# utiasASRL/dICP

Hardware: AMD Instinct MI355X
Metric: ICP cloud-iterations/sec (fwd+bwd), B=256x16384-pt clouds per GPU (higher is better)
Workload: dtype f32

## Files before the change

### dicp_amd/ICP.py

```python
import os.path as osp

import torch
import yaml

from . import _call, _lib
from ._ops import F16_SWEEP_MIN_TARGETS, F16_SWEEP_STATIC_TARGETS, KabschLoop, compute_device, pack_list, packable, prebuild_search, transform_points
from ._loop import CallHints, ICPLoop, LoopConfig, form_tally_wanted, resort_schedule
from .nn import nn


class ICP:
    def __init__(self, config_path=None, icp_type='pt2pl', max_iterations=100, tolerance=1e-12, differentiable=True):
        if config_path is None:
            config_path = osp.join(osp.dirname(osp.abspath(__file__)), 'config', 'dICP_config.yaml')
        with open(config_path, 'r') as f:
            self.config = yaml.safe_load(f)

        prm, log, fun = (self.config['dICP'][k] for k in ('parameters', 'logging', 'functionality'))
        self.icp_type = icp_type
        self.max_iterations = max_iterations
        self.tolerance = tolerance
        self.const_iter = prm['const_iter']
        self.verbose = log['verbose']
        self.target_pad_val = prm['target_pad_val']
        self.source_zeroes_are_pad = prm['source_zeroes_are_pad']
        self.match_ratio_thresh = log['matched_ratio_thresh']
        self.diff = differentiable
        self.nn = nn(self.diff, use_gumbel=fun['gumbel'], eps=fun['gumbel_eps'], tau=fun['gumbel_tau'])
        self.knn_variant = _lib.KNN_AUTO
        self.knn_stats = {}
        self.reuse_matches = True
        self.bwd_window = True
        self.bwd_skip_eps = None
        self.sync_every = None
        self.strict_errors = False
        self.deterministic = False
        self._tuning = dict(
            small_loop=True,
            sweep_resort=None,
            cert_from=None,
            cert_sets=True,
            cert_hint=True,
            cert_backoff=True,
            first_search=True,
            plan_call=True,
            bwd_tail=True,
            one_call=True,
            timing_events=None)
        self._hints = CallHints()
        self._eye = {}

    def icp(self, source, target, T_init, weight=None, trim_dist=None, loss_fn=None, dim=3, source_rows=None, target_rows=None):
        return self.dICP(source, target, T_init, weight, trim_dist, loss_fn, dim, source_rows, target_rows)

    def dICP(self, source, target, T_init, weight=None, trim_dist=None, loss_fn=None, dim=3, source_rows=None, target_rows=None):
        assert dim == 2 or dim == 3, "dim must be 2 or 3"
        unit_w = (weight is None and isinstance(source, torch.Tensor) and isinstance(target, torch.Tensor) and len(source) > 0 and len(target) > 0
                  and not self.source_zeroes_are_pad and not (self.nn.differentiable and self.nn.use_gumbel))
        source, target, T_init, w_pts, rows, per_cloud_w = self._batch(source, target, T_init, weight, unit_weights=unit_w)
        per_cloud_w = per_cloud_w and source.shape[1] > 1 and not self.source_zeroes_are_pad
        assert source.dtype == target.dtype == T_init.dtype
        if self.icp_type == 'pt2pl':
            assert target.shape[2] == 6
        else:
            target = target[:, :, :3]
        if loss_fn is not None and loss_fn['name'] not in ('huber', 'cauchy', 'trim'):
            raise ValueError("Invalid loss name: {}".format(loss_fn['name']))
        home = source.device
        dev = home if source.is_cuda else compute_device()
        source, target, T_init = (t.to(dev) for t in (source, target, T_init))
        w_pts = w_pts.to(dev) if w_pts is not None else None
        src_rows, tgt_rows = self._device_rows(rows, dev)
        if source_rows is not None or target_rows is not None:
            if rows is not None:
                raise ValueError("source_rows / target_rows describe a padded batch: not together with lists of clouds")
            src_rows, tgt_rows = self._given_rows(source_rows, source, "source_rows"), self._given_rows(target_rows, target, "target_rows")
            if src_rows is not None:
                live = (torch.arange(source.shape[1], device=dev)[None, :] < src_rows[:, None]).to(source.dtype)
                w_pts = live if w_pts is None else w_pts * live

        if dim == 2:
            key = ("dim2", source.dtype, dev)
            if key not in self._eye:
                self._eye[key] = torch.tensor([1.0, 1.0, 0.0, 1.0, 1.0, 0.0], dtype=source.dtype, device=dev)
            keep_t = self._eye[key][:target.shape[2]]
            source = source * self._eye[key][:3]
            target = target * keep_t

        loss_name = loss_fn['name'] if loss_fn is not None else None
        soft = bool(self.nn.differentiable and self.nn.use_gumbel)
        if not soft:
            target = target.contiguous()
            source = source.contiguous()
        wants_grad = torch.is_grad_enabled() and any(t.requires_grad for t in (source, target, T_init, w_pts) if t is not None)
        first_search = bool(self._tuning["first_search"]) and self._tuning["timing_events"] is None and not (wants_grad and not self.bwd_window)
        deterministic = bool(self.deterministic) and wants_grad
        if deterministic and soft:
            raise NotImplementedError("ICP.deterministic: not with Gumbel-softmax correspondences (their adjoint adds to the target with float atomics)")
        cfg = LoopConfig(
            icp_type=self.icp_type, differentiable=bool(self.diff), max_iterations=int(self.max_iterations),
            tolerance=float(self.tolerance), trim_dist=trim_dist, loss_name=loss_name,
            loss_metric=float(loss_fn['metric']) if loss_fn is not None else 1.0, dim=dim,
            const_iter=bool(self.const_iter),
            tanh_steepness=float(self.config['dICP']['parameters']['tanh_steepness']),
            match_ratio_thresh=float(self.match_ratio_thresh),
            knn_variant=(_lib.KNN_SWEEP | (self.knn_variant & 0xff00)) if deterministic else self.knn_variant, bwd_window=True if deterministic else bool(self.bwd_window),
            deterministic=deterministic, stats_out=self.knn_stats, hints=self._hints,
            sync_every=self.sync_every, timing_events=self._tuning["timing_events"], small_loop=False if deterministic else bool(self._tuning["small_loop"]),
            src_rows=src_rows, tgt_rows=tgt_rows, sweep_resort=resort_schedule(self._tuning["sweep_resort"], source.shape[0], source.shape[1], int(self.max_iterations), bool(self.reuse_matches), self._tuning["cert_from"]), reuse_matches=bool(self.reuse_matches), cert_from=self._tuning["cert_from"],
            bwd_skip_eps=self.bwd_skip_eps, cert_backoff=bool(self._tuning["cert_backoff"]), cert_sets=bool(self._tuning["cert_sets"]), cert_hint=bool(self._tuning["cert_hint"]),
            plan_call=bool(self._tuning["plan_call"]), bwd_tail=bool(self._tuning["bwd_tail"]), first_search=first_search, strict_errors=bool(self.strict_errors),
            gumbel=(self.nn.eps, self.nn.tau, getattr(self.nn, "_inject_U", None)) if soft else None)
        T_c = T_init.contiguous()
        if self._tuning["one_call"] and not deterministic and _call.eligible(cfg, source, target, T_c, w_pts, wants_grad):
            T, pc, deltas, weights, costs, converged, iterations, matched = _call.CallLoop.apply(source, target, T_c, w_pts, cfg)
        else:
            if not soft:
                rec = self._hints.form_record(dev, (source.shape[0], source.shape[1], target.shape[1], source.dtype)) if source.is_cuda else None
                cfg.prebuilt = prebuild_search(source, target, cfg.knn_variant, wants_grad and bool(cfg.bwd_window), T_init, src_rows, tgt_rows, first_search=first_search,
                                               tally=target.shape[1] < F16_SWEEP_STATIC_TARGETS and form_tally_wanted(rec, target.shape[1] >= F16_SWEEP_MIN_TARGETS))
            T, pc, deltas, weights, costs, converged, iterations, matched = ICPLoop.apply(source.contiguous(), target.contiguous(), T_init, w_pts, cfg)

        if per_cloud_w:
            n_pts = float(source.shape[1])
            on = (w_pts[:, 0] > self.match_ratio_thresh) & (matched > 0)
            matched = torch.where(on, torch.round(matched * n_pts), matched)
        if self.verbose:
            print("ICP converged in {} iterations".format(deltas.shape[1]))
            print("Final del_T_ts: {}".format(torch.linalg.norm(deltas[:, -1])))

        if self.icp_type == 'pt2pt':
            weights = weights.repeat_interleave(3, dim=2)
        results = {
            "pc": pc,
            "T": T,
            "costs": costs.unsqueeze(-1),
            "deltas": deltas.unsqueeze(-1),
            "weights": weights.unsqueeze(-1),
            "stats": {"converged": converged, "iterations": iterations, "matched_ratio": matched},
        }
        if home != dev:
            results = {k: (v.to(home) if k != "stats" else {s: x.to(home) for s, x in v.items()})
                       for k, v in results.items()}
        return results

    def check_errors(self):
        self._hints.check(wait=True)

    def pt2pt_dICP_SVD(self, source, target, T_init, trim_dist=None, huber_delta=None, dim=3, weight=None):
        single = not isinstance(source, list) and source is not None and source.dim() == 2
        s_b, t_b, T_b, w_pts, rows, _ = self._batch(source, target, T_init, weight)
        t_b = t_b[:, :, :3]
        assert s_b.dtype == t_b.dtype == T_b.dtype
        home = s_b.device
        dev = home if s_b.is_cuda else compute_device()
        s_b, t_b, T_b, w_pts = (t.to(dev) for t in (s_b, t_b, T_b, w_pts))
        src_rows, tgt_rows = self._device_rows(rows, dev)
        seed = bool(getattr(self, "svd_seed_T_init", False))
        if seed:
            T_start = T_b
        else:
            key = (int(T_b.shape[0]), T_b.dtype, dev)
            T_start = self._eye.get(key)
            if T_start is None:
                if len(self._eye) > 16:
                    self._eye.clear()
                T_start = self._eye[key] = torch.eye(4, dtype=T_b.dtype, device=dev).expand(T_b.shape[0], 4, 4).contiguous()
        if self._tuning["one_call"] and _call.kabsch_eligible(s_b, t_b, T_start, w_pts, bool(self.const_iter), self.knn_variant, src_rows, tgt_rows):
            T_found, pc, costs, iterations = _call.KabschCall.apply(s_b, t_b, T_start, w_pts, int(self.max_iterations), trim_dist)
        else:
            T_found, costs, iterations = KabschLoop.apply(s_b, t_b, T_start, w_pts, int(self.max_iterations), float(self.tolerance),
                                                          trim_dist, bool(self.const_iter), self.knn_variant, src_rows, tgt_rows, self.sync_every)
            pc = transform_points(s_b, T_found)
        if self.verbose:
            print("ICP converged in {} iterations".format(int(iterations.max().item()) - 1))
        T = T_found if seed else torch.matmul(T_found, T_b)
        self.svd_stats = {"costs": costs, "iterations": iterations}
        if home != dev:
            pc, T = pc.to(home), T.to(home)
        return (pc[0], T[0]) if single else (pc, T)

    def batch_size_handling(self, source, target, T_init=None, weight=None):
        s, t, T, w, _, _ = self._batch(source, target, T_init, weight)
        if self.icp_type == 'pt2pt':
            w = w.repeat_interleave(3, dim=1)
        return s, t, T, w

    @staticmethod
    def _device_rows(rows, dev):
        if rows is None:
            return None, None
        src_len, tgt_len, n_max, m_max = rows
        out = []
        for lens, full, extra in ((src_len, n_max, 0), (tgt_len, m_max, 1)):
# ... 137 lines not shown
```

### dicp_amd/_call.py

```python
import ctypes

import torch

from . import _lib
from . import _loop
from . import _ops
from ._ops import _DT, _on, _p, _stream

MAX_POINTS = 1 << 20
_PLANS = {}


def eligible(cfg, source, target, T_init, w0, need_grad):
    if cfg.gumbel is not None or not cfg.const_iter or cfg.timing_events is not None or cfg.src_rows is not None or cfg.tgt_rows is not None:
        return False
    if not cfg.plan_call or (cfg.knn_variant & 0xff00) or (need_grad and not cfg.bwd_window):
        return False
    dt = source.dtype
    if dt not in _DT or not (source.is_cuda and target.is_cuda and T_init.is_cuda) or target.dtype != dt or T_init.dtype != dt:
        return False
    if not (source.is_contiguous() and target.is_contiguous() and T_init.is_contiguous()) or (w0 is not None and not (w0.is_cuda and w0.is_contiguous() and w0.dtype == dt)):
        return False
    N, n, _ = source.shape
    m, c = target.shape[1], target.shape[2]
    if N * n > MAX_POINTS or N * m > 4 * MAX_POINTS:
        return False
    if tuple(T_init.shape) != (N, 4, 4) or c != (6 if cfg.icp_type == "pt2pl" else 3):
        return False
    kind = cfg.knn_variant & 0xff
    if kind == _lib.KNN_AUTO:
        kind = _ops.auto_knn_kind(N, n, m)
    if kind != _lib.KNN_SWEEP:
        return False
    Kmax = int(cfg.max_iterations)
    resorts = [k for k in cfg.sweep_resort if 0 <= k < Kmax]
    if len([k for k in resorts if k > 0]) >= _lib.MAX_SEGMENTS:
        return False
    cert_from = (max(resorts) if resorts else 0) if cfg.cert_from is None else max(0, int(cfg.cert_from))
    if _loop.certificates_pay(cfg.reuse_matches, Kmax, cert_from, N, n):
        return False
    if _ops.F16_SWEEP and dt == torch.float32 and float(N) * n >= _ops.F16_SWEEP_MIN_QUERIES and m >= _ops.F16_SWEEP_MIN_TARGETS:
        return False
    if _ops.HIST_CHUNK_BYTES // max(1, N * n * max(source.element_size(), 4)) < Kmax:
        return False
    return not torch.cuda.is_current_stream_capturing()


def _plan(code, N, n, m, c, K, dim, need_grad, resort, flags):
    key = (code, N, n, m, c, K, dim, need_grad, resort, flags)
    got = _PLANS.get(key)
    if got is None:
        call = _lib.Call(N=N, n=n, m=m, c=c, K=K, dim=dim, need_grad=need_grad, n_resort=len(resort), flags=flags)
        for i, k in enumerate(resort):
            call.resort[i] = k
        lay = _lib.CallLayout()
        _lib.check(_lib.load().dicp_call_plan(code, ctypes.byref(call), ctypes.byref(lay)), "dicp_call_plan")
        if len(_PLANS) > 256:
            _PLANS.clear()
        got = _PLANS[key] = lay
    return got


class CallLoop(torch.autograd.Function):

    @staticmethod
    def forward(ctx, source, target, T_init, w0, cfg):
        lib = _lib.load()
        dev, dt = source.device, source.dtype
        code, es = _DT[dt], source.element_size()
        N, n, _ = source.shape
        m, c = target.shape[1], target.shape[2]
        K = int(cfg.max_iterations)
        need_grad = int(any(ctx.needs_input_grad[:4]))
        stats = cfg.stats_out
        if stats is not None:
            for key in ("knn_pairs", "searched_again", "budgets", "bwd_live", "certs_off"):
                stats.pop(key, None)
        ctx.set_materialize_grads(False)
        resort = tuple(sorted(set(k for k in cfg.sweep_resort if 0 < k < K)))
        flags = (_lib.CALL_FIRST_SEARCH if cfg.first_search else 0) | (0 if cfg.small_loop else _lib.CALL_NO_SMALL_LOOP)
        L = _plan(code, N, n, m, c, K, int(cfg.dim), need_grad, resort, flags)
        P = cfg.params()
        with _on(dev):
            ws = torch.empty((L.total // es,), dtype=dt, device=dev)
            rs = torch.empty((L.results_total // es,), dtype=dt, device=dev)
            T = torch.empty((N, 4, 4), dtype=dt, device=dev)
            pc = torch.empty((N, n, 3), dtype=dt, device=dev)
            call = _lib.Call(T_out=T.data_ptr(), pc_out=pc.data_ptr(), results=rs.data_ptr(), src=source.data_ptr(), tgt=target.data_ptr(), T_init=T_init.data_ptr(), w0=w0.data_ptr() if w0 is not None else None,
                             N=N, n=n, m=m, c=c, K=K, dim=int(cfg.dim), need_grad=need_grad, n_resort=len(resort), flags=flags,
                             directions=int(_ops.FRAME_DIRECTIONS), quantum=_ops.CENTER_QUANTUM, tolerance=float(cfg.tolerance), workspace=ws.data_ptr())
            for i, k in enumerate(resort):
                call.resort[i] = k
            _lib.check(lib.dicp_call_forward(code, ctypes.byref(P), ctypes.byref(call), _stream()), "dicp_call_forward")
        def piece(off, count, shape):
            return rs.narrow(0, off // es, count).view(shape).data
        deltas = piece(L.deltas, N * K * 6, (N, K, 6))
        weights = piece(L.weights, N * K * n, (N, K, n))
        costs = piece(L.costs, N * K, (N, K))
        iterations = piece(L.iterations, N, (N,))
        matched = piece(L.matched_ratio, N, (N,))
        conv = rs[L.converged // es:L.converged // es + (N + es - 1) // es].view(torch.uint8)[:N].bool()
        if stats is not None:
            stats["knn_pairs"] = ws[L.pairs // es:L.pairs // es + _lib.PAIR_SHARDS * 8 // es].view(torch.int64).clone()
        if need_grad:
            ctx.save_for_backward(source, target, w0, deltas)
            ctx.ws, ctx.call, ctx.cfg, ctx.P, ctx.L = ws, call, cfg, P, L
        ctx.mark_non_differentiable(deltas, weights, costs, conv, iterations, matched)
        return T, pc, deltas, weights, costs, conv, iterations, matched

    @staticmethod
    def backward(ctx, gT, gpc, *_unused):
        src, tgt, w0, deltas = ctx.saved_tensors
        cfg, P, call, FL = ctx.cfg, ctx.P, ctx.call, ctx.L
        lib = _lib.load()
        dev, dt = src.device, src.dtype
        code, es = _DT[dt], src.element_size()
        N, n, _ = src.shape
        m = tgt.shape[1]
        K = call.K
        stats = cfg.stats_out
        want_tgt, want_w = bool(ctx.needs_input_grad[1]), bool(ctx.needs_input_grad[3] and w0 is not None)
        with _on(dev):
            st = _stream()
            gsrc_pc = None
            if gpc is not None:
                gsrc_pc = torch.empty_like(src)
                pcp = torch.empty((N, FL.nblk, _lib.NBWD_PAD), dtype=dt, device=dev)
                pose_K = ctx.ws.as_strided((N, 12), (12, 1), FL.poses // es + K * N * 12)
                _lib.check(lib.dicp_transform_points_bwd(code, _p(src), _p(pose_K), _p(gpc.contiguous()), _p(gsrc_pc), _p(pcp), N, n, st), "dicp_transform_points_bwd")
                gT_pc = _ops._pose_sums_to_gT(pcp, N, dt, dev, st)
                gT = gT_pc if gT is None else gT + gT_pc
            base = ctx.ws.data_ptr()
            F = _lib.LoopBackwardIn(src=src.data_ptr(), tgt_sorted=base + FL.tgt_sorted, w0=w0.data_ptr() if w0 is not None else None, tperm=base + FL.tperm,
                                    qorder=base + FL.orders + (FL.n_orders - 1) * N * n * 4, spos=base + FL.spos, poses=base + FL.poses, deltas=deltas.data_ptr(),
                                    areg=base + FL.areg, alive=base + FL.alive, N=N, n=n, m=m, c=call.c, K=K, K_cap=K, m_pad=FL.m_pad, dim=call.dim,
                                    knn_variant=_lib.KNN_SWEEP | ((1 << 25) if (call.flags & _lib.CALL_NO_SMALL_LOOP) else 0))
            gsrc, gtgt, gT0, gw = _loop.backward_once(lib, code, P, F, cfg, src, tgt, w0, gT, want_tgt, want_w)
            if gsrc_pc is not None:
                gsrc += gsrc_pc
        return gsrc, gtgt, gT0, gw, None


def kabsch_eligible(source, target, T_start, w0, const_iter, knn_variant, src_rows, tgt_rows):
    if not const_iter or src_rows is not None or tgt_rows is not None or (knn_variant & 0xff00):
        return False
    dt = source.dtype
    if dt not in _DT or not (source.is_cuda and target.is_cuda and T_start.is_cuda and w0.is_cuda) or target.dtype != dt or T_start.dtype != dt or w0.dtype != dt:
        return False
    N, n, _ = source.shape
    m = target.shape[1]
    if N * n > MAX_POINTS or N * m > 4 * MAX_POINTS or tuple(T_start.shape) != (N, 4, 4) or tuple(w0.shape) != (N, n):
        return False
    kind = knn_variant & 0xff
    if kind == _lib.KNN_AUTO:
        kind = _ops.auto_knn_kind(N, n, m)
    return kind == _lib.KNN_SWEEP and not torch.cuda.is_current_stream_capturing()


_KPLANS = {}


class KabschCall(torch.autograd.Function):

# ... 63 lines not shown
```

### dicp_amd/_lib.py

```python
import ctypes
import os
import subprocess
import threading

_HERE = os.path.dirname(os.path.abspath(__file__))
_ROOT = os.path.dirname(_HERE)
LIB_PATH = os.environ.get("DICP_HIP_LIB") or os.path.join(_HERE, "libdicp_hip.so")
SOURCES = [os.path.join(_HERE, "csrc", f) for f in ("dicp_kernels.hip", "knn_f16.hip", "dicp_call.hip", "normals.hip", "voxel.hip", "knn_points.hip")]
HEADERS = ([os.path.join(_HERE, "csrc", f) for f in ("dicp_math.h", "dicp_common.h", "dicp_internal.h", "dicp_fill.h", "dicp_normals.h", "dicp_voxel.h", "dicp_topk.h")]
           + [os.path.join(_HERE, "csrc", "kernels_%s.h" % f) for f in ("setup", "search", "setup_sort", "rows", "accumulate", "backward", "soft_svd", "host")]
           + [os.path.join(_ROOT, "include", "dicp_hip.h")])

F32, F64 = 0, 1
PT2PT, PT2PL = 0, 1
LOSS_NONE, LOSS_HUBER, LOSS_CAUCHY, LOSS_TRIM = 0, 1, 2, 3
KNN_AUTO, KNN_VALU, KNN_MFMA, KNN_SWEEP, KNN_GUMBEL = 0, 1, 2, 3, 4
NACC_PAD, NBWD_PAD, KAB_SAVE = 32, 16, 40
PAIR_SHARDS = 64
ABI_VERSION = 11
_ERRORS = {1: "null pointer", 2: "bad shape/stride", 3: "unsupported dtype", 4: "bad enum value", 5: "misaligned buffer"}

vp, i32, i64, f64 = ctypes.c_void_p, ctypes.c_int32, ctypes.c_int64, ctypes.c_double


# ... 32 lines not shown
    _fields_ = [("spos_ref", vp), ("gts_far", vp), ("overwrite", i32), ("skip", vp), ("mref", vp), ("live", vp), ("skip_eps", f64), ("tail_from", i32), ("tail_partials", vp),
                ("tail_arrive", vp), ("det_far_row", vp), ("det_far_val", vp)]


class LoopBuffers(ctypes.Structure):
    _fields_ = [("abi", i32), ("src", vp), ("tgt", vp), ("w_init", vp), ("c", i32), ("K", i32), ("converged", vp), ("iterations", vp), ("matched_ratio", vp), ("n_start", vp), ("n_matched", vp),
                ("partials", vp), ("counters", vp), ("counters_host", vp), ("counters_tag", i32), ("events", vp), ("src_rows", vp), ("tgt_rows", vp),
                ("search", SearchBuffers), ("cert", CertBuffers), ("hist", HistoryBuffers), ("bwd", BwdBuffers)]

    def __init__(self, **kw):
        super().__init__(abi=ABI_VERSION)
        subs = (self, self.search, self.cert, self.hist, self.bwd)
        where = LoopBuffers._KW
        for k, v in kw.items():
            if v is not None:
                i, f = where[k]
                setattr(subs[i], f, v)


LoopBuffers._KW = dict([(f[0], (0, f[0])) for f in LoopBuffers._fields_[:-4]] +
                       [(g + "_" + f[0], (i + 1, f[0])) for i, (g, cls) in enumerate((("search", SearchBuffers), ("cert", CertBuffers), ("hist", HistoryBuffers), ("bwd", BwdBuffers)))
                        for f in cls._fields_])


class GumbelLoop(ctypes.Structure):
    _fields_ = [("U", vp), ("seeds", vp), ("eps", f64), ("tau", f64), ("ps_t", vp), ("nbr", vp), ("lse", vp), ("g_nbr", vp), ("g_ps", vp)]


MAX_SEGMENTS = 16
CERT_OFF_FOR_GOOD = 1 << 20


class SegmentPlan(ctypes.Structure):
    _fields_ = [("nseg", i32), ("k0", i32 * MAX_SEGMENTS), ("k1", i32 * MAX_SEGMENTS), ("new_order", i32 * MAX_SEGMENTS),
                ("cert_from", i32), ("pad0", i32), ("order", vp * MAX_SEGMENTS), ("keys", vp), ("cert_q", vp), ("cert_qu", vp), ("cert_count", vp), ("cert_cloud", vp), ("cert_set", vp),
                ("cert_nbr", vp), ("cert_gdirty", vp), ("cert_pend", vp), ("cert_cm", vp), ("cert_glist", vp), ("cert_gcount", vp), ("cert_slist", vp), ("cert_scount", vp)]


class Call(ctypes.Structure):
    _fields_ = [("src", vp), ("tgt", vp), ("T_init", vp), ("w0", vp), ("N", i32), ("n", i32), ("m", i32), ("c", i32), ("K", i32), ("dim", i32), ("need_grad", i32),
                ("n_resort", i32), ("resort", i32 * MAX_SEGMENTS), ("flags", i32), ("directions", i32), ("quantum", f64), ("tolerance", f64), ("workspace", vp), ("results", vp), ("T_out", vp), ("pc_out", vp)]


_sz = ctypes.c_size_t


class CallLayout(ctypes.Structure):
    _fields_ = ([(k, _sz) for k in ("total", "zeroed", "results_total", "results_zeroed", "T", "pc", "deltas", "weights", "costs", "converged", "iterations", "matched_ratio", "pairs", "n_matched", "counters",
                                    "poses", "poses_search", "alive", "areg", "n_start", "partials", "tgs4", "tperm", "bucket", "brange", "keys", "tgt_sorted", "scratch",
                                    "scratch_bytes", "frame", "pose_s", "orders", "spos")]
                + [("n_orders", i32), ("m_pad", i32), ("nblk", i32), ("pad0", i32)])


class CallGrads(ctypes.Structure):
    _fields_ = [("gT", vp), ("gsrc", vp), ("gtgt", vp), ("gT0", vp), ("gw", vp), ("workspace", vp), ("skip_eps", f64), ("tail_from", i32), ("pad0", i32), ("live_host", vp)]


class CallBackwardLayout(ctypes.Structure):
    _fields_ = ([(k, _sz) for k in ("total", "zeroed", "live", "arrive", "mref", "decisions", "far", "gpose", "gtmp", "src_s", "w_s", "gsrc_s", "gw_s", "slab", "gs", "gb",
                                    "partials", "tail_partials", "spos_ref")] + [("nblk_w", i32), ("pad0", i32)])


class LoopBackwardIn(ctypes.Structure):
    _fields_ = ([(k, vp) for k in ("src", "tgt_sorted", "w0", "tperm", "qorder", "spos", "poses", "deltas", "areg", "alive", "src_rows", "tgt_rows", "spos_of")]
                + [(k, i32) for k in ("N", "n", "m", "c", "K", "K_cap", "m_pad", "dim", "knn_variant", "spos_of_from")]
                + [(k, vp) for k in ("src_s", "w_s", "spos_ref")])


class KabschCall(ctypes.Structure):
    _fields_ = [("src", vp), ("tgt", vp), ("T_start", vp), ("w0", vp), ("N", i32), ("n", i32), ("m", i32), ("c", i32), ("K", i32), ("trim_on", i32), ("directions", i32), ("pad0", i32),
                ("trim_dist", f64), ("quantum", f64), ("tolerance", f64), ("workspace", vp), ("T_out", vp), ("pc_out", vp)]


class KabschCallLayout(ctypes.Structure):
    _fields_ = ([(k, _sz) for k in ("total", "zeroed", "costs", "iterations", "pairs", "counters", "frame", "keys", "tperm", "bucket", "brange", "tgs4", "scratch", "scratch_bytes",
                                    "pose", "pose_search", "pose_used", "partials", "save", "idx", "rows_live", "orders", "gpose", "gacc")] + [("m_pad", i32), ("nblk", i32)])


class KabschCallGrads(ctypes.Structure):
    _fields_ = [("gT", vp), ("gsrc", vp), ("gtgt", vp), ("gw", vp)]


CALL_FIRST_SEARCH, CALL_NO_SMALL_LOOP, CALL_NBKT = 1, 2, 1024


class KabschBuffers(ctypes.Structure):
    _fields_ = [("src", vp), ("tgt", vp), ("w_init", vp), ("c", i32), ("K", i32), ("knn_variant", i32), ("m_pad", i32), ("tgt4", vp), ("tperm", vp),
                ("qorder", vp), ("bucket", vp), ("brange", vp), ("nbkt", i32), ("pad0", i32), ("pairs", vp), ("frame", vp), ("pose", vp),
                ("pose_search", vp), ("pose_used", vp), ("idx", vp), ("partials", vp), ("save", vp), ("costs", vp), ("iterations", vp),
                ("rows_live", vp), ("tgt_rows", vp), ("counters", vp), ("tgt_f16", vp)]


_SIGNATURES = {
    "dicp_abi_version": ([], ctypes.c_int),
    "dicp_copy": ([vp, vp, ctypes.c_size_t, vp], ctypes.c_int),
    "dicp_zero": ([vp, ctypes.c_size_t, vp], ctypes.c_int),
    "dicp_padded_targets": ([i32], ctypes.c_int),
    "dicp_accumulate_blocks": ([i32], ctypes.c_int),
    "dicp_pack_target": ([i32, vp, i32, vp, vp, i32, i32, vp, i32, vp], ctypes.c_int),
    "dicp_search_frame": ([i32, vp, i32, vp, i32, i32, f64, i32, vp, vp, i32, vp, vp, vp], ctypes.c_int),
    "dicp_knn_f16_bytes": ([i32, i32], ctypes.c_size_t),
    "dicp_knn_f16_pack": ([vp, vp, i32, i32, i32, vp, vp], ctypes.c_int),
    "dicp_knn_f16_probe": ([vp, vp, vp, vp, vp, vp, i32, i32, i32, i32, vp, vp], ctypes.c_int),
    "dicp_knn": ([i32, vp, vp, vp, vp, vp, i32, i32, i32, i32, vp, i32, vp, vp], ctypes.c_int),
    "dicp_knn_sweep": ([i32, vp, vp, vp, vp, vp, vp, vp, i32, vp, vp, i32, i32, i32, i32, vp, vp, vp, i32, vp, vp, vp, i32, vp], ctypes.c_int),
    "dicp_window_blocks": ([i32, i32, i32], ctypes.c_int),
    "dicp_window_rows": ([i32], ctypes.c_int),
    "dicp_bwd_tail_max_blocks": ([i32], ctypes.c_int),
    "dicp_sweep_sort_scratch_bytes": ([i32, i32, i32], ctypes.c_size_t),
    "dicp_sweep_sort": ([i32, vp, i32, vp, vp, i32, i32, i32, vp, vp, i32, vp, vp, vp, ctypes.c_size_t, vp], ctypes.c_int),
    "dicp_sweep_build": ([i32, vp, i32, vp, vp, vp, i32, i32, i32, vp, vp, i32, vp], ctypes.c_int),
    "dicp_sweep_setup": ([i32, vp, i32, vp, i32, i32, i32, f64, i32, vp, vp, vp, i32, vp, vp, vp, ctypes.c_size_t, vp, vp, i32, vp, vp, i32, vp, vp, vp, vp], ctypes.c_int),
    "dicp_query_order": ([i32, vp, vp, vp, i32, i32, i32, vp, vp, vp, vp, i32, vp, i32, vp, vp, i32, vp, vp, vp], ctypes.c_int),
    "dicp_query_reorder": ([i32, vp, vp, vp, vp, vp, i32, i32, i32, vp, i32, vp, vp, i32, vp, vp, vp], ctypes.c_int),
    "dicp_query_keys": ([i32, vp, vp, i32, i32, vp, vp], ctypes.c_int),
    "dicp_loop_init": ([i32, vp, vp, ctypes.c_double, i32, i32, i32, vp, vp, vp, vp, vp, vp, vp, vp, i32, vp], ctypes.c_int),
    "dicp_search_pose": ([i32, vp, vp, i32, vp, vp], ctypes.c_int),
    "dicp_loop_finish": ([i32, vp, vp, vp, vp, i32, i32, vp, vp, vp, vp], ctypes.c_int),
    "dicp_accumulate_bwd_window": ([i32, ctypes.POINTER(WeightParams), vp, vp, i32, vp, vp, vp, vp, vp, vp, vp, vp, vp, i32, i32, i32, vp, vp, vp, vp, vp, i32, vp], ctypes.c_int),
    "dicp_resolve_matches": ([vp, vp, i32, vp, i32, i32, vp, vp], ctypes.c_int),
    "dicp_match_order_scratch_bytes": ([i32, i32, i32], ctypes.c_size_t),
    "dicp_match_order": ([i32, vp, vp, i32, i32, vp, ctypes.c_size_t, vp, vp], ctypes.c_int),
    "dicp_window_reduce": ([i32, vp, vp, vp, vp, vp, vp, i32, i32, i32, i32, i32, vp, i32, i32, vp], ctypes.c_int),
    "dicp_permute_add_rows": ([i32, vp, vp, i32, i32, i32, i32, i32, i32, vp, i32, i32, vp], ctypes.c_int),
    "dicp_pose_grad_in": ([i32, vp, vp, i32, vp], ctypes.c_int),
    "dicp_pose_grad_out": ([i32, vp, vp, i32, vp, i32, vp], ctypes.c_int),
    "dicp_permute_rows": ([i32, vp, vp, i32, i32, i32, i32, i32, i32, vp, i32, i32, vp], ctypes.c_int),
    "dicp_gather_rows": ([i32, vp, vp, i32, i32, i32, i32, vp, vp], ctypes.c_int),
    "dicp_scatter_add_rows": ([i32, vp, vp, i32, i32, i32, i32, vp, vp], ctypes.c_int),
    "dicp_pack_list": ([i32, vp, vp, vp, i32, i32, i32, vp, vp, vp], ctypes.c_int),
    "dicp_unpack_list": ([i32, vp, vp, vp, vp, i32, i32, i32, i32, vp], ctypes.c_int),
    "dicp_accumulate": ([i32, ctypes.POINTER(WeightParams), vp, vp, i32, vp, vp, vp, vp, vp, i32, i32, i32, vp, vp, i64, vp], ctypes.c_int),
    "dicp_step": ([i32, ctypes.POINTER(StepIO), i32, vp], ctypes.c_int),
    "dicp_icp_forward": ([i32, ctypes.POINTER(WeightParams), ctypes.POINTER(LoopBuffers), i32, i32, i32, i32, i32, f64, i32, i32, vp], ctypes.c_int),
    "dicp_icp_forward_plan": ([i32, ctypes.POINTER(WeightParams), ctypes.POINTER(LoopBuffers), ctypes.POINTER(SegmentPlan), i32, i32, i32, i32, i32, f64, vp], ctypes.c_int),
    "dicp_icp_backward": ([i32, ctypes.POINTER(WeightParams), ctypes.POINTER(LoopBuffers), i32, i32, i32, i32, vp, vp, i32, vp, vp, vp, vp, vp, vp, i32, i32, vp], ctypes.c_int),
    "dicp_step_bwd": ([i32, vp, vp, i32, i32, vp, vp, i64, vp, vp, vp, vp, i32, vp], ctypes.c_int),
    "dicp_accumulate_bwd": ([i32, ctypes.POINTER(WeightParams), vp, vp, i32, vp, vp, vp, vp, vp, vp, vp, i32, i32, i32, vp, vp, vp, vp, vp], ctypes.c_int),
    "dicp_gumbel_nn": ([i32, vp, vp, i32, vp, ctypes.c_uint32, f64, f64, i32, i32, i32, vp, vp, vp], ctypes.c_int),
    "dicp_gumbel_nn_bwd": ([i32, vp, vp, i32, vp, ctypes.c_uint32, f64, f64, vp, vp, vp, i32, i32, i32, vp, vp, vp], ctypes.c_int),
    "dicp_kabsch_accumulate": ([i32, vp, vp, i32, vp, vp, vp, i32, f64, vp, i32, i32, i32, vp, vp], ctypes.c_int),
    "dicp_kabsch_step": ([i32, vp, i32, vp, vp, vp, i32, vp], ctypes.c_int),
    "dicp_kabsch_step_bwd": ([i32, vp, vp, vp, i32, vp], ctypes.c_int),
    "dicp_kabsch_forward": ([i32, ctypes.POINTER(KabschBuffers), i32, i32, i32, i32, f64, i32, f64, i32, i32, vp], ctypes.c_int),
    "dicp_kabsch_bwd": ([i32, vp, vp, i32, vp, vp, vp, i32, f64, vp, vp, i32, i32, i32, vp, vp, vp, vp], ctypes.c_int),
    "dicp_transform_points": ([i32, vp, vp, vp, i32, i32, vp], ctypes.c_int),
    "dicp_transform_points_bwd": ([i32, vp, vp, vp, vp, vp, i32, i32, vp], ctypes.c_int),
    "dicp_loss_weight": ([i32, i32, i32, f64, f64, vp, i64, i32, vp, vp], ctypes.c_int),
    "dicp_loss_weight_bwd": ([i32, i32, i32, f64, f64, vp, vp, i64, i32, vp, vp], ctypes.c_int),
    "dicp_call_plan": ([i32, ctypes.POINTER(Call), ctypes.POINTER(CallLayout)], ctypes.c_int),
    "dicp_call_forward": ([i32, ctypes.POINTER(WeightParams), ctypes.POINTER(Call), vp], ctypes.c_int),
    "dicp_call_backward_plan": ([i32, ctypes.POINTER(WeightParams), ctypes.POINTER(Call), i32, i32, ctypes.POINTER(CallBackwardLayout)], ctypes.c_int),
    "dicp_call_backward": ([i32, ctypes.POINTER(WeightParams), ctypes.POINTER(Call), ctypes.POINTER(CallGrads), vp], ctypes.c_int),
    "dicp_loop_backward_plan": ([i32, ctypes.POINTER(WeightParams), ctypes.POINTER(LoopBackwardIn), i32, i32, ctypes.POINTER(CallBackwardLayout)], ctypes.c_int),
    "dicp_loop_backward": ([i32, ctypes.POINTER(WeightParams), ctypes.POINTER(LoopBackwardIn), ctypes.POINTER(CallGrads), vp], ctypes.c_int),
    "dicp_loop_backward_prepare": ([i32, ctypes.POINTER(LoopBackwardIn), vp, vp, vp, vp], ctypes.c_int),
    "dicp_kabsch_call_plan": ([i32, ctypes.POINTER(KabschCall), ctypes.POINTER(KabschCallLayout)], ctypes.c_int),
    "dicp_kabsch_call_forward": ([i32, ctypes.POINTER(KabschCall), vp], ctypes.c_int),
    "dicp_kabsch_call_backward": ([i32, ctypes.POINTER(KabschCall), ctypes.POINTER(KabschCallGrads), vp], ctypes.c_int),
    "dicp_normals_workspace_bytes": ([i32, i32, i32, i32, i32, i32], ctypes.c_size_t),
    "dicp_normals_forward": ([i32, vp, i32, vp, i32, i32, i32, vp, i32, vp, vp, vp, vp, ctypes.c_size_t, vp, vp], ctypes.c_int),
    "dicp_normals_backward": ([i32, vp, vp, vp, i32, vp, i32, i32, i32, i32, vp, vp, vp, ctypes.c_size_t, vp], ctypes.c_int),
    "dicp_voxel_workspace_bytes": ([i32, i32, i32, i32], ctypes.c_size_t),
    "dicp_voxel_count": ([i32, vp, i32, vp, i32, i32, f64, f64, f64, vp, i32, i32, vp, vp, ctypes.c_size_t, vp], ctypes.c_int),
    "dicp_voxel_reduce": ([i32, vp, i32, i32, i32, i32, vp, ctypes.c_size_t, vp, vp, vp, vp], ctypes.c_int),
    "dicp_voxel_backward": ([i32, vp, vp, vp, i32, i32, i32, i32, vp, vp], ctypes.c_int),
# ... 74 lines not shown
```

### dicp_amd/_loop.py

```python
import ctypes
import time
from dataclasses import dataclass
from types import SimpleNamespace

import torch

from . import _lib
from . import _ops
from ._ops import (_DT, _LOSS, SweepIndex, _Arena, _gather_rows_raw, _on, _p, _pose_sums_to_gT, _segments, _stream, auto_knn_kind, f16_image,
                   pack_target, require_device, search_frame)


def form_tally_wanted(rec, have_image):
    if rec is None:
        return bool(have_image)
    reporting = rec["event"] is None and (rec["calls"] < 2 or rec["calls"] % 16 == 0)
    return bool(reporting or ((have_image or rec["long"]) and not rec.get("plan")))



class TailTimeout(RuntimeError):
    """A wait inside the one-launch tail of a backward pass ran out (dicp_hip.h, bwd_tail_arrive): that pass poisoned the gradients of the clouds
    concerned with NaN.  Raised by the pass itself when ICP.strict_errors is set (it then waits for its own kernels), else at the next backward pass of the
    same ICP object, or by ICP.check_errors()."""
# ... 26 lines not shown

    def tail_records(self, dev, shape, any_stream=False):
        key = self._where(dev) + tuple(shape)
        if any_stream and not self.tail.get(key):
            same = [recs for k, recs in self.tail.items() if k[0] == key[0] and k[2:] == key[2:] and recs]
            if same:
                return max(same, key=lambda recs: recs[-1][5])
        return self._slot(self.tail, key, list)

    def form_record(self, dev, shape):
        return self._slot(self.form, self._where(dev) + tuple(shape), lambda: {"long": False, "host": None, "event": None, "calls": 0})

    def cert_record(self, dev, shape):
        return self._slot(self.cert, self._where(dev) + tuple(shape), lambda: {"skip": 0, "host": None, "event": None, "calls": 0})

    def check(self, wait=False):
        for recs in self.tail.values():
            for rec in recs:
                if rec[1] is None or rec[4]:
                    continue
                if wait:
                    rec[1].synchronize()
                if rec[1].query():
                    rec[4] = True
                    if int(rec[0][rec[3]]) != 0:
                        raise TailTimeout("dicp_amd: a wait of an earlier backward pass's one-launch tail ran out (the GPU was kept full by other work for "
                                          "~0.5 s); the gradients of that pass were poisoned with NaN.  Re-run it, or set ICP._tuning['bwd_tail'] = False"
                                          "  [report word 0x%08x: arrivals seen %d, block %d, generation %d; live clouds by iteration %s]"
                                          % (int(rec[0][rec[3]]) & 0xffffffff, (int(rec[0][rec[3]]) >> 16) & 0xfff, (int(rec[0][rec[3]]) >> 8) & 0xff,
                                             int(rec[0][rec[3]]) & 0xff, rec[0][:rec[3]].tolist()))


CERT_MIN_WORK = 2.0e6
RESORT_SMALL_POINTS = 262144


def certificates_pay(reuse_matches, Kmax, cert_from, N, n):
    left = Kmax - 1 - cert_from
    return bool(reuse_matches) and left >= 3 and float(left) * N * n >= CERT_MIN_WORK


def resort_schedule(resort, N, n, Kmax, reuse_matches, cert_from):
    if resort is not None:
        return tuple(int(v) for v in resort)
    full, small = (0, 1, 2, 3), (0, 1)
    cf = max([k for k in full if k < Kmax] or [0]) if cert_from is None else max(0, int(cert_from))
    if certificates_pay(reuse_matches, Kmax, cf, N, n) or N * n >= RESORT_SMALL_POINTS:
        return full
    cf_small = max([k for k in small if k < Kmax] or [0]) if cert_from is None else cf
    return full if certificates_pay(reuse_matches, Kmax, cf_small, N, n) else small




@dataclass
class LoopConfig:
    icp_type: str
    differentiable: bool
    max_iterations: int
    tolerance: float
    trim_dist: object
    loss_name: object
    loss_metric: float
    dim: int
    const_iter: bool
    tanh_steepness: float
    match_ratio_thresh: float
    knn_variant: int = _lib.KNN_AUTO
    sweep_resort: tuple = (0, 1, 2, 3)
    bwd_window: bool = True
    stats_out: object = None
    hints: object = None
    sync_every: object = None
    timing_events: object = None
    prebuilt: object = None
    small_loop: bool = True
    cert_from: object = None
    gumbel: object = None
    deterministic: bool = False
    bwd_tail: bool = True
    strict_errors: bool = False
    plan_call: bool = True
    first_search: bool = True
    cert_hint: bool = True
    cert_sets: bool = True
    cert_backoff: bool = True
    reuse_matches: bool = True
    bwd_skip_eps: object = None
    src_rows: object = None
    tgt_rows: object = None

    def params(self):
        return _lib.WeightParams(
            mode=_lib.PT2PL if self.icp_type == "pt2pl" else _lib.PT2PT,
            trim_on=int(self.trim_dist is not None and self.trim_dist >= 0.0),
            differentiable=int(self.differentiable),
            loss=_LOSS[self.loss_name],
            trim_dist=float(self.trim_dist if self.trim_dist is not None else 0.0),
            tanh_k=float(self.tanh_steepness),
            loss_delta=float(self.loss_metric),
            match_thresh=float(self.match_ratio_thresh))



def order_by_matches(src, spos_ref, m, m_pad, src_rows, tgt_rows):
    N, n, _ = src.shape
    qo = torch.empty((N, n), dtype=torch.int32, device=src.device)
    unused = torch.ones((N, 2), dtype=src.dtype, device=src.device)
    with _on(src.device):
        _lib.check(_lib.load().dicp_query_order(_DT[src.dtype], _p(src), None, _p(unused), SweepIndex.NBKT, N, n, _p(qo), None, None, None, 0, _p(spos_ref), int(m_pad),
                                                None, None, int(m), _p(src_rows), _p(tgt_rows), _stream()), "dicp_query_order")
    return qo


def backward_once(lib, code, P, F, cfg, src, tgt, w0c, gT, want_tgt, want_w):
    dev, dt = src.device, src.dtype
    es = src.element_size()
    N, n, m, K, Kcap = F.N, F.n, F.m, F.K, F.K_cap
    stats = cfg.stats_out
    st = _stream()
    L = _lib.CallBackwardLayout()
    _lib.check(lib.dicp_loop_backward_plan(code, ctypes.byref(P), ctypes.byref(F), int(want_tgt), int(want_w), ctypes.byref(L)), "dicp_loop_backward_plan")
    eps = cfg.bwd_skip_eps
    if eps is None:
        eps = 2.0 ** -22 if dt == torch.float32 else 2.0 ** -40
    if cfg.loss_name == "huber" and not cfg.differentiable:
        eps = 0.0
    ws = torch.empty((L.total // es,), dtype=dt, device=dev)
    if stats is not None and eps > 0.0:
        stats["bwd_live"] = ws[L.live // es:L.live // es + (Kcap + 1 + (es // 4) - 1) * 4 // es].view(torch.int32)[:Kcap + 1]
    tail_from, hints, entry = 0, None, None
    capturing = torch.cuda.is_current_stream_capturing()
    use_tail = eps > 0.0 and cfg.bwd_tail and cfg.hints is not None
    if use_tail:
        if not capturing:
            cfg.hints.check()
        hints = cfg.hints.tail_records(dev, (N, n, m, Kcap, dt), any_stream=capturing)
        hint = next((h for h in reversed(hints) if h[2] == (N, n, K) and (capturing or h[1].query())), None)
        if hint is not None and L.nblk_w <= lib.dicp_bwd_tail_max_blocks(code):
            counts = hint[0][:K].tolist()
            tail_from = min(K, max(0, next((k for k in range(K) if counts[k] * 8 >= N), K) - 1))
        if not capturing:
            if len(hints) >= 4:
                if hints[0][1].query() and hints[0][0].numel() >= Kcap + 1:
                    cfg.hints.check()
                    entry = hints.pop(0)
            else:
                entry = [torch.empty((max(Kcap + 1, 64),), dtype=torch.int32).pin_memory(), None, None, Kcap, False, 0]
    tail_word = None
    if tail_from > 0:
        a0 = L.arrive // es
        tail_word = ws[a0:a0 + (N + 1 + (es // 4) - 1) * 4 // es].view(torch.int32)[N:N + 1]
    if stats is not None:
        stats["bwd_tail_from"] = int(tail_from)
        stats["bwd_tail_error"] = tail_word
    gsrc = torch.empty_like(src)
    gtgt = torch.empty_like(tgt) if want_tgt else None
    gw = torch.empty_like(w0c) if want_w else None
    gT0 = torch.empty((N, 4, 4), dtype=dt, device=dev)
    gTc = gT.contiguous() if gT is not None else None
    G = _lib.CallGrads(gT=gTc.data_ptr() if gTc is not None else None, gsrc=gsrc.data_ptr(), gtgt=gtgt.data_ptr() if want_tgt else None,
                       gT0=gT0.data_ptr(), gw=gw.data_ptr() if want_w else None, workspace=ws.data_ptr(), skip_eps=float(eps), tail_from=int(tail_from),
                       live_host=entry[0].data_ptr() if entry is not None else None)
    _lib.check(lib.dicp_loop_backward(code, ctypes.byref(P), ctypes.byref(F), ctypes.byref(G), st), "dicp_loop_backward")
    if entry is not None:
        entry[1] = torch.cuda.Event()
# ... 34 lines not shown
    S.kind = kind
    S.owned = kind == _lib.KNN_SWEEP and S.need_grad and cfg.bwd_window
    if cfg.deterministic and S.need_grad and not S.owned:
        raise NotImplementedError("ICP.deterministic covers the sweep search with the windowed backward (knn_variant KNN_SWEEP, bwd_window): this call "
                                  "would take another form")
    sweep = None
    with_q = S.T_init.dtype == dt and tuple(S.T_init.shape) == (N, 4, 4)
    if kind == _lib.KNN_SWEEP:
        pre = cfg.prebuilt
        if (pre is not None and pre[0].data_ptr() == S.tgt.data_ptr() and pre[0].shape == S.tgt.shape and pre[0].dtype == S.tgt.dtype
                and pre[1].tgt_s is not None and pre[1].tgt_rows is cfg.tgt_rows):
            sweep = pre[1]
        else:
            sweep = SweepIndex(S.tgt, sorted_rows=True, tgt_rows=cfg.tgt_rows,
                               frame=search_frame(S.tgt, tgt_rows=cfg.tgt_rows, src=S.src if with_q else None, T_init=S.T_init if with_q else None, src_rows=cfg.src_rows))
    S.sweep = sweep
    S.soft = kind == _lib.KNN_GUMBEL
    S.center = sweep.frame if sweep is not None else (None if S.soft else search_frame(S.tgt, tgt_rows=cfg.tgt_rows, src=S.src if with_q else None,
                                                                                   T_init=S.T_init if with_q else None, src_rows=cfg.src_rows))
    S.tgt4 = sweep.tgs4 if sweep is not None else (None if S.soft else pack_target(S.tgt, S.center, cfg.tgt_rows))
    S.m_pad = S.tgt4.shape[1] if S.tgt4 is not None else 0
    img16 = f16_image(S.tgt4, m, cfg.tgt_rows) if kind == _lib.KNN_MFMA else (sweep.img16 if sweep is not None else None)
    tally = (sweep is not None and _ops.F16_SWEEP and _ops.F16_SWEEP_ADAPTIVE and dt == torch.float32 and float(N) * n >= _ops.F16_SWEEP_MIN_QUERIES
             and not (cfg.knn_variant & 0xff00) and m < _ops.F16_SWEEP_STATIC_TARGETS)
    form_hint = None
    if tally and cfg.hints is not None and not torch.cuda.is_current_stream_capturing():
        form_hint = cfg.hints.form_record(dev, (N, n, m, dt))
        if form_hint["event"] is not None and form_hint["event"].query():
            rep = form_hint["host"].tolist()
            form_hint["long"] = bool(4 * rep[0] >= N)
            form_hint["moving"] = bool(4 * rep[1] >= N)
            form_hint["plan"] = [0] + [0 if c < 0 else (2 if 2 * c >= N else 1) for c in rep[2:2 + _ops.FORM_PLAN_ITERS]]
            form_hint["event"] = None
        if img16 is None and form_hint["long"]:
            img16 = sweep.make_image()
    S.form_plan = None
    if tally and img16 is not None and form_hint is not None and form_hint.get("plan"):
        pl = form_hint["plan"]
        S.form_plan = (ctypes.c_int32 * S.Kmax)(*[(pl[k] if k < len(pl) else pl[-1]) for k in range(S.Kmax)])
    if tally and not form_tally_wanted(form_hint, img16 is not None):
        tally = False
    S.img16, S.tally, S.form_hint = img16, tally, form_hint
    S.adaptive = bool(tally) and kind == _lib.KNN_SWEEP


def _fwd_certificate_policy(S):
    cfg, N, n, m, dt, dev, Kmax, sweep = S.cfg, S.N, S.n, S.m, S.dt, S.dev, S.Kmax, S.sweep
    S.keep_idx = (sweep is None or (S.need_grad and not S.owned)) and not S.soft
    resorts = [k for k in cfg.sweep_resort if 0 <= k < Kmax]
    S.cert_from = (max(resorts) if resorts else 0) if cfg.cert_from is None else max(0, int(cfg.cert_from))
    want_certs = sweep is not None and not (cfg.knn_variant & 0xff00) and not S.keep_idx and certificates_pay(cfg.reuse_matches, Kmax, S.cert_from, N, n)
    cert_hint = None
    clouds_moving = False
    if want_certs and cfg.cert_hint and cfg.cert_backoff and cfg.hints is not None and not torch.cuda.is_current_stream_capturing():
        cert_hint = cfg.hints.cert_record(dev, (N, n, m, Kmax, dt))
        if cert_hint["host"] is None or cert_hint["host"].shape[0] < N:
            cert_hint["host"] = torch.empty((N, 8), dtype=torch.int32).pin_memory()
        if cert_hint["skip"] > 0:
            cert_hint["skip"] -= 1
            want_certs = False
            clouds_moving = bool(cert_hint.get("moving", False))
        elif cert_hint["event"] is not None and cert_hint["event"].query():
            hc = cert_hint["host"][:N]
            most_off = float((hc[:, 2] > 0).float().mean()) >= 0.5
            if most_off or (N * ((n + 127) // 128) <= 8192 and bool((hc[:, 7] >= 2).any())):
                cert_hint.update(skip=31, calls=0, moving=most_off)
                want_certs = False
                clouds_moving = most_off
            cert_hint["event"] = None
        if want_certs:
            cert_hint["calls"] += 1
    S.clouds_moving = bool(clouds_moving or (not want_certs and S.form_hint is not None and S.form_hint.get("moving", False)))
    S.want_certs, S.cert_hint = want_certs, cert_hint


def _fwd_loop_state(S):
    cfg, lib, N, n, m, c, dt, dev, es, Kmax, sweep = S.cfg, S.lib, S.N, S.n, S.m, S.c, S.dt, S.dev, S.es, S.Kmax, S.sweep
    S.nblk = lib.dicp_accumulate_blocks(n)
    S.poses = torch.empty((Kmax + 1, N, 12), dtype=dt, device=dev)
    S.poses_c = torch.empty((Kmax + 1, N, 12), dtype=dt, device=dev) if S.center is not None else None
    S.alive = torch.empty((Kmax + 1, N), dtype=dt, device=dev)
    S.areg = torch.empty((Kmax, N, 36), dtype=torch.float64, device=dev) if S.need_grad else None
    S.n_start = torch.empty((N,), dtype=dt, device=dev)
    S.partials = torch.empty((N, S.nblk, _lib.NACC_PAD), dtype=dt, device=dev)
    want_certs = S.want_certs
    arena = _Arena(dev)
    arena.take((N, Kmax, 6), dt)
    arena.take((N, Kmax), dt)
    arena.take((N,), torch.uint8)
    arena.take((N,), dt)
    arena.take((N,), dt)
    arena.take((N,), dt)
    arena.take((Kmax,), torch.int32)
    arena.take((Kmax, 128) if want_certs else (0,), torch.int32)
    arena.take((N, 8) if want_certs else (0,), torch.int32)
    arena.take((N, n) if want_certs else (0,), torch.int32)
    arena.take((Kmax + 1, 8) if want_certs else (0,), torch.int32)
    arena.take((Kmax, N) if S.adaptive else (0,), torch.int32)
    arena.take((N,) if (want_certs and cfg.cert_sets) else (0,), torch.int32)
    (S.deltas, S.costs, S.converged, S.iterations, S.matched, S.n_matched, S.counters, cert_count, S.cert_cloud, cert_pend, cert_gcount, S.sweep_form,
     cert_scount) = arena.finish()
    S.certs = None
    if want_certs:
        units = (n + 63) // 64
        S.certs = dict(q=torch.empty((N, n), dtype=dt, device=dev), qu=torch.empty((N, units), dtype=dt, device=dev), count=cert_count,
                       nbr=torch.empty((N, n, 6 if cfg.icp_type == "pt2pl" else 3), dtype=dt, device=dev), gdirty=torch.empty((N, units), dtype=torch.int32, device=dev),
                       cm=torch.empty((N, n), dtype=torch.int32, device=dev), glist=torch.empty((8, max(N, 2) * units), dtype=torch.int32, device=dev), gcount=cert_gcount,
                       slist=torch.empty((N, n), dtype=torch.int32, device=dev) if cfg.cert_sets else None, scount=cert_scount if cfg.cert_sets else None,
                       pend=cert_pend, of=torch.empty((Kmax + 1, N, units), dtype=torch.int32, device=dev) if S.need_grad else None,
                       set=torch.empty((N * n * (es + 16),), dtype=torch.uint8, device=dev) if cfg.cert_sets else None,
                       rmax=torch.empty((N, 4), dtype=dt, device=dev), dcum=torch.empty((N, 2 * (Kmax + 1)), dtype=dt, device=dev))
    certs = S.certs
    _lib.check(lib.dicp_loop_init(S.code, _p(S.T_init.contiguous()), _p(S.w0c), float(cfg.match_ratio_thresh), S.rows, N, n,
                                  _p(S.poses), _p(S.alive), _p(S.n_start), _p(S.center), _p(S.poses_c),
                                  _p(S.src) if certs else None, _p(certs["rmax"]) if certs else None, _p(certs["dcum"]) if certs else None, 2 * (Kmax + 1), S.st),
               "dicp_loop_init")
    S.idx_once = torch.empty((N, n), dtype=torch.int32, device=dev) if (S.keep_idx and not S.need_grad) else None
    S.keep_spos = sweep is not None and S.need_grad
    S.spos_once = torch.empty((N, n), dtype=torch.int32, device=dev) if (sweep is not None and not S.need_grad) else None
    per_iter = N * n * max(es, 4)
    S.kc = max(1, min(Kmax, _ops.HIST_CHUNK_BYTES // max(1, per_iter)))
    S.w_slabs, S.idx_slabs, S.spos_slabs = [], [], []
    cuts = list(range(0, Kmax, S.kc))
    if sweep is not None:
        cuts += list(cfg.sweep_resort) + ([S.cert_from] if certs is not None else [])
    if not cfg.const_iter:
        every = cfg.sync_every
        if every is None:
            every = 1 if float(N) * n * m >= _ops.SWEEP_MIN_PAIRS else 4
        cuts += list(range(0, Kmax, max(1, int(every))))
    S.segs = _segments(Kmax, cuts)
    ev = cfg.timing_events
    S.events = ev.handles(Kmax) if ev is not None else None
    S.gum = None
    if S.soft:
        g_eps, g_tau, inject_U = cfg.gumbel
        S.nbr_hist = torch.empty((Kmax, N, n, c), dtype=dt, device=dev)
        S.lse_hist = torch.empty((Kmax, N, n), dtype=dt, device=dev)
        S.ps_t = torch.empty((N, n, 3), dtype=dt, device=dev)
        S.U_list = [u.to(device=dev, dtype=dt).contiguous() for u in inject_U[:Kmax]] if inject_U is not None else None
        assert S.U_list is None or len(S.U_list) >= Kmax, "one injected noise tensor per iteration"
        S.U_arr = (ctypes.c_void_p * Kmax)(*[u.data_ptr() for u in S.U_list]) if S.U_list is not None else None
        S.seed_list = [int(v) & 0xFFFFFFFF for v in torch.randint(0, 2 ** 31 - 1, (Kmax,)).tolist()] if S.U_list is None else [0] * Kmax
        S.seeds = (ctypes.c_uint32 * Kmax)(*S.seed_list)
        S.gum = _lib.GumbelLoop(U=ctypes.cast(S.U_arr, ctypes.c_void_p) if S.U_arr is not None else None, seeds=ctypes.cast(S.seeds, ctypes.c_void_p),
                                eps=float(g_eps), tau=float(g_tau), ps_t=_p(S.ps_t), nbr=_p(S.nbr_hist), lse=_p(S.lse_hist))
        S.g_eps, S.g_tau = float(g_eps), float(g_tau)
    S.first = cfg.prebuilt[2] if (sweep is not None and cfg.prebuilt is not None and cfg.prebuilt[1] is sweep) else None
    S.have_first = (S.first is not None and S.first[0].data_ptr() == S.src.data_ptr() and S.first[0].shape == S.src.shape
                    and S.first[1].data_ptr() == S.T_init.data_ptr() and S.T_init.is_contiguous())
    S.first_spos = None
    if (S.have_first and len(S.first) > 3 and S.first[3] is not None and not S.keep_idx and S.events is None and not (certs is not None and S.cert_from <= 0)):
        S.first_spos = S.first[3]
        if S.adaptive and sweep.form0 is not None:
            _lib.check(S.lib.dicp_copy(_p(S.sweep_form[0]), _p(sweep.form0), N * 4, S.st), "dicp_copy")
        if not S.keep_spos:
            S.spos_once = S.first_spos
    S.qorders, S.seg_q, S.done_segs = [], [], []
    S.K = Kmax


def _fwd_loop_buffers(S, plan_call):
    cfg, sweep, certs = S.cfg, S.sweep, S.certs
    LB = _lib.LoopBuffers(
        src=_p(S.src), tgt=_p(S.tgt), w_init=_p(S.w0c), c=S.c, K=S.Kmax, search_knn_variant=S.kind | (cfg.knn_variant & 0xff00) | ((0 if cfg.small_loop else 1) << 25), search_m_pad=S.m_pad,
        search_tgt4=_p(S.tgt4), search_tperm=_p(sweep.tperm) if sweep else None,
        search_bucket=_p(sweep.bucket) if sweep else None, search_brange=_p(sweep.brange) if sweep else None,
        search_nbkt=SweepIndex.NBKT, hist_per_iter=int(S.need_grad), search_pairs=_p(sweep.pair_shards) if sweep else None,
        hist_poses=_p(S.poses), hist_deltas=_p(S.deltas), hist_costs=_p(S.costs), hist_areg=_p(S.areg), hist_alive=_p(S.alive), converged=_p(S.converged),
        iterations=_p(S.iterations), matched_ratio=_p(S.matched), n_start=_p(S.n_start), n_matched=_p(S.n_matched),
        search_tgt_sorted=_p(sweep.tgt_s) if sweep is not None else None, search_tgt_sorted_stride=sweep.row_stride if sweep is not None else 0,
        cert_rmax=_p(certs["rmax"]) if certs else None, cert_dcum=_p(certs["dcum"]) if certs else None,
        hist_w_iter=S.n, hist_w_stride=S.kc * S.n,
        partials=_p(S.partials), counters=_p(S.counters), events=S.events, search_frame=_p(S.center), search_poses=_p(S.poses_c),
        src_rows=_p(cfg.src_rows), tgt_rows=_p(cfg.tgt_rows), search_tgt_f16=_p(S.img16),
        search_form=_p(S.sweep_form) if S.adaptive else None, search_form_default=sweep.form_default if sweep is not None else 0,
        search_form_plan=ctypes.cast(S.form_plan, ctypes.c_void_p) if S.form_plan is not None else None)
    if plan_call:
        LB.hist.w = _p(S.w_slabs[0])
        LB.hist.spos = _p(S.spos_slabs[0]) if S.keep_spos else _p(S.spos_once)
        LB.hist.idx = (_p(S.idx_slabs[0]) if S.need_grad else _p(S.idx_once)) if S.keep_idx else None
        LB.search.first_done = int(S.first_spos is not None)
        LB.hist.spos_of = _p(certs["of"]) if certs else None
    if S.gum is not None:
        LB.search.gumbel = ctypes.cast(ctypes.pointer(S.gum), ctypes.c_void_p)
    return LB


def _fwd_new_slab(S, j):
    kk = min(S.kc, S.Kmax - j * S.kc)
    S.w_slabs.append(torch.empty((S.N, S.kc, S.n), dtype=S.dt, device=S.dev))
    if S.need_grad and S.keep_idx:
        S.idx_slabs.append(torch.empty((kk, S.N, S.n), dtype=torch.int32, device=S.dev))
    if S.keep_spos:
        S.spos_slabs.append(torch.empty((kk, S.N, S.n), dtype=torch.int32, device=S.dev))
        if j == 0 and S.first_spos is not None:
            _lib.check(S.lib.dicp_copy(_p(S.spos_slabs[0][0]), _p(S.first_spos), S.first_spos.numel() * 4, S.st), "dicp_copy")


def _fwd_enqueue_plan(S):
    cfg, certs, N, n = S.cfg, S.certs, S.N, S.n
    _fwd_new_slab(S, 0)
    SP = _lib.SegmentPlan(nseg=len(S.segs), cert_from=S.cert_from if certs is not None else -1, keys=_p(S.sweep.keys),
                          cert_q=_p(certs["q"]) if certs else None, cert_qu=_p(certs["qu"]) if certs else None,
                          cert_count=_p(certs["count"]) if certs else None, cert_cloud=_p(S.cert_cloud) if (certs and cfg.cert_backoff) else None,
                          cert_set=_p(certs["set"]) if certs else None, cert_nbr=_p(certs["nbr"]) if certs else None,
                          cert_gdirty=_p(certs["gdirty"]) if certs else None, cert_pend=_p(certs["pend"]) if certs else None,
                          cert_cm=_p(certs["cm"]) if certs else None, cert_glist=_p(certs["glist"]) if certs else None,
                          cert_gcount=_p(certs["gcount"]) if certs else None, cert_slist=_p(certs["slist"]) if certs else None,
                          cert_scount=_p(certs["scount"]) if certs else None)
    n_new = sum(1 for (k0, _) in S.segs if (k0 == 0 or k0 in cfg.sweep_resort)) - (1 if S.have_first else 0)
    fresh_orders = torch.empty((max(n_new, 1), N, n), dtype=torch.int32, device=S.dev)
    used, qorder = 0, None
    for si, (k0, k1) in enumerate(S.segs):
        SP.k0[si], SP.k1[si] = k0, k1
        if k0 == 0 or k0 in cfg.sweep_resort:
            if k0 == 0 and S.have_first:
                qorder, SP.new_order[si] = S.first[2], 0
            else:
                qorder, SP.new_order[si] = fresh_orders[used], 1
                used += 1
            S.qorders.append(qorder)
        else:
            SP.new_order[si] = 0
        SP.order[si] = qorder.data_ptr()
        S.seg_q.append(len(S.qorders) - 1)
        S.done_segs.append((k0, k1))
    LB = _fwd_loop_buffers(S, True)
    _lib.check(S.lib.dicp_icp_forward_plan(S.code, ctypes.byref(S.P), ctypes.byref(LB), ctypes.byref(SP), N, n, S.m, int(cfg.dim), 1, float(cfg.tolerance), S.st),
               "dicp_icp_forward_plan")


_TOL_WORDS = {}


def _tolerance_words(dev, Kmax):
    key = CallHints._where(dev)
    rec = _TOL_WORDS.get(key)
    if rec is None or rec[0].numel() < Kmax:
        t = torch.empty((max(64, Kmax),), dtype=torch.int32).pin_memory()
        rec = _TOL_WORDS[key] = [t, t.numpy(), rec[2] if rec else 0, (rec[3] + [rec[0]]) if rec else []]
    rec[2] = (rec[2] + 1) % 0x7ff
    rec[1][:Kmax] = -1
    return rec, rec[2] << 20


def _words_converged_at(pending, view, tag):
    k0, k1 = pending
# ... 444 lines not shown
```

### dicp_amd/csrc/dicp_call.hip

```cpp
#include <hip/hip_runtime.h>
#include <string.h>
#include "dicp_hip.h"
#include "dicp_fill.h"

namespace {

struct Carver {
    size_t off = 0;
    size_t take(size_t bytes) {
        size_t o = off;
        off += (bytes + 255) / 256 * 256;
        return o;
    }
};

inline size_t esize(int dtype) { return dtype == DICP_F64 ? 8 : 4; }

inline bool call_ok(int dtype, const dicp_call* c) {
    if (dtype != DICP_F32 && dtype != DICP_F64) return false;
    if (c->N < 1 || c->n < 1 || c->m < 1 || c->K < 1 || (c->c != 3 && c->c != 6) || (c->dim != 2 && c->dim != 3)) return false;
    if (c->n_resort < 0 || c->n_resort >= DICP_MAX_SEGMENTS) return false;
    int prev = 0;
    for (int i = 0; i < c->n_resort; ++i) {
        if (c->resort[i] <= prev || c->resort[i] >= c->K) return false;
        prev = c->resort[i];
    }
    return true;
}

inline int zero_fill(void* p, size_t bytes, hipStream_t st) { return dicp_fill::zero(p, bytes, st); }

inline char* at(const dicp_call* c, size_t off) { return (char*)c->workspace + off; }
inline char* res(const dicp_call* c, size_t off) { return (char*)c->results + off; }

template <typename T>
__global__ void kabsch_prep_kernel(int32_t* __restrict__ rows_live, int N, int n) {
    const int b = blockIdx.x * blockDim.x + threadIdx.x;
    if (b < N) rows_live[b] = n;
}
template <typename T>
__global__ void kabsch_finish_kernel(const T* __restrict__ pose, T* __restrict__ iterations, T* __restrict__ T_out, int N, int K) {
    const int i = blockIdx.x * blockDim.x + threadIdx.x;
    if (i >= N * 16) return;
    const int b = i >> 4, e = i & 15, row = e >> 2, col = e & 3;
    T v = row == 3 ? (col == 3 ? T(1) : T(0)) : (col == 3 ? pose[b * 12 + 9 + row] : pose[b * 12 + row * 3 + col]);
    T_out[i] = v;
    if (e == 0 && iterations[b] == T(0)) iterations[b] = T(K);
}
template <typename T>
__global__ void kabsch_gpose_kernel(const T* __restrict__ gT, T* __restrict__ gpose, int N) {
    const int i = blockIdx.x * blockDim.x + threadIdx.x;
    if (i >= N * 12) return;
    const int b = i / 12, e = i % 12;
    gpose[i] = gT ? (e < 9 ? gT[b * 16 + (e / 3) * 4 + e % 3] : gT[b * 16 + (e - 9) * 4 + 3]) : T(0);
}

inline bool kabsch_call_ok(int dtype, const dicp_kabsch_call* c) {
    return (dtype == DICP_F32 || dtype == DICP_F64) && c->N >= 1 && c->n >= 1 && c->m >= 1 && c->K >= 1 && (c->c == 3 || c->c == 6);
}
inline char* kat(const dicp_kabsch_call* c, size_t off) { return (char*)c->workspace + off; }
inline int last_launch() { const hipError_t e = hipGetLastError(); return e == hipSuccess ? 0 : -(int)e; }

}

extern "C" {

int dicp_call_plan(int dtype, const dicp_call* c, dicp_call_layout* L) {
    if (!c || !L) return DICP_ERR_NULL;
    if (!call_ok(dtype, c)) return dtype != DICP_F32 && dtype != DICP_F64 ? DICP_ERR_DTYPE : DICP_ERR_SHAPE;
    const size_t es = esize(dtype), N = c->N, n = c->n, K = c->K;
    memset(L, 0, sizeof(*L));
    L->m_pad = dicp_padded_targets(c->m);
    L->nblk = dicp_accumulate_blocks(c->n);
    L->n_orders = 1 + c->n_resort;
    const size_t m_pad = L->m_pad;
    Carver rs;
    L->deltas = rs.take(N * K * 6 * es);
    L->costs = rs.take(N * K * es);
    L->converged = rs.take(N);
    L->iterations = rs.take(N * es);
    L->matched_ratio = rs.take(N * es);
    L->results_zeroed = rs.off;
    L->weights = rs.take(N * K * n * es);
    L->results_total = rs.off;
    Carver w;
    L->n_matched = w.take(N * es);
    L->counters = w.take(K * 4);
    L->pairs = w.take(DICP_PAIR_SHARDS * 8);
    L->zeroed = w.off;
    L->T = w.take(N * 16 * es);
    L->pc = w.take(N * n * 3 * es);
    L->poses = w.take((K + 1) * N * 12 * es);
    L->poses_search = w.take((K + 1) * N * 12 * es);
    L->alive = w.take((K + 1) * N * es);
    L->areg = c->need_grad ? w.take(K * N * 36 * 8) : 0;
    L->n_start = w.take(N * es);
    L->partials = w.take(N * L->nblk * DICP_NACC_PAD * es);
    L->tgs4 = w.take(N * m_pad * 4 * es);
    L->tperm = w.take(N * m_pad * 4);
    L->bucket = w.take(N * (DICP_CALL_NBKT + 1) * 4);
    L->brange = w.take(N * 2 * es);
    L->keys = w.take(N * m_pad * es);
    L->tgt_sorted = w.take(N * m_pad * c->c * es);
    L->scratch_bytes = dicp_sweep_sort_scratch_bytes(dtype, c->N, L->m_pad);
    L->scratch = L->scratch_bytes ? w.take(L->scratch_bytes) : 0;
    L->frame = w.take(N * 12 * es);
    L->pose_s = w.take(N * 12 * es);
    L->orders = w.take((size_t)L->n_orders * N * n * 4);
    L->spos = w.take((c->need_grad ? K : 1) * N * n * 4);
    L->total = w.off;
    return 0;
}

int dicp_call_forward(int dtype, const dicp_weight_params* prm, const dicp_call* c, void* stream) {
    if (!prm || !c || !c->src || !c->tgt || !c->T_init || !c->workspace || !c->results) return DICP_ERR_NULL;
    dicp_call_layout L;
    if (int rc = dicp_call_plan(dtype, c, &L)) return rc;
    if (((uintptr_t)c->workspace & 255) != 0 || ((uintptr_t)c->results & 255) != 0) return DICP_ERR_ALIGN;
    const size_t es = esize(dtype), N = c->N, n = c->n;
    const int K = c->K;
    hipStream_t st = (hipStream_t)stream;
    if (int rc = zero_fill(c->workspace, L.zeroed, st)) return rc;
    if (int rc = zero_fill(c->results, L.results_zeroed, st)) return rc;
    int32_t* order0 = (int32_t*)at(c, L.orders);
    int32_t* spos = (int32_t*)at(c, L.spos);
    if (int rc = dicp_sweep_setup(dtype, c->tgt, c->c, nullptr, c->N, c->m, L.m_pad, c->quantum, c->directions, at(c, L.frame), at(c, L.keys),
                                  (int32_t*)at(c, L.tperm), DICP_CALL_NBKT, (int32_t*)at(c, L.bucket), at(c, L.brange), L.scratch_bytes ? at(c, L.scratch) : nullptr,
                                  L.scratch_bytes, at(c, L.tgs4), at(c, L.tgt_sorted), c->c, c->src, nullptr, c->n, c->T_init, at(c, L.pose_s), order0, stream))
        return rc;
    const bool first_search = (c->flags & DICP_CALL_FIRST_SEARCH) != 0;
    if (first_search)
        if (int rc = dicp_knn_sweep(dtype, c->src, at(c, L.pose_s), at(c, L.tgs4), (int32_t*)at(c, L.tperm), order0, (int32_t*)at(c, L.bucket), at(c, L.brange),
                                    DICP_CALL_NBKT, nullptr, nullptr, c->N, c->n, c->m, L.m_pad, nullptr, spos, (unsigned long long*)at(c, L.pairs), 0, nullptr, nullptr, nullptr, 0, stream))
            return rc;
    if (int rc = dicp_loop_init(dtype, c->T_init, c->w0, prm->match_thresh, prm->mode == DICP_PT2PT ? 3 : 1, c->N, c->n, at(c, L.poses), at(c, L.alive),
                                at(c, L.n_start), at(c, L.frame), at(c, L.poses_search), nullptr, nullptr, nullptr, 2 * (K + 1), stream))
        return rc;
    dicp_segment_plan SP;
    memset(&SP, 0, sizeof(SP));
    SP.cert_from = -1;
    SP.keys = at(c, L.keys);
    int cuts[DICP_MAX_SEGMENTS + 1], nc = 0;
    cuts[nc++] = 0;
    for (int i = 0; i < c->n_resort; ++i) cuts[nc++] = c->resort[i];
    cuts[nc] = K;
    SP.nseg = nc;
    for (int s = 0; s < nc; ++s) {
        SP.k0[s] = cuts[s];
        SP.k1[s] = cuts[s + 1];
        SP.new_order[s] = s > 0;
        SP.order[s] = order0 + (size_t)s * N * n;
    }
    dicp_loop_buffers B;
    memset(&B, 0, sizeof(B));
    B.abi = DICP_ABI_VERSION;
    B.src = c->src; B.tgt = c->tgt; B.w_init = c->w0; B.c = c->c; B.K = K;
    B.search.knn_variant = DICP_KNN_SWEEP | ((c->flags & DICP_CALL_NO_SMALL_LOOP) ? (1 << 25) : 0);
    B.search.m_pad = L.m_pad;
    B.search.tgt4 = at(c, L.tgs4); B.search.tperm = (int32_t*)at(c, L.tperm); B.search.bucket = (int32_t*)at(c, L.bucket); B.search.brange = at(c, L.brange);
    B.search.nbkt = DICP_CALL_NBKT; B.hist.per_iter = c->need_grad ? 1 : 0; B.search.pairs = (unsigned long long*)at(c, L.pairs);
    B.hist.poses = at(c, L.poses); B.hist.deltas = res(c, L.deltas); B.hist.costs = res(c, L.costs); B.hist.areg = c->need_grad ? (double*)at(c, L.areg) : nullptr;
    B.hist.alive = at(c, L.alive); B.converged = (uint8_t*)res(c, L.converged); B.iterations = res(c, L.iterations); B.matched_ratio = res(c, L.matched_ratio);
    B.n_start = at(c, L.n_start); B.n_matched = at(c, L.n_matched);
    B.search.tgt_sorted = at(c, L.tgt_sorted); B.search.tgt_sorted_stride = c->c;
    B.hist.w_iter = c->n; B.hist.w_stride = (int64_t)K * c->n; B.hist.w = res(c, L.weights);
    B.hist.spos = spos;
    B.partials = at(c, L.partials); B.counters = (int32_t*)at(c, L.counters);
    B.search.frame = at(c, L.frame); B.search.poses = at(c, L.poses_search);
    B.search.first_done = first_search ? 1 : 0;
    if (int rc = dicp_icp_forward_plan(dtype, prm, &B, &SP, c->N, c->n, c->m, c->dim, 1, c->tolerance, stream)) return rc;
    char* pose_K = at(c, L.poses) + (size_t)K * N * 12 * es;
    if (int rc = dicp_loop_finish(dtype, pose_K, at(c, L.alive) + (size_t)K * N * es, at(c, L.n_start), at(c, L.n_matched), K, c->N, res(c, L.iterations),
                                  res(c, L.matched_ratio), c->T_out ? c->T_out : at(c, L.T), stream))
        return rc;
    return dicp_transform_points(dtype, c->src, pose_K, c->pc_out ? c->pc_out : at(c, L.pc), c->N, c->n, stream);
}

static int backward_layout(int dtype, const dicp_weight_params* prm, int N_, int n_, int m_, int Kcap_, bool has_w0, int want_tgt, int want_w, dicp_call_backward_layout* L) {
    const size_t es = esize(dtype), N = N_, n = n_, K = Kcap_;
    const int m_pad = dicp_padded_targets(m_), cv = prm->mode == DICP_PT2PL ? 6 : 3;
    memset(L, 0, sizeof(*L));
    L->nblk_w = dicp_window_blocks(dtype, n_, m_pad);
    const size_t nblk = (size_t)(L->nblk_w > dicp_accumulate_blocks(n_) ? L->nblk_w : dicp_accumulate_blocks(n_));
    Carver w;
    L->mref = w.take(N * 8);
    L->decisions = w.take(N * 4);
    L->live = w.take((K + 1) * 4);
    L->arrive = w.take((N + 1) * 4);
    L->far = want_tgt ? w.take(N * (size_t)m_pad * cv * es) : 0;
    L->zeroed = w.off;
    L->gpose = w.take(N * 12 * 8);
    L->gtmp = w.take(N * 12 * 8);
    L->src_s = w.take(N * n * 3 * es);
    L->w_s = has_w0 ? w.take(N * n * es) : 0;
    L->gsrc_s = w.take(N * n * 3 * es);
    L->gw_s = want_w ? w.take(N * n * es) : 0;
    L->slab = want_tgt ? w.take(N * (size_t)L->nblk_w * dicp_window_rows(dtype) * cv * es) : 0;
    L->gs = w.take(N * 36 * es);
    L->gb = w.take(N * 6 * es);
    L->partials = w.take(N * nblk * DICP_NBWD_PAD * es);
    L->tail_partials = w.take(N * (size_t)L->nblk_w * DICP_NBWD_PAD * es);
    L->spos_ref = w.take(N * n * 4);
    L->total = w.off;
    return 0;
}

static int prepare_pass(int dtype, const dicp_loop_backward_in* f, void* src_s, void* w_s, int32_t* spos_ref, void* stream) {
    if (int rc = dicp_gather_rows(dtype, f->src, f->qorder, f->N, f->n, f->n, 3, src_s, stream)) return rc;
    if (f->w0)
        if (int rc = dicp_gather_rows(dtype, f->w0, f->qorder, f->N, f->n, f->n, 1, w_s, stream)) return rc;
    if (spos_ref)
        if (int rc = dicp_resolve_matches(f->spos, f->spos_of, f->K - 1, f->src_rows, f->N, f->n, spos_ref, stream)) return rc;
    return 0;
}

static int backward_once(int dtype, const dicp_weight_params* prm, const dicp_loop_backward_in* f, const dicp_call_grads* g, void* stream) {
    const int want_tgt = g->gtgt != nullptr, want_w = g->gw != nullptr;
    if (want_w && !f->w0) return DICP_ERR_NULL;
    const int cv = prm->mode == DICP_PT2PL ? 6 : 3;
    if (f->c != cv) return DICP_ERR_SHAPE;
    if (((uintptr_t)g->workspace & 255) != 0) return DICP_ERR_ALIGN;
    dicp_call_backward_layout L;
    backward_layout(dtype, prm, f->N, f->n, f->m, f->K_cap, f->w0 != nullptr, want_tgt, want_w, &L);
    const size_t N = f->N, n = f->n;
    const int K = f->K;
    const bool skip = g->skip_eps > 0.0;
    int tail_from = skip ? g->tail_from : 0;
    if (tail_from < 0) return DICP_ERR_SHAPE;
    if (tail_from > K) tail_from = K;
    hipStream_t st = (hipStream_t)stream;
    char* W = (char*)g->workspace;
    if (int rc = zero_fill(W, L.zeroed, st)) return rc;
    double* gpose = (double*)(W + L.gpose);
    double* gtmp = (double*)(W + L.gtmp);
    if (int rc = dicp_pose_grad_in(dtype, g->gT, gpose, f->N, stream)) return rc;
    const int32_t* qo = f->qorder;
    const bool prepared = f->src_s != nullptr;
    if (prepared && f->w0 && !f->w_s) return DICP_ERR_NULL;
    const char* src_s = prepared ? (const char*)f->src_s : W + L.src_s;
    const char* w_s = f->w0 ? (prepared ? (const char*)f->w_s : W + L.w_s) : nullptr;
// ... 190 lines not shown
```

### dicp_amd/csrc/dicp_kernels.hip

```cpp
#include <hip/hip_runtime.h>
#include <hip/hip_ext.h>
#include <stdint.h>

#include "dicp_common.h"
#include "dicp_internal.h"
#include "dicp_fill.h"

namespace {

#include "kernels_setup.h"
#include "kernels_search.h"
#include "kernels_setup_sort.h"
#include "kernels_rows.h"
#include "kernels_accumulate.h"
#include "kernels_backward.h"
#include "kernels_soft_svd.h"
#include "kernels_host.h"

}

extern "C" {

int dicp_abi_version(void) { return DICP_ABI_VERSION; }
int dicp_copy(void* dst, const void* src, size_t bytes, void* stream) {
// ... 302 lines not shown
#undef DICP_SWEEP_CG
#undef DICP_SWEEP_ARGS
    return launch_status();
}

int dicp_knn_sweep(int dtype, const void* src, const void* pose, const void* tgs4, const int32_t* tperm,
                   const int32_t* qorder, const int32_t* bucket, const void* brange, int nbkt, const int32_t* src_rows, const int32_t* tgt_rows,
                   int N, int n, int m, int m_pad, int32_t* idx, int32_t* spos, unsigned long long* pairs, int cfg, const void* f16_image,
                   const int32_t* form_in, int32_t* form_out, int form_default, void* stream) {
    if (!src || !tgs4 || !tperm || !bucket || !brange || (!idx && !spos)) return DICP_ERR_NULL;
    if (bad_dtype(dtype)) return DICP_ERR_DTYPE;
    if (N <= 0 || n <= 0 || m <= 0 || nbkt <= 0 || m_pad != dicp_padded_targets(m)) return DICP_ERR_SHAPE;
    if ((uintptr_t)tgs4 % (dtype == DICP_F32 ? 16 : 32)) return DICP_ERR_ALIGN;
    begin_launch();
    return sweep_launch(dtype, src, pose, tgs4, tperm, qorder, bucket, brange, nbkt, N, n, m, m_pad, idx, spos, pairs, cfg, Rows{src_rows, tgt_rows}, (hipStream_t)stream,
                        CertArgs{}, f16_image, FormArgs{form_in, form_out, form_default});
}

int dicp_gather_rows(int dtype, const void* tgt, const int32_t* idx, int N, int n, int m, int c, void* out, void* stream) {
    if (!tgt || !idx || !out) return DICP_ERR_NULL;
    if (bad_dtype(dtype)) return DICP_ERR_DTYPE;
    if (N <= 0 || n <= 0 || m <= 0 || c <= 0) return DICP_ERR_SHAPE;
    hipStream_t st = (hipStream_t)stream;
    begin_launch();
    if ((size_t)n * c > 0x7fffffffu) return DICP_ERR_SHAPE;
    const int bpc = (int)(((size_t)n * c + BLOCK * ROWS_U - 1) / (BLOCK * ROWS_U));
    const unsigned g = grid_for(N, bpc);
#define DICP_ROWS(K, T, C) K<T, C><<<g, BLOCK, 0, st>>>((const T*)tgt, idx, N, n, m, c, bpc, (T*)out)
#define DICP_ROWS_C(K, T) do { if (c == 1) DICP_ROWS(K, T, 1); else if (c == 3) DICP_ROWS(K, T, 3); else if (c == 6) DICP_ROWS(K, T, 6); \
        else DICP_ROWS(K, T, 0); } while (0)
    if (dtype == DICP_F32) DICP_ROWS_C(gather_kernel, float); else DICP_ROWS_C(gather_kernel, double);
#undef DICP_ROWS
    return launch_status();
}

int dicp_pack_list(int dtype, const void* const* ptrs, const int32_t* lens, const int32_t* strides, int N, int n_max, int cols, void* out, const void* pad, void* stream) {
    if (!ptrs || !lens || !strides || !out) return DICP_ERR_NULL;
    if (bad_dtype(dtype)) return DICP_ERR_DTYPE;
    if (N <= 0 || n_max <= 0 || cols <= 0) return DICP_ERR_SHAPE;
    hipStream_t st = (hipStream_t)stream;
    begin_launch();
    const int bpc = (int)blocks_for((size_t)n_max * cols);
    if (dtype == DICP_F32) pack_list_kernel<float><<<grid_for(N, bpc), BLOCK, 0, st>>>((const float* const*)ptrs, lens, strides, N, n_max, cols, bpc, (float*)out, (const float*)pad);
    else                   pack_list_kernel<double><<<grid_for(N, bpc), BLOCK, 0, st>>>((const double* const*)ptrs, lens, strides, N, n_max, cols, bpc, (double*)out, (const double*)pad);
    return launch_status();
}
int dicp_unpack_list(int dtype, const void* gout, void* const* ptrs, const int32_t* lens, const int32_t* strides, int N, int n_max, int cols, int stride_max, void* stream) {
    if (!gout || !ptrs || !lens || !strides) return DICP_ERR_NULL;
    if (bad_dtype(dtype)) return DICP_ERR_DTYPE;
    if (N <= 0 || n_max <= 0 || cols <= 0 || stride_max < cols) return DICP_ERR_SHAPE;
    hipStream_t st = (hipStream_t)stream;
    begin_launch();
    const int bpc = (int)blocks_for((size_t)n_max * stride_max);
    if (dtype == DICP_F32) unpack_list_kernel<float><<<grid_for(N, bpc), BLOCK, 0, st>>>((const float*)gout, (float* const*)ptrs, lens, strides, N, n_max, cols, bpc);
    else                   unpack_list_kernel<double><<<grid_for(N, bpc), BLOCK, 0, st>>>((const double*)gout, (double* const*)ptrs, lens, strides, N, n_max, cols, bpc);
    return launch_status();
}
int dicp_scatter_add_rows(int dtype, const void* gout, const int32_t* idx, int N, int n, int m, int c, void* gtgt, void* stream) {
    if (!gout || !idx || !gtgt) return DICP_ERR_NULL;
    if (bad_dtype(dtype)) return DICP_ERR_DTYPE;
    if (N <= 0 || n <= 0 || m <= 0 || c <= 0) return DICP_ERR_SHAPE;
    hipStream_t st = (hipStream_t)stream;
    begin_launch();
    if ((size_t)n * c > 0x7fffffffu) return DICP_ERR_SHAPE;
    const int bpc = (int)blocks_for((size_t)n * c);
    const unsigned g = grid_for(N, bpc);
#define DICP_ROWS(K, T, C) K<T, C><<<g, BLOCK, 0, st>>>((const T*)gout, idx, N, n, m, c, bpc, (T*)gtgt)
    if (dtype == DICP_F32) DICP_ROWS_C(scatter_add_kernel, float); else DICP_ROWS_C(scatter_add_kernel, double);
#undef DICP_ROWS
#undef DICP_ROWS_C
    return launch_status();
}

static int check_params(const dicp_weight_params* p, int c) {
    if (!p) return DICP_ERR_NULL;
    if (p->mode != DICP_PT2PT && p->mode != DICP_PT2PL) return DICP_ERR_ENUM;
    if (p->loss < DICP_LOSS_NONE || p->loss > DICP_LOSS_TRIM) return DICP_ERR_ENUM;
    if (p->mode == DICP_PT2PL ? (c != 6 && c != 8) : (c != 3 && c != 4 && c != 6 && c != 8)) return DICP_ERR_SHAPE;
    return 0;
}

static int accumulate_go(int dtype, const dicp_weight_params* prm, const void* src, const void* tgt, int c,
                         const int32_t* idx, const void* pose, const void* w_init, const void* alive, const int32_t* src_rows,
                         int N, int n, int m, void* partials, void* w_out, int64_t w_stride, void* stream, const CertAcc* ca, const void* w_prev = nullptr) {
    if (const int e = check_params(prm, c)) return e;
    if (!src || !tgt || !partials) return DICP_ERR_NULL;
    if (bad_dtype(dtype)) return DICP_ERR_DTYPE;
    if (N <= 0 || n <= 0 || m <= 0 || (w_out && w_stride < n) || (!idx && !ca && m != n)) return DICP_ERR_SHAPE;
    hipStream_t st = (hipStream_t)stream;
    begin_launch();
    const WeightParams P = to_params(prm);
    const int bpc = dicp_accumulate_blocks(n);
    const unsigned g = grid_for(N, bpc);
    hipEvent_t ev0, ev1;
    take_launch_events(ev0, ev1);
#define DICP_ACC(T, M, CERT, PS) hipExtLaunchKernelGGL((accumulate_kernel<T, M, CERT>), dim3(g), dim3(BLOCK), 0, st, ev0, ev1, 0, P, (const T*)src, (const T*)tgt, c, idx, (const T*)pose, \
        (const T*)w_init, (const T*)alive, N, n, m, bpc, (T*)partials, (T*)w_out, (long)w_stride, src_rows, PS, (const T*)w_prev)
#define DICP_ACC_T(T) do { \
        AccCert<T> ps{}; \
        if (ca) { \
            ps.spos = ca->spos; ps.hist = ca->hist; ps.hist_prev = ca->hist_prev; ps.of = ca->of; ps.k_floor = ca->k_floor; ps.N = N; ps.nwr = (n + WAVE - 1) / WAVE; ps.k = ca->k; \
            ps.nbr = (T*)ca->nbr; ps.gdirty = ca->gdirty; ps.pend = ca->pend; ps.cloud = ca->cloud; ps.fresh = ca->fresh; ps.units = ca->units; ps.sets = ca->sets; ps.scount = ca->scount; \
            if (P.mode == MODE_PT2PL) DICP_ACC(T, MODE_PT2PL, true, ps); else DICP_ACC(T, MODE_PT2PT, true, ps); \
        } else { if (P.mode == MODE_PT2PL) DICP_ACC(T, MODE_PT2PL, false, ps); else DICP_ACC(T, MODE_PT2PT, false, ps); } } while (0)
    if (dtype == DICP_F32) DICP_ACC_T(float); else DICP_ACC_T(double);
#undef DICP_ACC_T
#undef DICP_ACC
    return launch_status();
}

int dicp_accumulate(int dtype, const dicp_weight_params* prm, const void* src, const void* tgt, int c,
                    const int32_t* idx, const void* pose, const void* w_init, const void* alive, const int32_t* src_rows,
                    int N, int n, int m, void* partials, void* w_out, int64_t w_stride, void* stream) {
    return accumulate_go(dtype, prm, src, tgt, c, idx, pose, w_init, alive, src_rows, N, n, m, partials, w_out, w_stride, stream, nullptr);
}

int dicp_step(int dtype, const dicp_step_io* io, int N, void* stream) {
    if (!io || !io->partials || !io->pose_in || !io->pose_out || !io->delta || !io->cost || !io->alive || !io->alive_out ||
        !io->converged || !io->iterations || !io->matched_ratio || !io->n_start) return DICP_ERR_NULL;
    if (bad_dtype(dtype)) return DICP_ERR_DTYPE;
    if (N <= 0 || io->nblk <= 0 || (io->dim != 2 && io->dim != 3) || io->delta_stride < 6 || io->cost_stride < 1 ||
        (io->w_cur && io->w_stride < io->n)) return DICP_ERR_SHAPE;
    hipStream_t st = (hipStream_t)stream;
    begin_launch();
    if (dtype == DICP_F32) step_kernel<float><<<N, WAVE, 0, st>>>(*io, N);
    else                   step_kernel<double><<<N, WAVE, 0, st>>>(*io, N);
    return launch_status();
}

struct SkipHost { int32_t* skip; double* mref; const void* alive_k; int32_t* live_k; double eps; int k; };
static int step_bwd_go(int dtype, const double* gpose_in, const void* bwd_partials, int nblk, int dim,
                       const void* pose_k, const void* delta_k, int64_t delta_stride, const double* areg_k,
                       void* gs, void* gb, double* gpose_out, int N, void* stream, const SkipHost& sh) {
    if (!gpose_in || !pose_k || !delta_k || !areg_k || !gs || !gb || !gpose_out || (sh.skip && !sh.mref)) return DICP_ERR_NULL;
    if (bad_dtype(dtype)) return DICP_ERR_DTYPE;
    if (N <= 0 || (dim != 2 && dim != 3) || delta_stride < 6 || (bwd_partials && nblk <= 0)) return DICP_ERR_SHAPE;
    hipStream_t st = (hipStream_t)stream;
    begin_launch();
    if (dtype == DICP_F32)
        step_bwd_kernel<float><<<N, WAVE, 0, st>>>(gpose_in, (const float*)bwd_partials, nblk, dim, (const float*)pose_k,
                                                  (const float*)delta_k, (long)delta_stride, areg_k, (float*)gs, (float*)gb, gpose_out, N,
                                                  SkipArgs<float>{sh.skip, sh.mref, (const float*)sh.alive_k, sh.live_k, sh.eps, sh.k});
    else
        step_bwd_kernel<double><<<N, WAVE, 0, st>>>(gpose_in, (const double*)bwd_partials, nblk, dim, (const double*)pose_k,
                                                   (const double*)delta_k, (long)delta_stride, areg_k, (double*)gs, (double*)gb, gpose_out, N,
                                                   SkipArgs<double>{sh.skip, sh.mref, (const double*)sh.alive_k, sh.live_k, sh.eps, sh.k});
    return launch_status();
}
int dicp_step_bwd(int dtype, const double* gpose_in, const void* bwd_partials, int nblk, int dim,
                  const void* pose_k, const void* delta_k, int64_t delta_stride, const double* areg_k,
                  void* gs, void* gb, double* gpose_out, int N, void* stream) {
    return step_bwd_go(dtype, gpose_in, bwd_partials, nblk, dim, pose_k, delta_k, delta_stride, areg_k, gs, gb, gpose_out, N, stream, SkipHost{});
}

static int accumulate_bwd_go(int dtype, const dicp_weight_params* prm, const void* src, const void* tgt, int c,
                             const int32_t* idx, const void* pose, const void* w_init, const void* alive,
                             const void* gs, const void* gb, const int32_t* src_rows, int N, int n, int m,
                             void* gsrc, void* gtgt, void* gw, void* bwd_partials, void* stream, const int32_t* skip);
int dicp_accumulate_bwd(int dtype, const dicp_weight_params* prm, const void* src, const void* tgt, int c,
                        const int32_t* idx, const void* pose, const void* w_init, const void* alive,
                        const void* gs, const void* gb, const int32_t* src_rows, int N, int n, int m,
                        void* gsrc, void* gtgt, void* gw, void* bwd_partials, void* stream) {
    return accumulate_bwd_go(dtype, prm, src, tgt, c, idx, pose, w_init, alive, gs, gb, src_rows, N, n, m, gsrc, gtgt, gw, bwd_partials, stream, nullptr);
}
static int accumulate_bwd_go(int dtype, const dicp_weight_params* prm, const void* src, const void* tgt, int c,
                             const int32_t* idx, const void* pose, const void* w_init, const void* alive,
                             const void* gs, const void* gb, const int32_t* src_rows, int N, int n, int m,
                             void* gsrc, void* gtgt, void* gw, void* bwd_partials, void* stream, const int32_t* skip) {
    if (const int e = check_params(prm, c)) return e;
    if (!src || !tgt || !gs || !gb || !gsrc || !bwd_partials || (gw && !w_init)) return DICP_ERR_NULL;
    if (bad_dtype(dtype)) return DICP_ERR_DTYPE;
    if (N <= 0 || n <= 0 || m <= 0 || (!idx && m != n)) return DICP_ERR_SHAPE;
    hipStream_t st = (hipStream_t)stream;
    begin_launch();
    const WeightParams P = to_params(prm);
    const int bpc = dicp_accumulate_blocks(n);
    const unsigned g = grid_for(N, bpc);
#define DICP_BWD(T, M) accumulate_bwd_kernel<T, M><<<g, BLOCK, 0, st>>>(P, (const T*)src, (const T*)tgt, c, idx, (const T*)pose, \
        (const T*)w_init, (const T*)alive, (const T*)gs, (const T*)gb, N, n, m, bpc, (T*)gsrc, (T*)gtgt, (T*)gw, (T*)bwd_partials, src_rows, skip)
    if (dtype == DICP_F32) { if (P.mode == MODE_PT2PL) DICP_BWD(float, MODE_PT2PL); else DICP_BWD(float, MODE_PT2PT); }
    else                   { if (P.mode == MODE_PT2PL) DICP_BWD(double, MODE_PT2PL); else DICP_BWD(double, MODE_PT2PT); }
#undef DICP_BWD
    return launch_status();
}

int dicp_gumbel_nn(int dtype, const void* x, const void* y, int c, const void* U, uint32_t seed, double eps, double tau,
                   int N, int n, int m, void* out, void* lse, void* stream) {
    if (!x || !y || !out || !lse) return DICP_ERR_NULL;
    if (bad_dtype(dtype)) return DICP_ERR_DTYPE;
    if (N <= 0 || n <= 0 || m <= 0 || (c != 3 && c != 6) || !(tau > 0.0)) return DICP_ERR_SHAPE;
    hipStream_t st = (hipStream_t)stream;
    begin_launch();
    const int bpc = (n + BLOCK - 1) / BLOCK;
    const unsigned g = grid_for(N, bpc);
#define DICP_GF(T, C) gumbel_fwd_kernel<T, C><<<g, BLOCK, 0, st>>>((const T*)x, (const T*)y, (const T*)U, seed, (T)eps, (T)(1.0 / tau), (T*)out, (T*)lse, N, n, m, bpc)
    if (dtype == DICP_F32) { if (c == 6) DICP_GF(float, 6); else DICP_GF(float, 3); }
    else                   { if (c == 6) DICP_GF(double, 6); else DICP_GF(double, 3); }
#undef DICP_GF
    return launch_status();
}

static int gumbel_nn_bwd_go(int dtype, const void* x, const void* y, int c, const void* U, uint32_t seed, double eps, double tau,
                            const void* out, const void* lse, const void* gout, int N, int n, int m, void* gx, void* gy, int add_gy, void* stream);
int dicp_gumbel_nn_bwd(int dtype, const void* x, const void* y, int c, const void* U, uint32_t seed, double eps, double tau,
                       const void* out, const void* lse, const void* gout, int N, int n, int m, void* gx, void* gy, void* stream) {
// ... 230 lines not shown
    hipStream_t st = (hipStream_t)stream;
    begin_launch();
    const int bpc = dicp_window_blocks(dtype, n, m_pad);
    const int rpc = (m * cv + BLOCK * WR_U - 1) / (BLOCK * WR_U);
    const unsigned g = grid_for(N, rpc);
#define DICP_RED(T, CVV) window_reduce_kernel<T, WindowRows<T>::v, CVV><<<g, BLOCK, 0, st>>>((const T*)slab, spos_ref, qorder, tperm, (const T*)gts_far, N, n, m, m_pad, cv, \
        window_slots(WindowRows<T>::v, n, m_pad), bpc, rpc, (T*)gtgt, c, overwrite, src_rows)
    if (dtype == DICP_F32) { if (cv == 6) DICP_RED(float, 6); else DICP_RED(float, 3); }
    else                   { if (cv == 6) DICP_RED(double, 6); else DICP_RED(double, 3); }
#undef DICP_RED
    return launch_status();
}

static int permute_rows(int dtype, const void* in, const int32_t* perm, int N, int cnt, int in_rows, int perm_rows, int c_in, int cols,
                        void* out, int out_rows, int c_out, int overwrite, void* stream);
int dicp_permute_add_rows(int dtype, const void* in, const int32_t* perm, int N, int cnt, int in_rows, int perm_rows, int c_in, int cols,
                          void* out, int out_rows, int c_out, void* stream) {
    return permute_rows(dtype, in, perm, N, cnt, in_rows, perm_rows, c_in, cols, out, out_rows, c_out, 0, stream);
}
int dicp_permute_rows(int dtype, const void* in, const int32_t* perm, int N, int cnt, int in_rows, int perm_rows, int c_in, int cols,
                      void* out, int out_rows, int c_out, void* stream) {
    return permute_rows(dtype, in, perm, N, cnt, in_rows, perm_rows, c_in, cols, out, out_rows, c_out, 1, stream);
}
static int permute_rows(int dtype, const void* in, const int32_t* perm, int N, int cnt, int in_rows, int perm_rows, int c_in, int cols,
                        void* out, int out_rows, int c_out, int overwrite, void* stream) {
    if (!in || !perm || !out) return DICP_ERR_NULL;
    if (bad_dtype(dtype)) return DICP_ERR_DTYPE;
    if (N <= 0 || cnt <= 0 || cnt > in_rows || cnt > perm_rows || cols <= 0 || cols > c_in || cols > c_out || out_rows <= 0) return DICP_ERR_SHAPE;
    hipStream_t st = (hipStream_t)stream;
    begin_launch();
    if ((size_t)cnt * cols > 0x7fffffffu) return DICP_ERR_SHAPE;
    const int bpc = (int)(((size_t)cnt * cols + BLOCK * ROWS_U - 1) / (BLOCK * ROWS_U));
    const unsigned g = grid_for(N, bpc);
#define DICP_PERM(T, C) permute_add_rows_kernel<T, C><<<g, BLOCK, 0, st>>>((const T*)in, perm, N, cnt, in_rows, perm_rows, c_in, cols, (T*)out, out_rows, c_out, bpc, overwrite)
#define DICP_PERM_C(T) do { if (cols == 1) DICP_PERM(T, 1); else if (cols == 3) DICP_PERM(T, 3); else if (cols == 6) DICP_PERM(T, 6); else DICP_PERM(T, 0); } while (0)
    if (dtype == DICP_F32) DICP_PERM_C(float); else DICP_PERM_C(double);
#undef DICP_PERM
#undef DICP_PERM_C
    return launch_status();
}

constexpr long SMALL_PAIRS = 128L * 1024;
static bool small_loop_eligible(int dtype, int kind, int knn_variant, int n, int m_pad) {
    if (kind == DICP_KNN_SWEEP || kind == DICP_KNN_MFMA || ((knn_variant >> 25) & 1) || ((knn_variant >> 8) & 0xff)) return false;
    const size_t lds = (size_t)m_pad * (dtype == DICP_F32 ? 16 : 32);
    return lds <= 48 * 1024 && (long)n * m_pad <= SMALL_PAIRS;
}

static int transform_points_bwd_go(int dtype, const void* src, const void* pose, const void* gout, void* gsrc, void* partials, int N, int n, int add, void* stream);
static int report_counters(const dicp_loop_buffers* B, int const_iter, int k0, int k1, void* stream) {
    if (const_iter || !B->counters_host || k1 <= k0) return 0;
    begin_launch();
    counters_report_kernel<<<1, WAVE, 0, (hipStream_t)stream>>>(B->counters, B->counters_host, k0, k1 - k0, B->counters_tag);
    return launch_status();
}

int dicp_icp_forward(int dtype, const dicp_weight_params* prm, const dicp_loop_buffers* B, int N, int n, int m,
                     int dim, int const_iter, double tolerance, int k0, int k1, void* stream) {
    if (!prm || !B || !B->src || !B->tgt || !B->hist.poses || !B->hist.deltas || !B->hist.costs || !B->hist.alive ||
        !B->converged || !B->iterations || !B->matched_ratio || !B->n_start || !B->n_matched || !B->hist.w ||
        !B->partials || !B->counters) return DICP_ERR_NULL;
    if (B->abi != DICP_ABI_VERSION) return DICP_ERR_ABI;
    if (bad_dtype(dtype)) return DICP_ERR_DTYPE;
    if (k0 < 0 || k1 > B->K || k0 > k1 || N <= 0 || n <= 0 || m <= 0 || B->hist.w_stride < n || B->hist.w_iter < n) return DICP_ERR_SHAPE;
    const size_t es = dtype == DICP_F32 ? 4 : 8;
    const int kind = B->search.knn_variant & 0xff;
    const dicp_gumbel_loop* G = kind == DICP_KNN_GUMBEL ? B->search.gumbel : nullptr;
    if (kind == DICP_KNN_GUMBEL) { if (!G || !G->ps_t || !G->nbr || !G->lse || (!G->U && !G->seeds)) return DICP_ERR_NULL; }
    else if ((!B->hist.idx && !B->hist.spos) || (kind == DICP_KNN_SWEEP ? (!B->search.tperm || !B->search.bucket || !B->search.brange) : !B->search.tgt4)) return DICP_ERR_NULL;
    hipStream_t st = (hipStream_t)stream;
    const int nblk = dicp_accumulate_blocks(n);
    if (!G && small_loop_eligible(dtype, kind, B->search.knn_variant, n, B->search.m_pad) && k1 > k0) {
        if (const int e = check_params(prm, B->c)) return e;
        begin_launch();
        const WeightParams P = to_params(prm);
        const size_t lds = (size_t)B->search.m_pad * (dtype == DICP_F32 ? sizeof(float4) : sizeof(double4));
#define DICP_SMALL(T, M) icp_small_forward_kernel<T, M><<<N, BLOCK, lds, st>>>(P, *B, N, n, m, dim, const_iter, tolerance, k0, k1)
        if (dtype == DICP_F32) { if (P.mode == MODE_PT2PL) DICP_SMALL(float, MODE_PT2PL); else DICP_SMALL(float, MODE_PT2PT); }
        else                   { if (P.mode == MODE_PT2PL) DICP_SMALL(double, MODE_PT2PL); else DICP_SMALL(double, MODE_PT2PT); }
#undef DICP_SMALL
        if (const int e = launch_status()) return e;
        return report_counters(B, const_iter, k0, k1, stream);
    }
    for (int k = k0; k < k1; ++k) {
        const char* pose_k = (const char*)B->hist.poses + (size_t)k * N * 12 * es;
        const char* pose_s = B->search.poses ? (const char*)B->search.poses + (size_t)k * N * 12 * es : pose_k;
        int32_t* idx_k = B->hist.idx ? B->hist.idx + (B->hist.per_iter ? (size_t)k * N * n : 0) : nullptr;
        char* w_k = (char*)B->hist.w + (size_t)k * B->hist.w_iter * es;
        const char* w_prev_k = k > k0 ? (const char*)B->hist.w + (size_t)(k - 1) * B->hist.w_iter * es : (const char*)B->hist.w_prev0;
        const char* alive_k = (const char*)B->hist.alive + (size_t)k * N * es;
        if (B->events) {
            if (kind == DICP_KNN_SWEEP) set_launch_events((hipEvent_t)B->events[6 * k + 0], (hipEvent_t)B->events[6 * k + 1]);
            else if (hipEventRecord((hipEvent_t)B->events[6 * k + 0], st) != hipSuccess) return -(int)hipGetLastError();
        }
        int rc;
        if (kind == DICP_KNN_SWEEP) {
            int cfg = (B->search.knn_variant >> 8) & 0xff;
            int32_t* spos_k = B->hist.spos ? B->hist.spos + (B->hist.per_iter ? (size_t)k * N * n : 0) : nullptr;
            const bool sorted_rows = B->search.tgt_sorted && spos_k;
            if (!sorted_rows && !B->hist.idx) { set_launch_events(nullptr, nullptr); return DICP_ERR_NULL; }
            const int cfg_plain = cfg ? cfg : sweep_auto_cfg(N, n);
            const bool cert = B->cert.q && B->cert.qu && B->cert.rmax && B->cert.dcum && spos_k && sorted_rows && !B->hist.idx && B->search.qorder && sweep_queries_per_lane(cfg_plain) > 0;
            if (cert && (!B->cert.nbr || !B->cert.gdirty || !B->cert.pend || !B->cert.cm || !B->cert.glist || !B->cert.gcount || (B->cert.set && (!B->cert.slist || !B->cert.scount)) || (B->hist.per_iter && !B->hist.spos_of))) { set_launch_events(nullptr, nullptr); return DICP_ERR_NULL; }
            const int cert_units = cert ? (n + WAVE * sweep_queries_per_lane(cfg_plain) - 1) / (WAVE * sweep_queries_per_lane(cfg_plain)) : 0;
            const int glist_cap = guard_list_cap(N, n);
            const bool fresh = k == 0 || (k == k0 && B->cert.reset);
            int32_t* count_k = B->cert.count ? B->cert.count + (size_t)k * 2 * CERT_SHARDS : nullptr;
            const bool searched = B->search.first_done && k == 0 && !cert && spos_k && !B->hist.idx;
            if (searched) rc = 0;
            else if (cert) {
                begin_launch();
                rc = sweep_launch(dtype, B->src, pose_s, B->search.tgt4, B->search.tperm, B->search.qorder, B->search.bucket, B->search.brange, B->search.nbkt, N, n, m, B->search.m_pad, nullptr, spos_k,
                                  B->search.pairs, cfg, Rows{B->src_rows, B->tgt_rows}, st, CertArgs{B->cert.q, B->cert.qu, B->cert.dcum, 2 * (B->K + 1), k, count_k, !fresh, B->cert.cloud, B->cert.set,
                                                                                              B->cert.cm, B->cert.pend, B->cert.gdirty, B->cert.set ? B->cert.slist : nullptr, B->cert.set ? B->cert.scount : nullptr,
                                                                                              B->cert.glist, B->cert.gcount ? B->cert.gcount + (size_t)k * 8 : nullptr, glist_cap});
            } else
            {
                const int planned = (B->search.form_plan && B->search.tgt_f16) ? B->search.form_plan[k] : 0;
                const int32_t* form_in = (!planned && B->search.form && B->search.tgt_f16 && k > 0) ? B->search.form + (size_t)(k - 1) * N : nullptr;
                int32_t* form_out = B->search.form ? B->search.form + (size_t)k * N : nullptr;
                const void* img = planned ? (planned == 2 ? B->search.tgt_f16 : nullptr) : ((form_in || B->search.form_default || !B->search.form) ? B->search.tgt_f16 : nullptr);
                begin_launch();
                rc = sweep_launch(dtype, B->src, pose_s, B->search.tgt4, B->search.tperm, B->search.qorder, B->search.bucket, B->search.brange, B->search.nbkt, N, n, m, B->search.m_pad, B->hist.idx ? idx_k : nullptr, spos_k, B->search.pairs, cfg,
                                  Rows{B->src_rows, B->tgt_rows}, st, CertArgs{}, img, FormArgs{form_in, form_out, B->search.form_default});
            }
            set_launch_events(nullptr, nullptr);
            if (rc) return rc;
            if (B->events) set_launch_events((hipEvent_t)B->events[6 * k + 2], (hipEvent_t)B->events[6 * k + 3]);
            if (cert) {
                const CertAcc ca{spos_k, B->hist.spos, B->hist.spos_prev_chunk, B->hist.per_iter ? B->hist.spos_of : nullptr, B->hist.spos_floor, k,
                                 B->cert.nbr, B->cert.gdirty, B->cert.pend, B->cert.cloud, fresh ? 1 : 0, cert_units, B->cert.set ? 1 : 0, B->cert.scount};
                rc = accumulate_go(dtype, prm, B->src, B->search.tgt_sorted, B->search.tgt_sorted_stride, spos_k, pose_k, B->w_init, alive_k, B->src_rows, N, n, B->search.m_pad,
                                   B->partials, w_k, B->hist.w_stride, stream, &ca, w_prev_k);
            } else if (sorted_rows)
                rc = accumulate_go(dtype, prm, B->src, B->search.tgt_sorted, B->search.tgt_sorted_stride, spos_k, pose_k, B->w_init, alive_k, B->src_rows, N, n, B->search.m_pad,
                                   B->partials, w_k, B->hist.w_stride, stream, nullptr, w_prev_k);
            else
                rc = accumulate_go(dtype, prm, B->src, B->tgt, B->c, idx_k, pose_k, B->w_init, alive_k, B->src_rows, N, n, m, B->partials, w_k, B->hist.w_stride, stream, nullptr, w_prev_k);
            set_launch_events(nullptr, nullptr);
            if (rc) return rc;
        } else if (G) {
            char* nbr_k = (char*)G->nbr + (size_t)k * N * n * B->c * es;
            char* lse_k = (char*)G->lse + (size_t)k * N * n * es;
            rc = dicp_transform_points(dtype, B->src, pose_k, G->ps_t, N, n, stream);
            if (!rc) rc = dicp_gumbel_nn(dtype, G->ps_t, B->tgt, B->c, G->U ? G->U[k] : nullptr, G->seeds ? G->seeds[k] : 0u, G->eps, G->tau, N, n, m, nbr_k, lse_k, stream);
            if (rc) return rc;
            if (B->events) {
                if (hipEventRecord((hipEvent_t)B->events[6 * k + 1], st) != hipSuccess) return -(int)hipGetLastError();
                set_launch_events((hipEvent_t)B->events[6 * k + 2], (hipEvent_t)B->events[6 * k + 3]);
            }
            rc = accumulate_go(dtype, prm, B->src, nbr_k, B->c, nullptr, pose_k, B->w_init, alive_k, nullptr, N, n, n, B->partials, w_k, B->hist.w_stride, stream, nullptr, w_prev_k);
            set_launch_events(nullptr, nullptr);
            if (rc) return rc;
        } else {
            rc = dicp_knn(dtype, B->src, pose_s, B->search.tgt4, B->src_rows, B->tgt_rows, N, n, m, B->search.m_pad, idx_k, B->search.knn_variant & 0xffff, B->search.tgt_f16, stream);
            if (rc) return rc;
            if (B->events) {
                if (hipEventRecord((hipEvent_t)B->events[6 * k + 1], st) != hipSuccess) return -(int)hipGetLastError();
                set_launch_events((hipEvent_t)B->events[6 * k + 2], (hipEvent_t)B->events[6 * k + 3]);
            }
            rc = accumulate_go(dtype, prm, B->src, B->tgt, B->c, idx_k, pose_k, B->w_init, alive_k, B->src_rows, N, n, m, B->partials, w_k, B->hist.w_stride, stream, nullptr, w_prev_k);
            set_launch_events(nullptr, nullptr);
            if (rc) return rc;
        }
        dicp_step_io io = make_step_io(*B, k, k0, N, n, prm->mode, dim, const_iter, tolerance, es, nblk);
        io.w_copied = w_prev_k ? 1 : 0;
        if (kind == DICP_KNN_SWEEP && B->cert.q && B->cert.qu && B->cert.glist && B->cert.gcount && B->cert.rmax && B->cert.dcum && k + 1 < B->K) {
            const int cfgp = ((B->search.knn_variant >> 8) & 0xff) ? ((B->search.knn_variant >> 8) & 0xff) : sweep_auto_cfg(N, n);
            const int Qp = sweep_queries_per_lane(cfgp);
            if (Qp > 0) {
                io.cert_qu = B->cert.qu; io.cert_units = (n + WAVE * Qp - 1) / (WAVE * Qp); io.glist_cap = guard_list_cap(N, n);
                io.glist = B->cert.glist; io.gcount = B->cert.gcount + (size_t)(k + 1) * 8;
                io.cert_scount = B->cert.set ? B->cert.scount : nullptr; io.cert_slist = B->cert.set ? B->cert.slist : nullptr;
            }
        }
        rc = dicp_step(dtype, &io, N, stream);
        if (rc) return rc;
    }
    return report_counters(B, const_iter, k0, k1, stream);
}

int dicp_icp_forward_plan(int dtype, const dicp_weight_params* prm, const dicp_loop_buffers* buf, const dicp_segment_plan* S, int N, int n, int m,
                          int dim, int const_iter, double tolerance, void* stream) {
    if (!prm || !buf || !S) return DICP_ERR_NULL;
    if (buf->abi != DICP_ABI_VERSION) return DICP_ERR_ABI;
    if (bad_dtype(dtype)) return DICP_ERR_DTYPE;
    if (S->nseg <= 0 || S->nseg > DICP_MAX_SEGMENTS) return DICP_ERR_SHAPE;
    const size_t es = dtype == DICP_F32 ? 4 : 8;
    dicp_loop_buffers B = *buf;
    const int32_t* order_before = nullptr;
    int k_before = 0;
    for (int s = 0; s < S->nseg; ++s) {
        const int k0 = S->k0[s], k1 = S->k1[s];
        if (k0 < 0 || k1 > B.K || k0 >= k1 || (s > 0 && k0 != S->k1[s - 1])) return DICP_ERR_SHAPE;
        int32_t* qo = S->order[s];
        if (qo && S->new_order[s]) {
            if (!S->keys) return DICP_ERR_NULL;
            const char* poses_s = (const char*)(B.search.poses ? B.search.poses : B.hist.poses);
            if (const int rc = query_order_go(dtype, B.src, poses_s + (size_t)k0 * N * 12 * es, B.search.brange, B.search.nbkt, N, n, qo, nullptr, nullptr, nullptr, 0, nullptr, B.search.m_pad,
                                              S->keys, B.search.bucket, m, B.src_rows, B.tgt_rows, (order_before && order_before != qo) ? poses_s + (size_t)k_before * N * 12 * es : nullptr,
                                              order_before != qo ? order_before : nullptr, stream)) return rc;
        }
        if (qo && qo != order_before) { order_before = qo; k_before = k0; }
        B.search.qorder = qo;
        const bool certs = S->cert_from >= 0 && k0 >= S->cert_from;
        B.cert.q = certs ? S->cert_q : nullptr; B.cert.qu = certs ? S->cert_qu : nullptr; B.cert.count = certs ? S->cert_count : nullptr;
        B.cert.cloud = certs ? S->cert_cloud : nullptr;
        B.cert.set = certs ? S->cert_set : nullptr;
        B.cert.nbr = certs ? S->cert_nbr : nullptr; B.cert.gdirty = certs ? S->cert_gdirty : nullptr; B.cert.pend = certs ? S->cert_pend : nullptr; B.cert.cm = certs ? S->cert_cm : nullptr; B.cert.glist = certs ? S->cert_glist : nullptr; B.cert.gcount = certs ? S->cert_gcount : nullptr; B.cert.slist = certs ? S->cert_slist : nullptr; B.cert.scount = certs ? S->cert_scount : nullptr;
        B.cert.reset = (S->cert_from >= 0 && k0 == S->cert_from) ? 1 : 0;
        B.hist.spos_prev_chunk = nullptr; B.hist.spos_floor = 0;
        B.hist.w_prev0 = k0 > 0 ? (const char*)B.hist.w + (size_t)(k0 - 1) * B.hist.w_iter * es : nullptr;
        if (const int rc = dicp_icp_forward(dtype, prm, &B, N, n, m, dim, const_iter, tolerance, k0, k1, stream)) return rc;
    }
    return 0;
}

int dicp_icp_backward(int dtype, const dicp_weight_params* prm, const dicp_loop_buffers* B, int N, int n, int m, int dim,
                      double* gpose, double* gpose_tmp, int have_partials, void* gs, void* gb, void* gsrc, void* gtgt, void* gw,
                      void* bwd_partials, int k0, int k1, void* stream) {
    const dicp_gumbel_loop* G = (B && (B->search.knn_variant & 0xff) == DICP_KNN_GUMBEL) ? B->search.gumbel : nullptr;
    if (!prm || !B || !B->src || !B->tgt || !B->hist.poses || !B->hist.deltas || !B->hist.areg || !B->hist.alive || (!G && !B->hist.idx && !B->hist.spos) || (gw && !B->w_init) ||
        !gpose || !gpose_tmp || !gs || !gb || !gsrc || !bwd_partials) return DICP_ERR_NULL;
    if (B->abi != DICP_ABI_VERSION) return DICP_ERR_ABI;
    if ((B->search.knn_variant & 0xff) == DICP_KNN_GUMBEL && (!G || !G->ps_t || !G->nbr || !G->lse || !G->g_nbr || !G->g_ps || (!G->U && !G->seeds))) return DICP_ERR_NULL;
    if (bad_dtype(dtype)) return DICP_ERR_DTYPE;
    if (k0 < 0 || k1 > B->K || k0 > k1 || !B->hist.per_iter || (B->hist.spos && (B->search.m_pad <= 0 || !B->bwd.spos_ref))) return DICP_ERR_SHAPE;
    if (B->bwd.skip && (!B->bwd.mref || !(B->bwd.skip_eps >= 0.0))) return DICP_ERR_NULL;
    const size_t es = dtype == DICP_F32 ? 4 : 8;
    hipStream_t st = (hipStream_t)stream;
    const int nblk = B->hist.spos ? dicp_window_blocks(dtype, n, B->search.m_pad) : dicp_accumulate_blocks(n);
    {
        const size_t lds = (size_t)m * (prm->mode == DICP_PT2PL ? 6 : 3) * es;
        if (!G && !B->hist.spos && k1 > k0 && B->search.m_pad > 0 && lds <= 40 * 1024 &&
            small_loop_eligible(dtype, B->search.knn_variant & 0xff, B->search.knn_variant, n, B->search.m_pad)) {
            if (const int e = check_params(prm, B->c)) return e;
            begin_launch();
            const WeightParams P = to_params(prm);
            double* dst = ((k1 - k0) & 1) ? gpose_tmp : gpose;
#define DICP_SMALLB(T, M) icp_small_backward_kernel<T, M><<<N, BLOCK, lds, st>>>(P, *B, N, n, m, dim, gpose, dst, have_partials, \
                (T*)gsrc, (T*)gtgt, (T*)gw, (T*)bwd_partials, nblk, k0, k1)
            if (dtype == DICP_F32) { if (P.mode == MODE_PT2PL) DICP_SMALLB(float, MODE_PT2PL); else DICP_SMALLB(float, MODE_PT2PT); }
            else                   { if (P.mode == MODE_PT2PL) DICP_SMALLB(double, MODE_PT2PL); else DICP_SMALLB(double, MODE_PT2PT); }
#undef DICP_SMALLB
            return launch_status();
        }
    }
    double* gin = gpose;
    double* gout = gpose_tmp;
    int kt = k0;
    if (B->hist.spos && B->bwd.skip && B->bwd.tail_from > k0) {
        if (B->bwd.det_far_row) return DICP_ERR_SHAPE;
        if (k0 != 0) return DICP_ERR_SHAPE;
        if (!B->bwd.tail_partials || !B->bwd.tail_arrive) return DICP_ERR_NULL;
        if (nblk > dicp_bwd_tail_max_blocks(dtype)) return DICP_ERR_SHAPE;
        kt = B->bwd.tail_from < k1 ? B->bwd.tail_from : k1;
        if (B->bwd.overwrite && kt >= k1) kt = k1 - 1;
    }
    for (int k = k1 - 1; k >= kt; --k) {
        const char* pose_k = (const char*)B->hist.poses + (size_t)k * N * 12 * es;
// ... 114 lines not shown
```

### dicp_amd/csrc/dicp_math.h

```cpp
#pragma once
#include <math.h>

#if defined(__HIPCC__)
#define DICP_HD __host__ __device__ __forceinline__
#else
#define DICP_HD inline
#endif

namespace dicp {

enum Mode { MODE_PT2PT = 0, MODE_PT2PL = 1 };
enum Loss { LOSS_NONE = 0, LOSS_HUBER = 1, LOSS_CAUCHY = 2, LOSS_TRIM = 3 };

constexpr int ACC_A = 0, ACC_B = 21, ACC_COST = 27, ACC_SUMW = 28, ACC_NMATCH = 29, NACC = 30;
constexpr int NACC_PAD = 32;
constexpr int NBWD = 12, NBWD_PAD = 16;

struct WeightParams {
    int mode;
    int trim_on;
    int differentiable;
    int loss;
    double trim_dist;
    double tanh_k;
// ... 268 lines not shown
    gp[1] = C[1] * qbar[0] + C[4] * qbar[1] + C[7] * qbar[2];
    gp[2] = C[2] * qbar[0] + C[5] * qbar[1] + C[8] * qbar[2];
}


DICP_HD void so3_coeffs(const double* phi, double& a, double& b, double& c) {
    const double t2 = phi[0] * phi[0] + phi[1] * phi[1] + phi[2] * phi[2];
    if (t2 < 1e-8) {
        a = 1.0 - t2 / 6.0 + t2 * t2 / 120.0;
        b = 0.5 - t2 / 24.0 + t2 * t2 / 720.0;
        c = 1.0 / 6.0 - t2 / 120.0 + t2 * t2 / 5040.0;
    } else {
        const double t = sqrt(t2);
        a = sin(t) / t;
        b = (1.0 - cos(t)) / t2;
        c = (1.0 - a) / t2;
    }
}

DICP_HD void so3_exp(const double* phi, double* R) {
    double a, b, c;
    so3_coeffs(phi, a, b, c);
    const double x = phi[0], y = phi[1], z = phi[2];
    const double t2 = x * x + y * y + z * z;
    R[0] = 1.0 + b * (x * x - t2); R[1] = -a * z + b * x * y;     R[2] = a * y + b * x * z;
    R[3] = a * z + b * x * y;      R[4] = 1.0 + b * (y * y - t2); R[5] = -a * x + b * y * z;
    R[6] = -a * y + b * x * z;     R[7] = a * x + b * y * z;      R[8] = 1.0 + b * (z * z - t2);
}

template <typename T> DICP_HD void unpack_sym6(const T* tri21, double* A) {
    int k = 0;
    for (int i = 0; i < 6; ++i)
        for (int j = i; j < 6; ++j) { A[i * 6 + j] = A[j * 6 + i] = (double)tri21[k++]; }
}

DICP_HD int slot(int dim, int i) { return dim == 2 ? i + 2 : i; }
DICP_HD int ndof(int dim) { return dim == 2 ? 3 : 6; }

template <int D>
DICP_HD bool solve_fixed(double (&M)[D * D], double (&rhs)[D], double (&x)[D]) {
#pragma unroll
    for (int k = 0; k < D; ++k) {
        int piv = k;
        double best = fabs(M[k * D + k]);
#pragma unroll
        for (int i = k + 1; i < D; ++i) {
            const double v = fabs(M[i * D + k]);
            if (v > best) { best = v; piv = i; }
        }
        if (best == 0.0) return false;
#pragma unroll
        for (int i = k + 1; i < D; ++i) {
            const bool sw = (piv == i);
#pragma unroll
            for (int c = k; c < D; ++c) {
                const double a = M[k * D + c], b = M[i * D + c];
                M[k * D + c] = sw ? b : a;
                M[i * D + c] = sw ? a : b;
            }
            const double a = rhs[k], b = rhs[i];
            rhs[k] = sw ? b : a;
            rhs[i] = sw ? a : b;
        }
        const double inv = 1.0 / M[k * D + k];
#pragma unroll
        for (int i = k + 1; i < D; ++i) {
            const double f = M[i * D + k] * inv;
#pragma unroll
            for (int c = k + 1; c < D; ++c) M[i * D + c] -= f * M[k * D + c];
            rhs[i] -= f * rhs[k];
        }
    }
#pragma unroll
    for (int i = D - 1; i >= 0; --i) {
        double v = rhs[i];
#pragma unroll
        for (int c = i + 1; c < D; ++c) v -= M[i * D + c] * x[c];
        x[i] = v / M[i * D + i];
    }
    return true;
}

template <int D>
DICP_HD void step_solve_fixed(const double* A6, const double* b6, double* delta6, double* Areg) {
    constexpr int OFF = (D == 3) ? 2 : 0;
    double M[D * D], rhs[D], x[D];
#pragma unroll
    for (int i = 0; i < D; ++i) {
#pragma unroll
        for (int j = 0; j < D; ++j) M[i * D + j] = A6[(i + OFF) * 6 + (j + OFF)];
        M[i * D + i] += 1e-12;
        rhs[i] = b6[i + OFF];
    }
    for (int i = 0; i < 36; ++i) Areg[i] = 0.0;
#pragma unroll
    for (int i = 0; i < D; ++i)
#pragma unroll
        for (int j = 0; j < D; ++j) Areg[i * 6 + j] = M[i * D + j];
    for (int i = 0; i < 6; ++i) delta6[i] = 0.0;
    if (solve_fixed<D>(M, rhs, x)) {
#pragma unroll
        for (int i = 0; i < D; ++i) delta6[i + OFF] = -x[i];
    }
}

DICP_HD void step_solve(const double* A6, const double* b6, int dim, double* delta6, double* Areg) {
    if (dim == 2) step_solve_fixed<3>(A6, b6, delta6, Areg);
    else          step_solve_fixed<6>(A6, b6, delta6, Areg);
}

DICP_HD void step_forward(const double* A6, const double* b6, int dim, const double* C, const double* r,
                          double* delta6, double* Cn, double* rn, double* Areg) {
    step_solve(A6, b6, dim, delta6, Areg);
    double R[9];
    so3_exp(delta6, R);
    for (int i = 0; i < 3; ++i)
        for (int j = 0; j < 3; ++j)
            Cn[i * 3 + j] = R[0 * 3 + i] * C[0 * 3 + j] + R[1 * 3 + i] * C[1 * 3 + j] + R[2 * 3 + i] * C[2 * 3 + j];
    for (int i = 0; i < 3; ++i) rn[i] = r[i] - delta6[3 + i];
}

template <int D>
DICP_HD void step_backward_fixed(const double* gCn, const double* grn, const double* C,
                                 const double* delta6, const double* Areg,
                                 double* Gs, double* gb, double* gC, double* gr) {
    constexpr int OFF = (D == 3) ? 2 : 0;
    double R[9];
    so3_exp(delta6, R);
    double gR[9];
    for (int i = 0; i < 3; ++i)
        for (int j = 0; j < 3; ++j) {
            gC[i * 3 + j] = R[i * 3 + 0] * gCn[0 * 3 + j] + R[i * 3 + 1] * gCn[1 * 3 + j] + R[i * 3 + 2] * gCn[2 * 3 + j];
            gR[i * 3 + j] = C[i * 3 + 0] * gCn[j * 3 + 0] + C[i * 3 + 1] * gCn[j * 3 + 1] + C[i * 3 + 2] * gCn[j * 3 + 2];
        }
    for (int i = 0; i < 3; ++i) gr[i] = grn[i];
    double Mm[9];
    for (int i = 0; i < 3; ++i)
        for (int j = 0; j < 3; ++j)
            Mm[i * 3 + j] = gR[i * 3 + 0] * R[j * 3 + 0] + gR[i * 3 + 1] * R[j * 3 + 1] + gR[i * 3 + 2] * R[j * 3 + 2];
    const double v[3] = {Mm[7] - Mm[5], Mm[2] - Mm[6], Mm[3] - Mm[1]};
    double a, b, c;
    so3_coeffs(delta6, a, b, c);
    const double* phi = delta6;
    const double pv = phi[0] * v[0] + phi[1] * v[1] + phi[2] * v[2];
    double pxv[3];
    cross3(phi, v, pxv);
    double gd[6];
    for (int i = 0; i < 3; ++i) gd[i] = a * v[i] + c * phi[i] * pv - b * pxv[i];
    for (int i = 0; i < 3; ++i) gd[3 + i] = -grn[i];
    double Mx[D * D], rhs[D], g[D];
#pragma unroll
    for (int i = 0; i < D; ++i) {
#pragma unroll
        for (int j = 0; j < D; ++j) Mx[i * D + j] = Areg[i * 6 + j];
        rhs[i] = gd[i + OFF];
    }
    for (int i = 0; i < 36; ++i) Gs[i] = 0.0;
    for (int i = 0; i < 6; ++i) gb[i] = 0.0;
    if (!solve_fixed<D>(Mx, rhs, g)) return;
#pragma unroll
    for (int i = 0; i < D; ++i) {
        gb[i + OFF] = -g[i];
#pragma unroll
        for (int j = 0; j < D; ++j) Gs[(i + OFF) * 6 + (j + OFF)] = -(g[i] * delta6[j + OFF] + delta6[i + OFF] * g[j]);
    }
}
// ... 158 lines not shown
```

### dicp_amd/csrc/kernels_accumulate.h

```cpp
template <typename T, int H>
__device__ __forceinline__ void halve_step(T* v, int lane) {
    const bool up = (lane & (2 * H)) != 0;
#pragma unroll
    for (int k = 0; k < H; ++k) {
        const T keep = up ? v[H + k] : v[k];
        const T give = up ? v[k] : v[H + k];
        v[k] = keep + __shfl_xor(give, 2 * H);
    }
}
template <typename T, int NV, int PAD, int NT>
__device__ __forceinline__ void block_reduce_store(T* v, T* __restrict__ out, T* lds ) {
    static_assert(NV <= 32 && PAD >= NV, "reduce-scatter over 32 slots");
    const int tid = threadIdx.x, lane = tid & (WAVE - 1), wave = tid >> 6;
    if constexpr (NV <= 16) {
        T a[16];
#pragma unroll
        for (int k = 0; k < 16; ++k) a[k] = k < NV ? v[k] : T(0);
        halve_step<T, 8>(a, lane);
        halve_step<T, 4>(a, lane);
        halve_step<T, 2>(a, lane);
        halve_step<T, 1>(a, lane);
        T x = a[0] + __shfl_xor(a[0], 1);
        x += __shfl_xor(x, 32);
        const int slot = ((lane >> 4) & 1) * 8 + ((lane >> 3) & 1) * 4 + ((lane >> 2) & 1) * 2 + ((lane >> 1) & 1);
        if (!(lane & 33) && slot < NV) lds[wave * PAD + slot] = x;
        __syncthreads();
        if (tid < PAD) {
            T s = T(0);
            if (tid < NV) {
#pragma unroll
                for (int w = 0; w < NT / WAVE; ++w) s += lds[w * PAD + tid];
            }
            out[tid] = s;
        }
        return;
    }
    T a[32];
#pragma unroll
    for (int k = 0; k < 32; ++k) a[k] = k < NV ? v[k] : T(0);
    halve_step<T, 16>(a, lane);
    halve_step<T, 8>(a, lane);
    halve_step<T, 4>(a, lane);
    halve_step<T, 2>(a, lane);
    halve_step<T, 1>(a, lane);
    const T x = a[0] + __shfl_xor(a[0], 1);
    const int slot = ((lane >> 5) & 1) * 16 + ((lane >> 4) & 1) * 8 + ((lane >> 3) & 1) * 4 + ((lane >> 2) & 1) * 2 + ((lane >> 1) & 1);
    if (!(lane & 1) && slot < NV) lds[wave * PAD + slot] = x;
    __syncthreads();
    if (tid < PAD) {
        T s = T(0);
        if (tid < NV) {
#pragma unroll
            for (int w = 0; w < NT / WAVE; ++w) s += lds[w * PAD + tid];
        }
        out[tid] = s;
    }
}

constexpr bool PAIR_ROWS = true;
template <typename T, int NB> __device__ __forceinline__ void load_cached_row(const T* __restrict__ p, T* v) {
    if constexpr (NB == 6 && sizeof(T) == 4) {
        const float2* q = reinterpret_cast<const float2*>(p);
        const float2 a = q[0], b = q[1], c = q[2];
        v[0] = a.x; v[1] = a.y; v[2] = b.x; v[3] = b.y; v[4] = c.x; v[5] = c.y;
    } else {
#pragma unroll
        for (int k = 0; k < NB; ++k) v[k] = p[k];
    }
}
template <typename T, int NB> __device__ __forceinline__ void store_cached_row(T* __restrict__ p, const T* v) {
    if constexpr (NB == 6 && sizeof(T) == 4) {
        float2* q = reinterpret_cast<float2*>(p);
        q[0] = make_float2(v[0], v[1]); q[1] = make_float2(v[2], v[3]); q[2] = make_float2(v[4], v[5]);
    } else {
#pragma unroll
        for (int k = 0; k < NB; ++k) p[k] = v[k];
    }
}

#ifndef DICP_ACC_CERT_WAVES
#define DICP_ACC_CERT_WAVES 7
#endif
#ifndef DICP_ACC_PRELOAD
#define DICP_ACC_PRELOAD 2
#endif
template <typename T, int MODE, bool CERT = false>
__global__ __launch_bounds__(BLOCK, (CERT && sizeof(T) == 4) ? DICP_ACC_CERT_WAVES : 1) void accumulate_kernel(WeightParams P, const T* __restrict__ src, const T* __restrict__ tgt, int c ,
                                                           const int32_t* __restrict__ idx, const T* __restrict__ pose,
                                                           const T* __restrict__ w_init, const T* __restrict__ alive,
                                                           int N, int n, int m, int bpc, T* __restrict__ partials,
                                                           T* __restrict__ w_out, long w_stride, const int32_t* __restrict__ src_rows, AccCert<T> ps,
                                                           const T* __restrict__ w_prev ) {
    constexpr int NB = MODE == MODE_PT2PL ? 6 : 3;
    constexpr int ROUNDS = ACC_PTS / BLOCK;
    __shared__ T red[(BLOCK / WAVE) * NACC_PAD];
    int cloud, blk;
    if (!decode_block(bpc, N, cloud, blk)) return;
    const int nc = rows_of(src_rows, cloud, n);
    const int end = min(nc, (blk + 1) * ACC_PTS);
    const int lane = threadIdx.x & (WAVE - 1);
    const int wave = __builtin_amdgcn_readfirstlane((int)(threadIdx.x >> 6));
    bool cached = false;
    size_t of_k = 0;
    unsigned live_mask = 0, todo_mask = 0;
    int gslab[ROUNDS];
#pragma unroll
    for (int t = 0; t < ROUNDS; ++t) gslab[t] = 0;
    if (CERT) {
        of_k = ((size_t)ps.k * ps.N + cloud) * ps.nwr;
        const int cstate = ps.cloud ? ps.cloud[(size_t)cloud * CERT_CLOUD + 2] : 0;
        int dirty[ROUNDS];
#pragma unroll
        for (int t = 0; t < ROUNDS; ++t) {
            const int g0 = blk * ACC_PTS + t * BLOCK + wave * WAVE;
            const bool have = g0 < end;
            dirty[t] = (have && !ps.fresh) ? ps.gdirty[(size_t)cloud * ps.nwr + (g0 >> 6)] : 0;
            gslab[t] = (have && !ps.fresh && ps.of) ? ps.of[of_k + (g0 >> 6)] : ps.k;
            live_mask |= have ? (1u << t) : 0u;
        }
        cached = !ps.fresh && !(cstate > 0) && cstate != CERT_RECERTIFY;
        if (ps.cloud && !ps.fresh && blk == 0 && threadIdx.x == 0) { ps.cloud[(size_t)cloud * CERT_CLOUD + 3] = ps.units; ps.cloud[(size_t)cloud * CERT_CLOUD + 5] = ps.sets; }
        if (ps.fresh && ps.scount && blk == 0 && threadIdx.x == 0) ps.scount[cloud] = 0;
        if (cached) {
#pragma unroll
            for (int t = 0; t < ROUNDS; ++t)
                if (((live_mask >> t) & 1u) && (dirty[t] != 0 || (ps.of && gslab[t] < ps.k_floor))) todo_mask |= 1u << t;
        }
    }
    if (CERT && cached && todo_mask) {
#pragma unroll
        for (int t = 0; t < ROUNDS; ++t) {
            if (!((todo_mask >> t) & 1u)) continue;
            const int i = blk * ACC_PTS + t * BLOCK + (int)threadIdx.x;
            const int grp = (i - lane) >> 6;
            const int s = gslab[t];
            if (ps.of && s != ps.k) {
                const int32_t* from = (s < ps.k_floor ? ps.hist_prev : ps.hist) + ((size_t)s * ps.N + cloud) * n;
                if (i < end) ps.spos[(size_t)cloud * n + i] = from[i];
                if (lane == 0) ps.of[of_k + grp] = ps.k;
                gslab[t] = ps.k;
            }
            if (i < end) {
                const size_t pt = (size_t)cloud * n + i;
                const int pd = ps.pend[pt];
                if (pd != 0) {
                    ps.spos[pt] = pd - 2;
                    ps.pend[pt] = 0;
                    const T* yp = tgt + ((size_t)cloud * m + min(max(pd - 2, 0), m - 1)) * c;
                    T row[NB];
#pragma unroll
                    for (int e = 0; e < NB; ++e) row[e] = yp[e];
                    store_cached_row<T, NB>(ps.nbr + pt * NB, row);
                }
            }
            if (lane == 0) ps.gdirty[(size_t)cloud * ps.nwr + grp] = 0;
        }
    }
    T C[9], r[3];
    load_pose(pose, cloud, C, r);
    const T live = alive ? alive[cloud] : T(1);
    T acc[NACC];
#pragma unroll
    for (int k = 0; k < NACC; ++k) acc[k] = T(0);
    if (w_out)
        for (int i = max(blk * ACC_PTS, nc) + threadIdx.x; i < min(n, (blk + 1) * ACC_PTS); i += BLOCK) w_out[(size_t)cloud * w_stride + i] = T(0);
    const int32_t* __restrict__ ix = CERT ? ps.spos : idx;
    auto point = [&](const T* p, const T* y, const T* nrm, size_t pt, int i) {
        PointState<T> s;
        point_forward<T, MODE>(P, C, r, p, y, nrm, (w_init ? w_init[pt] : T(1)) * live, acc, s);
        if (w_out) w_out[(size_t)cloud * w_stride + i] = (w_prev && live == T(0)) ? w_prev[(size_t)cloud * w_stride + i] : s.w;
    };
    if (CERT && cached) {
        constexpr int PRE = DICP_ACC_PRELOAD < ROUNDS ? DICP_ACC_PRELOAD : ROUNDS;
#pragma unroll
        for (int t0 = 0; t0 < ROUNDS; t0 += PRE) {
            T pp[PRE][3], rw[PRE][NB];
#pragma unroll
            for (int u = 0; u < PRE; ++u) {
                const int i = blk * ACC_PTS + (t0 + u) * BLOCK + (int)threadIdx.x;
                const size_t pt = (size_t)cloud * n + min(i, end - 1);
                const T* sp = src + pt * 3;
                pp[u][0] = sp[0]; pp[u][1] = sp[1]; pp[u][2] = sp[2];
                load_cached_row<T, NB>(ps.nbr + pt * NB, rw[u]);
            }
#pragma unroll
            for (int u = 0; u < PRE; ++u) {
                const int t = t0 + u;
                const int i = blk * ACC_PTS + t * BLOCK + (int)threadIdx.x;
                if (ps.of && lane == 0 && ((live_mask >> t) & 1u))
                    ps.of[of_k + (size_t)ps.N * ps.nwr + ((i - lane) >> 6)] = gslab[t];
                if (i < end) {
                    const T nrm[3] = {MODE == MODE_PT2PL ? rw[u][NB - 3] : T(0), MODE == MODE_PT2PL ? rw[u][NB - 2] : T(0), MODE == MODE_PT2PL ? rw[u][NB - 1] : T(0)};
                    point(pp[u], rw[u], nrm, (size_t)cloud * n + i, i);
                }
            }
        }
    } else {
        for (int base = blk * ACC_PTS; base < end; base += BLOCK) {
            const int i = base + (int)threadIdx.x;
            const bool on = i < end;
            const size_t pt = (size_t)cloud * n + (on ? i : end - 1);
            const T* sp = src + pt * 3;
            const T p[3] = {sp[0], sp[1], sp[2]};
            T y[3], nrm[3] = {T(0), T(0), T(0)};
            const int jm = ix ? ix[pt] : (on ? i : end - 1);
            const int j = min(max(jm, 0), m - 1);
            if (MODE == MODE_PT2PL && PAIR_ROWS) {
                const int half = threadIdx.x & 1;
                const int je = __shfl(j, lane & ~1), jo = __shfl(j, lane | 1);
                const T* re = tgt + ((size_t)cloud * m + je) * c + 3 * half;
                const T* ro = tgt + ((size_t)cloud * m + jo) * c + 3 * half;
                const T e[3] = {re[0], re[1], re[2]}, o[3] = {ro[0], ro[1], ro[2]};
                const T pe[3] = {__shfl_xor(e[0], 1), __shfl_xor(e[1], 1), __shfl_xor(e[2], 1)};
                const T po[3] = {__shfl_xor(o[0], 1), __shfl_xor(o[1], 1), __shfl_xor(o[2], 1)};
                if (half == 0) { y[0] = e[0]; y[1] = e[1]; y[2] = e[2]; nrm[0] = pe[0]; nrm[1] = pe[1]; nrm[2] = pe[2]; }
                else           { y[0] = po[0]; y[1] = po[1]; y[2] = po[2]; nrm[0] = o[0]; nrm[1] = o[1]; nrm[2] = o[2]; }
            } else {
                const T* yp = tgt + ((size_t)cloud * m + j) * c;
                y[0] = yp[0]; y[1] = yp[1]; y[2] = yp[2];
                if (MODE == MODE_PT2PL) { nrm[0] = yp[3]; nrm[1] = yp[4]; nrm[2] = yp[5]; }
            }
            if (CERT && (i - lane) < end) {
                if (on) {
                    T row[NB];
                    row[0] = y[0]; row[1] = y[1]; row[2] = y[2];
                    if (MODE == MODE_PT2PL) { row[3] = nrm[0]; row[4] = nrm[1]; row[5] = nrm[2]; }
                    store_cached_row<T, NB>(ps.nbr + pt * NB, row);
                }
                if (lane == 0) {
                    const int grp = (i - lane) >> 6;
                    ps.gdirty[(size_t)cloud * ps.nwr + grp] = 0;
                    if (ps.of) { ps.of[of_k + grp] = ps.k; ps.of[of_k + (size_t)ps.N * ps.nwr + grp] = ps.k; }
                }
            }
            if (on) point(p, y, nrm, pt, i);
        }
    }
    block_reduce_store<T, NACC, NACC_PAD>(acc, partials + ((size_t)cloud * bpc + blk) * NACC_PAD, red);
}

__host__ __device__ inline dicp_step_io make_step_io(const dicp_loop_buffers& B, int k, int k0, int N, int n, int mode, int dim,
                                                     int const_iter, double tolerance, size_t es, int nblk) {
    dicp_step_io io;
    io.partials = B.partials; io.nblk = nblk; io.iter = k; io.dim = dim; io.const_iter = const_iter; io.tolerance = tolerance;
    io.rows_per_point = mode == DICP_PT2PT ? 3 : 1; io.n = n;
    io.pose_in = (const char*)B.hist.poses + (size_t)k * N * 12 * es; io.pose_out = (char*)B.hist.poses + (size_t)(k + 1) * N * 12 * es;
    io.frame = B.search.frame; io.pose_search_out = B.search.poses ? (char*)B.search.poses + (size_t)(k + 1) * N * 12 * es : nullptr;
    io.delta = (char*)B.hist.deltas + (size_t)k * 6 * es; io.delta_stride = (int64_t)B.K * 6;
    io.cost = (char*)B.hist.costs + (size_t)k * es; io.cost_prev = k > 0 ? (const char*)B.hist.costs + (size_t)(k - 1) * es : nullptr;
    io.cost_stride = B.K;
    io.areg = B.hist.areg ? B.hist.areg + (size_t)k * N * 36 : nullptr;
    io.alive = (const char*)B.hist.alive + (size_t)k * N * es; io.alive_out = (char*)B.hist.alive + (size_t)(k + 1) * N * es;
    io.converged = B.converged; io.iterations = B.iterations; io.matched_ratio = B.matched_ratio;
    io.n_start = B.n_start; io.n_matched = B.n_matched;
    io.w_cur = (char*)B.hist.w + (size_t)k * B.hist.w_iter * es;
    io.w_prev = k > k0 ? (const char*)B.hist.w + (size_t)(k - 1) * B.hist.w_iter * es : (const char*)B.hist.w_prev0; io.w_stride = B.hist.w_stride;
    io.n_not_converged = B.counters + k;
    io.rmax = B.cert.rmax; io.dcum = B.cert.dcum; io.dcum_stride = 2 * (B.K + 1);
    io.cert_cloud = B.cert.cloud;
    io.cert_qu = nullptr; io.cert_units = 0; io.glist_cap = 0; io.glist = nullptr; io.gcount = nullptr; io.cert_scount = nullptr; io.cert_slist = nullptr;
    io.w_copied = 0;
    return io;
}

template <typename T, int NT>
__device__ __forceinline__ void step_body(const dicp_step_io& io, int cloud, int tid) {
    __shared__ double sacc[NACC_PAD], sA[36], sAreg[36], spose[12], sout[24], smisc[16];
    __shared__ T sframe[12];
    __shared__ int scc[7];
    __shared__ int s_copy, s_next_state;
    __shared__ T s_dnext[2];
    if (tid < WAVE) {
        const int slot_i = tid & 31, part = tid >> 5;
        const T* pp = (const T*)io.partials + (size_t)cloud * io.nblk * NACC_PAD + slot_i;
        double s = 0.0;
        constexpr int UB = 8;
        for (int b0 = part; b0 < io.nblk; b0 += 2 * UB) {
            T v[UB];
#pragma unroll
            for (int u = 0; u < UB; ++u) v[u] = (b0 + 2 * u < io.nblk) ? pp[(size_t)(b0 + 2 * u) * NACC_PAD] : T(0);
#pragma unroll
            for (int u = 0; u < UB; ++u) if (b0 + 2 * u < io.nblk) s += (double)v[u];
        }
        s += __shfl_down(s, 32);
        if (tid < NACC_PAD) sacc[tid] = s;
        if (tid < 12) spose[tid] = (double)((const T*)io.pose_in)[(size_t)cloud * 12 + tid];
        if (tid == 40) smisc[0] = (double)((const T*)io.alive)[cloud];
        if (tid == 41) smisc[1] = io.cost_prev ? (double)((const T*)io.cost_prev)[(size_t)cloud * io.cost_stride] : 0.0;
        if (tid >= 42 && tid < 46) smisc[2 + (tid - 42)] = io.dcum ? (double)((const T*)io.rmax)[(size_t)cloud * 4 + (tid - 42)] : 0.0;
        if (tid >= 46 && tid < 49) smisc[6 + (tid - 46)] = io.frame ? (double)((const T*)io.frame)[(size_t)cloud * 12 + 9 + (tid - 46)] : 0.0;
        if (tid == 49) smisc[9] = io.dcum ? (double)((const T*)io.dcum)[(size_t)cloud * io.dcum_stride + 2 * io.iter] : 0.0;
        if (tid == 50) smisc[10] = (double)((const T*)io.n_start)[cloud];
        if (tid == 51) smisc[11] = (double)((const T*)io.iterations)[cloud];
        if (tid == 52) smisc[12] = (double)((const T*)io.matched_ratio)[cloud];
        if (tid >= 12 && tid < 24 && io.frame) sframe[tid - 12] = ((const T*)io.frame)[(size_t)cloud * 12 + (tid - 12)];
        if (tid >= 24 && tid < 31 && io.cert_cloud) scc[tid - 24] = io.cert_cloud[(size_t)cloud * CERT_CLOUD + (tid - 24)];
    }
    __syncthreads();
    if (tid == 0) {
        double* d6 = sout;
        unpack_sym6(sacc + ACC_A, sA);
        step_solve(sA, sacc + ACC_B, io.dim, d6, sAreg);
        T* dout = (T*)io.delta + (size_t)cloud * io.delta_stride;
        double nrm2 = 0.0;
        for (int k = 0; k < 6; ++k) { const T v = (T)d6[k]; dout[k] = v; d6[k] = (double)v; nrm2 += d6[k] * d6[k]; }
        double R[9];
        so3_exp(d6, R);
        T* pout = (T*)io.pose_out + (size_t)cloud * 12;
        const double* C = spose;
        T pn[12];
        for (int i = 0; i < 3; ++i)
            for (int j = 0; j < 3; ++j)
                pn[i * 3 + j] = (T)(R[0 * 3 + i] * C[0 * 3 + j] + R[1 * 3 + i] * C[1 * 3 + j] + R[2 * 3 + i] * C[2 * 3 + j]);
        for (int k = 0; k < 3; ++k) pn[9 + k] = (T)(spose[9 + k] - d6[3 + k]);
        for (int k = 0; k < 12; ++k) pout[k] = pn[k];
        if (io.dcum) {
            const double rad = smisc[2], p0[3] = {smisc[3], smisc[4], smisc[5]};
            double dC = 0.0, mv = 0.0, rn2 = 0.0;
            for (int i = 0; i < 3; ++i) {
                double m = (double)pn[9 + i] - spose[9 + i];
                for (int j = 0; j < 3; ++j) { const double d = (double)pn[i * 3 + j] - spose[i * 3 + j]; dC += d * d; m += d * p0[j]; }
                mv += m * m;
                rn2 += (double)pn[9 + i] * (double)pn[9 + i];
            }
            const double ulp = sizeof(T) == 4 ? 1.2e-7 : 2.3e-16;
            T* dc = (T*)io.dcum + (size_t)cloud * io.dcum_stride + 2 * io.iter;
            const T nxt = (T)((double)(T)smisc[9] + (sqrt(dC) * rad + sqrt(mv)) * 1.0001);
            dc[2] = nxt + m_abs(nxt) * (T)(4.0 * ulp);
            s_dnext[0] = dc[2];
            const double cn = io.frame ? sqrt(smisc[6] * smisc[6] + smisc[7] * smisc[7] + smisc[8] * smisc[8]) : 0.0;
            const double pnm = sqrt(p0[0] * p0[0] + p0[1] * p0[1] + p0[2] * p0[2]);
            dc[3] = (T)(8.0 * ulp * (pnm + rad + sqrt(rn2) + cn + 1.0) * 1.0001);
            s_dnext[1] = dc[3];
        }
        if (io.pose_search_out) {
            T* ps = (T*)io.pose_search_out + (size_t)cloud * 12;
            T Fr[12];
            for (int k = 0; k < 12; ++k) Fr[k] = io.frame ? sframe[k] : T(0);
            for (int k = 0; k < 12; ++k) ps[k] = frame_pose_entry<T>(io.frame ? Fr : nullptr, pn, k);
        }

        T cost = (T)sacc[ACC_COST];
        if (io.cost_prev && cost == T(0)) cost = (T)smisc[1];
        ((T*)io.cost)[(size_t)cloud * io.cost_stride] = cost;

        const double nmatch = sacc[ACC_NMATCH];
        if (io.n_matched) ((T*)io.n_matched)[cloud] = (T)nmatch;
        const T alive_in = (T)smisc[0];
        T alive_next = alive_in;
        const bool hit = (double)(T)sqrt(nrm2) < io.tolerance;
        if (hit) io.converged[cloud] = 1;
        else if (io.n_not_converged) atomicAdd(io.n_not_converged, 1);
        if (hit && !io.const_iter) {
            T* it = (T*)io.iterations + cloud;
            if ((T)smisc[11] == T(0)) *it = (T)(io.iter + 1);
            T* mr = (T*)io.matched_ratio + cloud;
            if ((T)smisc[12] == T(0)) {
                float start = (alive_in != T(0)) ? (float)(T)smisc[10] : 0.f;
                if (start == 0.f) start = 1.f;
                *mr = (T)((float)nmatch / start);
            }
            alive_next = T(0);
        }
        ((T*)io.alive_out)[cloud] = alive_next;
        s_copy = (io.w_cur && io.w_prev && sacc[ACC_SUMW] == 0.0 && !(io.w_copied && alive_in == T(0))) ? 1 : 0;
        s_next_state = io.cert_cloud ? scc[2] : 0;
        if (io.cert_cloud) {
            int32_t* cc = io.cert_cloud + (size_t)cloud * CERT_CLOUD;
            const int c_units = scc[0], c_single = scc[1], state = scc[2], units = scc[3], c_back = scc[4];
            const bool sets = scc[5] != 0;
            if (units > 0) {
                const bool costly = 1.3 * c_units + 0.12 * c_single > 0.6 * units;
                int next = state;
                if (state >= CERT_OFF_FOR_GOOD) next = state;
                else if (state > 0) next = state > 1 ? state - 1 : CERT_RECERTIFY;
                else if (state == CERT_RECERTIFY) next = sets ? (costly ? -1 : 0) : ((0.12 * c_single > 0.6 * units) ? CERT_OFF_FOR_GOOD : 0);
                else if (sets && 2 * scc[6] > io.n) next = CERT_OFF_FOR_GOOD;
                else if (!costly) next = 0;
                else if (c_units == 0 && !sets) next = CERT_OFF_FOR_GOOD;
                else if (state == -1 && sets && c_units == 0) next = CERT_OFF_FOR_GOOD;
                else if (state == -1) { const int d = c_back > 0 ? min(2 * c_back, 16) : 2; cc[4] = d; next = d; }
                else next = -1;
                cc[2] = next;
                s_next_state = next;
                if (costly || state > 0) cc[7] += 1;
                cc[0] = 0; cc[1] = 0; cc[3] = 0; cc[6] = 0;
            }
        }
    }
    __syncthreads();
    if (io.cert_qu && io.glist && tid < WAVE) {
        const T spent = cert_spent<T>(s_dnext);
        const int st = s_next_state;
        const bool certs_on = st <= 0 && st != CERT_RECERTIFY;
        const T* qu = (const T*)io.cert_qu + (size_t)cloud * io.cert_units;
        int32_t* list = io.glist + (size_t)(cloud & 7) * io.glist_cap;
        for (int u0 = 0; u0 < io.cert_units; u0 += WAVE) {
            const int u = u0 + tid;
            bool work = false;
            if (u < io.cert_units) { const T v = qu[u]; work = !(certs_on && v >= T(0) && v > spent); }
            const unsigned long long mk = __ballot(work);
            if (mk) {
                int base = 0;
                if (tid == 0) base = atomicAdd(io.gcount + (cloud & 7), __popcll(mk));
                base = __shfl(base, 0);
                const int rank = __builtin_amdgcn_mbcnt_hi((unsigned)(mk >> 32), __builtin_amdgcn_mbcnt_lo((unsigned)mk, 0u));
                if (work && base + rank < io.glist_cap) list[base + rank] = cloud * io.cert_units + u;
            }
        }
        if (io.cert_scount) {
            if (!certs_on) { if (tid == 0) io.cert_scount[cloud] = 0; }
            else {
                const int nwr = (io.n + WAVE - 1) / WAVE;
                const int have = min(io.cert_scount[cloud], io.n);
                const int nch = (have + WAVE - 1) / WAVE;
                if (io.cert_slist && nch > 0) {
                    const int upto = min(nch * WAVE, io.n);
                    for (int e = have + tid; e < upto; e += WAVE) io.cert_slist[(size_t)cloud * io.n + e] = -1;
                    if (tid == 0 && upto > have) io.cert_scount[cloud] = upto;
                }
                if (nch > 0) {
                    int base = 0;
                    if (tid == 0) base = atomicAdd(io.gcount + (cloud & 7), nch);
                    base = __shfl(base, 0);
                    for (int c = tid; c < nch; c += WAVE)
                        if (base + c < io.glist_cap) list[base + c] = -1 - (cloud * nwr + c);
                }
            }
        }
    }
    if (io.areg && tid < 36) io.areg[(size_t)cloud * 36 + tid] = sAreg[tid];
    if (s_copy) {
        T* wc = (T*)io.w_cur + (size_t)cloud * io.w_stride;
        const T* wp = (const T*)io.w_prev + (size_t)cloud * io.w_stride;
        for (int i = tid; i < io.n; i += NT) wc[i] = wp[i];
    }
}

template <typename T>
__global__ __launch_bounds__(WAVE) void step_kernel(dicp_step_io io, int N) {
    step_body<T, WAVE>(io, blockIdx.x, threadIdx.x);
}

__global__ __launch_bounds__(WAVE) void counters_report_kernel(const int32_t* __restrict__ counters, int32_t* __restrict__ host, int k0, int cnt, int tag) {
    for (int k = threadIdx.x; k < cnt; k += WAVE) {
        const int v = __hip_atomic_load(counters + k0 + k, __ATOMIC_RELAXED, __HIP_MEMORY_SCOPE_AGENT);
        __hip_atomic_store(host + k0 + k, (tag & 0x7ff00000) | (v < 0xfffff ? v : 0xfffff), __ATOMIC_RELAXED, __HIP_MEMORY_SCOPE_SYSTEM);
    }
}

template <typename T, int MODE>
__global__ __launch_bounds__(BLOCK) void icp_small_forward_kernel(WeightParams P, dicp_loop_buffers B, int N, int n, int m, int dim,
                                                                  int const_iter, double tolerance, int k0, int k1) {
    using T4 = typename V4<T>::type;
    extern __shared__ __align__(32) unsigned char small_lds[];
    T4* tg = reinterpret_cast<T4*>(small_lds);
    __shared__ T red[(BLOCK / WAVE) * NACC_PAD];
    const int cloud = blockIdx.x, tid = threadIdx.x, c = B.c;
    const int nc = rows_of(B.src_rows, cloud, n), mc = max(rows_of(B.tgt_rows, cloud, m), 1);
    const int m_pad = min((mc + KNN_PAD - 1) / KNN_PAD * KNN_PAD, B.search.m_pad);
    {
        const T4* __restrict__ g = (const T4*)B.search.tgt4 + (size_t)cloud * B.search.m_pad;
        for (int j = tid; j < m_pad; j += BLOCK) tg[j] = g[j];
    }
    __syncthreads();
    const T* __restrict__ src = (const T*)B.src + (size_t)cloud * n * 3;
    const T* __restrict__ tgt = (const T*)B.tgt + (size_t)cloud * m * c;
    const T* __restrict__ w_init = B.w_init ? (const T*)B.w_init + (size_t)cloud * n : nullptr;
    for (int k = k0; k < k1; ++k) {
        T C[9], r[3];
        load_pose((const T*)B.hist.poses + (size_t)k * N * 12, cloud, C, r);
        T Cs[9], rs[3];
        {
            const T pw[12] = {C[0], C[1], C[2], C[3], C[4], C[5], C[6], C[7], C[8], r[0], r[1], r[2]};
            const T* F = B.search.frame ? (const T*)B.search.frame + (size_t)cloud * 12 : nullptr;
#pragma unroll
            for (int e = 0; e < 9; ++e) Cs[e] = frame_pose_entry<T>(F, pw, e);
#pragma unroll
            for (int e = 0; e < 3; ++e) rs[e] = frame_pose_entry<T>(F, pw, 9 + e);
        }
        const T live = ((const T*)B.hist.alive)[(size_t)k * N + cloud];
        int32_t* __restrict__ idx_k = B.hist.idx + (B.hist.per_iter ? (size_t)k * N * n : 0) + (size_t)cloud * n;
        T* __restrict__ w_k = (T*)B.hist.w + (size_t)k * B.hist.w_iter + (size_t)cloud * B.hist.w_stride;
        T acc[NACC];
#pragma unroll
        for (int a = 0; a < NACC; ++a) acc[a] = T(0);
        for (int i = nc + tid; i < n; i += BLOCK) w_k[i] = T(0);
        for (int i = tid; i < nc; i += BLOCK) {
            const T p[3] = {src[i * 3], src[i * 3 + 1], src[i * 3 + 2]};
            T nx[3];
            query_point(Cs, rs, p, nx);
            T best = inf_v<T>();
            int bj = 0;
            for (int j = 0; j < m_pad; j += 4) {
                const T s0 = score<T, T4>(nx, tg[j]), s1 = score<T, T4>(nx, tg[j + 1]);
                const T s2 = score<T, T4>(nx, tg[j + 2]), s3 = score<T, T4>(nx, tg[j + 3]);
                if (s0 < best) { best = s0; bj = j; }
// ... 24 lines not shown
```

### dicp_amd/csrc/kernels_backward.h

```cpp
template <typename T, int MODE>
__global__ __launch_bounds__(BLOCK) void accumulate_bwd_kernel(WeightParams P, const T* __restrict__ src, const T* __restrict__ tgt, int c,
                                                               const int32_t* __restrict__ idx, const T* __restrict__ pose,
                                                               const T* __restrict__ w_init, const T* __restrict__ alive,
                                                               const T* __restrict__ gs, const T* __restrict__ gb,
                                                               int N, int n, int m, int bpc,
                                                               T* __restrict__ gsrc, T* __restrict__ gtgt, T* __restrict__ gw,
                                                               T* __restrict__ bwd_partials, const int32_t* __restrict__ src_rows,
                                                               const int32_t* __restrict__ skip ) {
    constexpr int CV = (MODE == MODE_PT2PL) ? 6 : 3;
    __shared__ T red[(BLOCK / WAVE) * NBWD_PAD];
    __shared__ T stage_v[(BLOCK / WAVE) * WAVE * CV];
    __shared__ int stage_j[BLOCK];
    int cloud, blk;
    if (!decode_block(bpc, N, cloud, blk)) return;
    if (skip && skip[cloud]) {
        if (threadIdx.x < NBWD_PAD) bwd_partials[((size_t)cloud * bpc + blk) * NBWD_PAD + threadIdx.x] = T(0);
        return;
    }
    const int tid = threadIdx.x, lane = tid & (WAVE - 1), wave = tid >> 6;
    T C[9], r[3], Gs[36], Gb[6];
    load_pose(pose, cloud, C, r);
#pragma unroll
    for (int k = 0; k < 36; ++k) Gs[k] = gs[(size_t)cloud * 36 + k];
#pragma unroll
// ... 669 lines not shown
        }
        const T* pose_k = (const T*)B.hist.poses + (size_t)k * N * 12;
        if (tid < NBWD) sg[tid] = spart[tid] + sgo[tid];
        if (tid < 9) sC[tid] = (double)pose_k[(size_t)cloud * 12 + tid];
        if (tid < 6) sd[tid] = (double)dlt[(size_t)k * 6 + tid];
        if (tid < 36) sAreg[tid] = B.hist.areg[((size_t)k * N + cloud) * 36 + tid];
        if (B.bwd.skip && tid >= WAVE && tid < 2 * WAVE) {
            double dm[6] = {0.0, 0.0, 0.0, 0.0, 0.0, 0.0};
            for (int j = tid - WAVE; j < k; j += WAVE) {
#pragma unroll
                for (int i = 0; i < 6; ++i) { const double v = fabs((double)dlt[(size_t)j * 6 + i]); dm[i] = v > dm[i] ? v : dm[i]; }
            }
#pragma unroll
            for (int i = 0; i < 6; ++i) {
#pragma unroll
                for (int off = WAVE / 2; off > 0; off >>= 1) { const double o = __shfl_down(dm[i], off); dm[i] = o > dm[i] ? o : dm[i]; }
            }
            if (tid == WAVE) {
#pragma unroll
                for (int i = 0; i < 6; ++i) sdmax[i] = dm[i];
            }
        }
        __syncthreads();
        if (tid == 0) {
            step_backward(sg, sg + 9, dim, sC, sd, sAreg, sGs, sGb, sgo, sgo + 9);
            s_skip = 0;
            if (B.bwd.skip) {
                const SkipArgs<T> sk{B.bwd.skip, B.bwd.mref, (const T*)B.hist.alive + (size_t)k * N, B.bwd.live ? B.bwd.live + k : nullptr, B.bwd.skip_eps, k};
                s_skip = skip_decision(sGs, sGb, sAreg, sdmax, dim, cloud, sk, sk.alive_k[cloud] != T(0), B.bwd.mref[cloud]);
                B.bwd.skip[cloud] = s_skip;
            }
        }
        __syncthreads();
        if (s_skip) {
            if (tid < NBWD_PAD) { spart[tid] = 0.0; part[tid] = T(0); }
            __syncthreads();
            if (s_skip == 2) { ended = true; }
            continue;
        }
        T C[9], r[3], Gs[36], Gb[6];
        load_pose(pose_k, cloud, C, r);
#pragma unroll
        for (int a = 0; a < 36; ++a) Gs[a] = (T)sGs[a];
#pragma unroll
        for (int a = 0; a < 6; ++a) Gb[a] = (T)sGb[a];
        const T live = ((const T*)B.hist.alive)[(size_t)k * N + cloud];
        const int32_t* __restrict__ idx_k = B.hist.idx + (size_t)k * N * n + (size_t)cloud * n;
        T acc[NBWD];
#pragma unroll
        for (int a = 0; a < NBWD; ++a) acc[a] = T(0);
        for (int i = tid; i < nc; i += NT) {
            const T p[3] = {src[i * 3], src[i * 3 + 1], src[i * 3 + 2]};
            const int j = min(max(idx_k[i], 0), m - 1);
            const T* yp = tgt + (size_t)j * c;
            const T y[3] = {yp[0], yp[1], yp[2]};
            T nrm[3] = {T(0), T(0), T(0)};
            if (MODE == MODE_PT2PL) { nrm[0] = yp[3]; nrm[1] = yp[4]; nrm[2] = yp[5]; }
            T gp[3], gy[3], gn[3], gw0;
            point_backward<T, MODE>(P, C, r, p, y, nrm, (w_init ? w_init[i] : T(1)) * live, Gs, Gb, gp, gy, gn, gw0, acc, acc + 9);
            T* gsp = gsrc + ((size_t)cloud * n + i) * 3;
            gsp[0] += gp[0]; gsp[1] += gp[1]; gsp[2] += gp[2];
            if (gw) gw[(size_t)cloud * n + i] += gw0 * live;
            if (gtgt) {
                T* row = gt + j * CV;
                atomicAdd(&row[0], gy[0]); atomicAdd(&row[1], gy[1]); atomicAdd(&row[2], gy[2]);
                if (MODE == MODE_PT2PL) { atomicAdd(&row[3], gn[0]); atomicAdd(&row[4], gn[1]); atomicAdd(&row[5], gn[2]); }
            }
        }
        block_reduce_store<T, NBWD, NBWD_PAD, NT>(acc, part, red);
        __syncthreads();
        if (tid < NBWD_PAD) spart[tid] = (double)part[tid];
        __syncthreads();
    }
    if (tid < 12) gpose_out[(size_t)cloud * 12 + tid] = sgo[tid];
    for (int e = tid; e < nblk * NBWD_PAD; e += NT)
        bwd_partials[(size_t)cloud * nblk * NBWD_PAD + e] = e < NBWD_PAD ? part[e] : T(0);
    if (gtgt)
        for (int e = tid; e < m * CV; e += NT) {
            const int j = e / CV, col = e - j * CV;
            gtgt[((size_t)cloud * m + j) * c + col] += gt[e];
        }
}

__device__ __forceinline__ void coherent_store(float* p, float v)   { __hip_atomic_store(p, v, __ATOMIC_RELAXED, __HIP_MEMORY_SCOPE_AGENT); }
__device__ __forceinline__ void coherent_store(double* p, double v) { __hip_atomic_store(p, v, __ATOMIC_RELAXED, __HIP_MEMORY_SCOPE_AGENT); }
__device__ __forceinline__ float  coherent_load(const float* p)  { return __hip_atomic_load(p, __ATOMIC_RELAXED, __HIP_MEMORY_SCOPE_AGENT); }
__device__ __forceinline__ double coherent_load(const double* p) { return __hip_atomic_load(p, __ATOMIC_RELAXED, __HIP_MEMORY_SCOPE_AGENT); }

template <typename T, int MODE, int WT>
__global__ __launch_bounds__(BLOCK, sizeof(T) == 4 ? 2 : 1) void bwd_tail_kernel(WeightParams P, dicp_loop_buffers B, int N, int n, int dim, int spb, int bpc,
                                                         const double* __restrict__ gpose_in, double* __restrict__ gpose_out, int have_partials,
                                                         T* __restrict__ gsrc_s, T* __restrict__ slab, T* __restrict__ gw_s,
                                                         T* part0 , T* part1 ,
                                                         int32_t* arrive , int k1) {
    __shared__ double sg[NBWD_PAD], sC[9], sd[6], sAreg[36], sGs[36], sGb[6], sgo[12], sdmax[6], sR[WAVE * 9], smref;
    __shared__ T sGsT[36], sGbT[6], spub[NBWD_PAD];
    __shared__ int s_verdict, s_alive, s_timeout;
    int cloud, blk;
    if (!decode_block(bpc, N, cloud, blk)) return;
    const int tid = threadIdx.x;
    bool ended = B.bwd.skip[cloud] == 2;
    if (ended && blk != 0) return;
    if (tid < 12) sgo[tid] = gpose_in[(size_t)cloud * 12 + tid];
    if (tid == 32) smref = B.bwd.mref[cloud];
    if (tid == 33) s_timeout = 0;
    const T* __restrict__ dlt = (const T*)B.hist.deltas + (size_t)cloud * B.K * 6;
    const T* cur = have_partials ? part0 : nullptr;
    int gen = 0;
    __syncthreads();
    auto fold = [&](const T* rows) {
        if (tid < WAVE) {
            const int slot_i = tid & 15, part = tid >> 4;
            double s = 0.0;
            if (rows && slot_i < NBWD) {
                const T* pp = rows + (size_t)cloud * bpc * NBWD_PAD + slot_i;
                constexpr int UB = 4;
                for (int b0 = part; b0 < bpc; b0 += 4 * UB) {
                    T v[UB];
#pragma unroll
                    for (int u = 0; u < UB; ++u) v[u] = (b0 + 4 * u < bpc) ? coherent_load(pp + (size_t)(b0 + 4 * u) * NBWD_PAD) : T(0);
#pragma unroll
                    for (int u = 0; u < UB; ++u) if (b0 + 4 * u < bpc) s += (double)v[u];
                }
            }
            s += __shfl_down(s, 32);
            s += __shfl_down(s, 16);
            if (tid < NBWD) sg[tid] = s_timeout ? __builtin_nan("") : s + sgo[tid];
        }
        __syncthreads();
    };
    for (int k = k1 - 1; k >= 0; --k) {
        if (ended) {
            fold(cur);
            cur = nullptr;
            if (tid < 12) sgo[tid] = sg[tid];
            __syncthreads();
            for (int kb = k; kb >= 0; kb -= WAVE) {
                const int cnt = min(WAVE, kb + 1);
                if (tid < cnt) {
                    const T* dp = dlt + (size_t)(kb - tid) * 6;
                    const double d[6] = {(double)dp[0], (double)dp[1], (double)dp[2], (double)dp[3], (double)dp[4], (double)dp[5]};
                    double R[9];
                    so3_exp(d, R);
#pragma unroll
                    for (int e = 0; e < 9; ++e) sR[tid * 9 + e] = R[e];
                }
                __syncthreads();
                if (tid < 3) {
                    double v0 = sgo[0 * 3 + tid], v1 = sgo[1 * 3 + tid], v2 = sgo[2 * 3 + tid];
                    for (int t = 0; t < cnt; ++t) {
                        const double* R = sR + t * 9;
                        const double a = R[0] * v0 + R[1] * v1 + R[2] * v2, b = R[3] * v0 + R[4] * v1 + R[5] * v2, cc = R[6] * v0 + R[7] * v1 + R[8] * v2;
                        v0 = a; v1 = b; v2 = cc;
                    }
                    sgo[0 * 3 + tid] = v0; sgo[1 * 3 + tid] = v1; sgo[2 * 3 + tid] = v2;
                }
                __syncthreads();
            }
            break;
        }
        const T* pose_k = (const T*)B.hist.poses + (size_t)k * N * 12;
        const T* alive_k = (const T*)B.hist.alive + (size_t)k * N;
        if (tid >= WAVE && tid < 2 * WAVE) {
            double dm[6] = {0.0, 0.0, 0.0, 0.0, 0.0, 0.0};
            for (int j = tid - WAVE; j < k; j += WAVE) {
#pragma unroll
                for (int i = 0; i < 6; ++i) { const double v = fabs((double)dlt[(size_t)j * 6 + i]); dm[i] = v > dm[i] ? v : dm[i]; }
            }
#pragma unroll
            for (int i = 0; i < 6; ++i) {
// ... 117 lines not shown
```

### include/dicp_hip.h

```cpp
#ifndef DICP_HIP_H
#define DICP_HIP_H
#include <stddef.h>
#include <stdint.h>

#ifdef __cplusplus
extern "C" {
#endif

#define DICP_ABI_VERSION 11

enum { DICP_F32 = 0, DICP_F64 = 1 };
enum { DICP_PT2PT = 0, DICP_PT2PL = 1 };
enum { DICP_LOSS_NONE = 0, DICP_LOSS_HUBER = 1, DICP_LOSS_CAUCHY = 2, DICP_LOSS_TRIM = 3 };
enum { DICP_KNN_AUTO = 0, DICP_KNN_VALU = 1, DICP_KNN_MFMA = 2, DICP_KNN_SWEEP = 3 ,
       DICP_KNN_GUMBEL = 4  };
enum { DICP_ERR_NULL = 1, DICP_ERR_SHAPE = 2, DICP_ERR_DTYPE = 3, DICP_ERR_ENUM = 4, DICP_ERR_ALIGN = 5, DICP_ERR_ABI = 6  };

#define DICP_NACC_PAD 32
#define DICP_NBWD_PAD 16

typedef struct dicp_weight_params {
    int32_t mode;
    int32_t trim_on;
    int32_t differentiable;
    int32_t loss;
    double trim_dist;
    double tanh_k;
    double loss_delta;
    double match_thresh;
} dicp_weight_params;

int dicp_abi_version(void);
int dicp_copy(void* dst, const void* src, size_t bytes, void* stream);
int dicp_zero(void* dst, size_t bytes, void* stream);

int dicp_padded_targets(int m);
int dicp_accumulate_blocks(int n);

int dicp_search_frame(int dtype, const void* tgt, int c, const int32_t* tgt_rows, int N, int m, double quantum, int directions,
                      const void* src, const int32_t* src_rows, int n, const void* T_init, void* frame, void* stream);

int dicp_pack_target(int dtype, const void* tgt, int c, const void* frame, const int32_t* tgt_rows, int N, int m, void* tgt4, int m_pad, void* stream);

size_t dicp_knn_f16_bytes(int N, int m_pad);
int dicp_knn_f16_pack(const void* tgt4, const int32_t* tgt_rows, int N, int m, int m_pad, void* image, void* stream);
int dicp_knn_f16_probe(const void* src, const void* pose, const void* tgt4, const void* f16_image, const int32_t* src_rows, const int32_t* tgt_rows,
                       int N, int n, int m, int m_pad, float* out, void* stream);

int dicp_knn(int dtype, const void* src, const void* pose, const void* tgt4, const int32_t* src_rows, const int32_t* tgt_rows,
             int N, int n, int m, int m_pad, int32_t* idx, int variant, const void* f16_image, void* stream);

size_t dicp_sweep_sort_scratch_bytes(int dtype, int N, int m_pad);
int dicp_sweep_sort(int dtype, const void* tgt, int c, const void* frame, const int32_t* tgt_rows, int N, int m, int m_pad, void* keys_sorted,
                    int32_t* tperm, int nbkt, int32_t* bucket, void* brange, void* scratch, size_t scratch_bytes, void* stream);
int dicp_sweep_build(int dtype, const void* tgt, int c, const void* frame, const int32_t* tgt_rows, const int32_t* tperm, int N, int m, int m_pad,
                     void* tgs4, void* tgt_s, int tgt_s_stride, void* stream);
int dicp_sweep_setup(int dtype, const void* tgt, int c, const int32_t* tgt_rows, int N, int m, int m_pad, double quantum, int directions,
                     void* frame, void* keys_sorted, int32_t* tperm, int nbkt, int32_t* bucket, void* brange, void* scratch, size_t scratch_bytes,
                     void* tgs4, void* tgt_s, int tgt_s_stride,
                     const void* src, const int32_t* src_rows, int n, const void* T_init, void* pose_search0, int32_t* qorder0, void* stream);

int dicp_query_keys(int dtype, const void* src, const void* pose, int N, int n, void* keys, void* stream);
int dicp_query_order(int dtype, const void* src, const void* pose, const void* brange, int nbkt, int N, int n, int32_t* qorder,
                     const void* w, void* src_s, void* w_s, int reproducible, const int32_t* spos_prev, int m_pad,
                     const void* keys_sorted, const int32_t* bucket, int m, const int32_t* src_rows, const int32_t* tgt_rows, void* stream);
int dicp_query_reorder(int dtype, const void* src, const void* pose, const void* pose_prev, const int32_t* order_prev, const void* brange, int nbkt, int N, int n,
                       int32_t* qorder, int m_pad, const void* skeys, const int32_t* bucket, int m, const int32_t* src_rows, const int32_t* tgt_rows, void* stream);

#define DICP_PAIR_SHARDS 64
int dicp_knn_sweep(int dtype, const void* src, const void* pose, const void* tgs4, const int32_t* tperm,
                   const int32_t* qorder, const int32_t* bucket, const void* brange, int nbkt, const int32_t* src_rows, const int32_t* tgt_rows,
                   int N, int n, int m, int m_pad, int32_t* idx, int32_t* spos, unsigned long long* pairs, int cfg, const void* f16_image,
                   const int32_t* form_in, int32_t* form_out, int form_default, void* stream);

int dicp_gather_rows(int dtype, const void* tgt, const int32_t* idx, int N, int n, int m, int c, void* out, void* stream);
int dicp_pack_list(int dtype, const void* const* ptrs, const int32_t* lens, const int32_t* strides, int N, int n_max, int cols, void* out, const void* pad, void* stream);
int dicp_unpack_list(int dtype, const void* gout, void* const* ptrs, const int32_t* lens, const int32_t* strides, int N, int n_max, int cols, int stride_max, void* stream);
int dicp_scatter_add_rows(int dtype, const void* gout, const int32_t* idx, int N, int n, int m, int c, void* gtgt, void* stream);

int dicp_accumulate(int dtype, const dicp_weight_params* prm, const void* src, const void* tgt, int c,
                    const int32_t* idx, const void* pose, const void* w_init, const void* alive, const int32_t* src_rows,
                    int N, int n, int m, void* partials, void* w_out, int64_t w_stride, void* stream);

typedef struct dicp_step_io {
    const void* partials;
    int32_t nblk;
    int32_t iter;
    int32_t dim;
    int32_t const_iter;
    double tolerance;
    int32_t rows_per_point;
    int32_t n;
    const void* pose_in;
    void* pose_out;
    void* delta;
    int64_t delta_stride;
    void* cost;
    const void* cost_prev;
// ... 173 lines not shown
int dicp_match_order(int dtype, const int32_t* spos_ref, const int32_t* src_rows, int N, int n, void* scratch, size_t scratch_bytes, int32_t* qorder, void* stream);


int dicp_step_bwd(int dtype, const double* gpose_in, const void* bwd_partials, int nblk, int dim,
                  const void* pose_k, const void* delta_k, int64_t delta_stride, const double* areg_k,
                  void* gs, void* gb, double* gpose_out, int N, void* stream);

int dicp_accumulate_bwd(int dtype, const dicp_weight_params* prm, const void* src, const void* tgt, int c,
                        const int32_t* idx, const void* pose, const void* w_init, const void* alive,
                        const void* gs, const void* gb, const int32_t* src_rows, int N, int n, int m,
                        void* gsrc, void* gtgt, void* gw, void* bwd_partials, void* stream);

int dicp_window_blocks(int dtype, int n, int m_pad);
int dicp_window_rows(int dtype);
int dicp_bwd_tail_max_blocks(int dtype);
int dicp_accumulate_bwd_window(int dtype, const dicp_weight_params* prm, const void* src_s, const void* tgt_s, int c,
                               const int32_t* spos, const int32_t* spos_ref, const int32_t* qorder, const void* pose, const void* w_s,
                               const void* alive, const void* gs, const void* gb, const int32_t* src_rows, int N, int n, int m_pad, void* gsrc_s, void* slab,
                               void* gts_far, void* gw_s, void* bwd_partials, int overwrite, void* stream);
int dicp_window_reduce(int dtype, const void* slab, const int32_t* spos_ref, const int32_t* qorder, const int32_t* tperm, const void* gts_far,
                       const int32_t* src_rows, int N, int n, int m, int m_pad, int cv, void* gtgt, int c, int overwrite, void* stream);

int dicp_permute_add_rows(int dtype, const void* in, const int32_t* perm, int N, int cnt, int in_rows, int perm_rows, int c_in, int cols,
                          void* out, int out_rows, int c_out, void* stream);
int dicp_permute_rows(int dtype, const void* in, const int32_t* perm, int N, int cnt, int in_rows, int perm_rows, int c_in, int cols,
                      void* out, int out_rows, int c_out, void* stream);

int dicp_gumbel_nn(int dtype, const void* x, const void* y, int c, const void* U, uint32_t seed, double eps, double tau,
                   int N, int n, int m, void* out, void* lse, void* stream);
int dicp_gumbel_nn_bwd(int dtype, const void* x, const void* y, int c, const void* U, uint32_t seed, double eps, double tau,
                       const void* out, const void* lse, const void* gout, int N, int n, int m, void* gx, void* gy, void* stream);

#define DICP_KAB_SAVE 40
int dicp_kabsch_accumulate(int dtype, const void* src, const void* tgt, int c, const int32_t* idx, const void* pose,
                           const void* w_init, int trim_on, double trim_dist, const int32_t* src_rows, int N, int n, int m, void* partials, void* stream);
int dicp_kabsch_step(int dtype, const void* partials, int nblk, void* pose_out, void* cost, double* save, int N, void* stream);
int dicp_kabsch_step_bwd(int dtype, const void* gpose, const double* save, void* gacc, int N, void* stream);

typedef struct dicp_kabsch_buffers {
    const void* src;
    const void* tgt;
    const void* w_init;
    int32_t c;
    int32_t K;
    int32_t knn_variant;
    int32_t m_pad;
    const void* tgt4;
    const int32_t* tperm;
    const int32_t* qorder;
    const int32_t* bucket;
    const void* brange;
    int32_t nbkt;
    int32_t pad0;
    unsigned long long* pairs;
    const void* frame;
    void* pose;
    void* pose_search;
    void* pose_used;
    int32_t* idx;
    void* partials;
    double* save;
    void* costs;
    void* iterations;
    int32_t* rows_live;
    const int32_t* tgt_rows;
    int32_t* counters;
    const void* tgt_f16;
} dicp_kabsch_buffers;
int dicp_kabsch_forward(int dtype, const dicp_kabsch_buffers* buf, int N, int n, int m, int trim_on, double trim_dist, int const_iter, double tolerance,
                        int k0, int k1, void* stream);
int dicp_kabsch_bwd(int dtype, const void* src, const void* tgt, int c, const int32_t* idx, const void* pose, const void* w_init,
                    int trim_on, double trim_dist, const void* gacc, const int32_t* src_rows, int N, int n, int m, void* gsrc, void* gtgt, void* gw, void* stream);

int dicp_transform_points(int dtype, const void* src, const void* pose, void* out, int N, int n, void* stream);
int dicp_transform_points_bwd(int dtype, const void* src, const void* pose, const void* gout, void* gsrc, void* partials,
                              int N, int n, void* stream);

int dicp_loss_weight(int dtype, int loss, int differentiable, double metric, double tanh_k,
                     const void* err, int64_t rows, int r, void* w, void* stream);
int dicp_loss_weight_bwd(int dtype, int loss, int differentiable, double metric, double tanh_k,
                         const void* err, const void* gw, int64_t rows, int r, void* gerr, void* stream);

#define DICP_CALL_NBKT 1024
enum { DICP_CALL_FIRST_SEARCH = 1 , DICP_CALL_NO_SMALL_LOOP = 2  };
typedef struct dicp_call {
    const void* src;
    const void* tgt;
    const void* T_init;
    const void* w0;
    int32_t N, n, m, c;
    int32_t K;
    int32_t dim;
    int32_t need_grad;
    int32_t n_resort;
    int32_t resort[DICP_MAX_SEGMENTS];
    int32_t flags;
    int32_t directions;
    double quantum;
    double tolerance;
    void* workspace;
    void* results;
    void* T_out;
    void* pc_out;
} dicp_call;
typedef struct dicp_call_layout {
    size_t total, zeroed;
    size_t results_total, results_zeroed;
    size_t T, pc;
    size_t deltas, weights, costs, converged, iterations, matched_ratio;
    size_t pairs;
    size_t n_matched, counters, poses, poses_search, alive, areg, n_start, partials, tgs4, tperm, bucket, brange, keys, tgt_sorted, scratch, scratch_bytes,
           frame, pose_s, orders, spos;
    int32_t n_orders, m_pad, nblk, pad0;
} dicp_call_layout;
int dicp_call_plan(int dtype, const dicp_call* call, dicp_call_layout* layout);
int dicp_call_forward(int dtype, const dicp_weight_params* prm, const dicp_call* call, void* stream);

typedef struct dicp_call_grads {
    const void* gT;
    void* gsrc;
    void* gtgt;
    void* gT0;
    void* gw;
    void* workspace;
    double skip_eps;
    int32_t tail_from;
    int32_t pad0;
    int32_t* live_host;
} dicp_call_grads;
typedef struct dicp_call_backward_layout {
    size_t total, zeroed;
    size_t live, arrive;
    size_t mref, decisions, far, gpose, gtmp, src_s, w_s, gsrc_s, gw_s, slab, gs, gb, partials, tail_partials;
    size_t spos_ref;
    int32_t nblk_w, pad0;
} dicp_call_backward_layout;
int dicp_call_backward_plan(int dtype, const dicp_weight_params* prm, const dicp_call* call, int want_tgt, int want_w, dicp_call_backward_layout* layout);
int dicp_call_backward(int dtype, const dicp_weight_params* prm, const dicp_call* call, const dicp_call_grads* grads, void* stream);
typedef struct dicp_loop_backward_in {
    const void* src;
    const void* tgt_sorted;
    const void* w0;
    const int32_t* tperm;
    const int32_t* qorder;
    const int32_t* spos;
    const void* poses;
    const void* deltas;
    const double* areg;
    const void* alive;
    const int32_t* src_rows;
    const int32_t* tgt_rows;
    const int32_t* spos_of;
    int32_t N, n, m, c, K, K_cap, m_pad, dim;
    int32_t knn_variant;
    int32_t spos_of_from;
    const void* src_s;
    const void* w_s;
    const int32_t* spos_ref;
} dicp_loop_backward_in;
int dicp_loop_backward_prepare(int dtype, const dicp_loop_backward_in* fwd, void* src_s_out, void* w_s_out, int32_t* spos_ref_out, void* stream);
int dicp_loop_backward_plan(int dtype, const dicp_weight_params* prm, const dicp_loop_backward_in* fwd, int want_tgt, int want_w, dicp_call_backward_layout* layout);
int dicp_loop_backward(int dtype, const dicp_weight_params* prm, const dicp_loop_backward_in* fwd, const dicp_call_grads* grads, void* stream);

typedef struct dicp_kabsch_call {
    const void* src;
    const void* tgt;
    const void* T_start;
// ... 57 lines not shown
```

Measured before the change: 3.323 million.

## Fuse step kernel into accumulate via last-block arrival counter (opt-in)

Adds an optional fused-step mode: the accumulate kernel writes its partials with coherent stores, counts arriving blocks with an atomic, and the last block per cloud runs the step solve. This is meant to remove a separate step-kernel launch per iteration. The step solve also becomes a wave-parallel Gaussian elimination in both paths. The fused flag defaults to False, so only the new solver affects default runs, while the fused path adds extra fence and atomic cost.

```diff
diff --git a/dicp_amd/ICP.py b/dicp_amd/ICP.py
--- a/dicp_amd/ICP.py
+++ b/dicp_amd/ICP.py
@@ -45,6 +45,7 @@
             first_search=True,
             plan_call=True,
             bwd_tail=True,
+            fused_step=False,
             one_call=True,
             timing_events=None)
         self._hints = CallHints()
@@ -109,7 +110,7 @@
             sync_every=self.sync_every, timing_events=self._tuning["timing_events"], small_loop=False if deterministic else bool(self._tuning["small_loop"]),
             src_rows=src_rows, tgt_rows=tgt_rows, sweep_resort=resort_schedule(self._tuning["sweep_resort"], source.shape[0], source.shape[1], int(self.max_iterations), bool(self.reuse_matches), self._tuning["cert_from"]), reuse_matches=bool(self.reuse_matches), cert_from=self._tuning["cert_from"],
             bwd_skip_eps=self.bwd_skip_eps, cert_backoff=bool(self._tuning["cert_backoff"]), cert_sets=bool(self._tuning["cert_sets"]), cert_hint=bool(self._tuning["cert_hint"]),
-            plan_call=bool(self._tuning["plan_call"]), bwd_tail=bool(self._tuning["bwd_tail"]), first_search=first_search, strict_errors=bool(self.strict_errors),
+            plan_call=bool(self._tuning["plan_call"]), bwd_tail=bool(self._tuning["bwd_tail"]), first_search=first_search, strict_errors=bool(self.strict_errors), fused_step=bool(self._tuning["fused_step"]),
             gumbel=(self.nn.eps, self.nn.tau, getattr(self.nn, "_inject_U", None)) if soft else None)
         T_c = T_init.contiguous()
         if self._tuning["one_call"] and not deterministic and _call.eligible(cfg, source, target, T_c, w_pts, wants_grad):
diff --git a/dicp_amd/_call.py b/dicp_amd/_call.py
--- a/dicp_amd/_call.py
+++ b/dicp_amd/_call.py
@@ -78,7 +78,7 @@
                 stats.pop(key, None)
         ctx.set_materialize_grads(False)
         resort = tuple(sorted(set(k for k in cfg.sweep_resort if 0 < k < K)))
-        flags = (_lib.CALL_FIRST_SEARCH if cfg.first_search else 0) | (0 if cfg.small_loop else _lib.CALL_NO_SMALL_LOOP)
+        flags = (_lib.CALL_FIRST_SEARCH if cfg.first_search else 0) | (0 if cfg.small_loop else _lib.CALL_NO_SMALL_LOOP) | (_lib.CALL_FUSED_STEP if cfg.fused_step else 0)
         L = _plan(code, N, n, m, c, K, int(cfg.dim), need_grad, resort, flags)
         P = cfg.params()
         with _on(dev):
diff --git a/dicp_amd/_lib.py b/dicp_amd/_lib.py
--- a/dicp_amd/_lib.py
+++ b/dicp_amd/_lib.py
@@ -138,6 +138,8 @@
 
 
 CALL_FIRST_SEARCH, CALL_NO_SMALL_LOOP, CALL_NBKT = 1, 2, 1024
+CALL_FUSED_STEP = 4
+LOOP_FUSED_STEP = 1 << 26
 
 
 class KabschBuffers(ctypes.Structure):
diff --git a/dicp_amd/_loop.py b/dicp_amd/_loop.py
--- a/dicp_amd/_loop.py
+++ b/dicp_amd/_loop.py
@@ -132,6 +132,7 @@
     strict_errors: bool = False
     plan_call: bool = True
     first_search: bool = True
+    fused_step: bool = False
     cert_hint: bool = True
     cert_sets: bool = True
     cert_backoff: bool = True
@@ -332,7 +333,6 @@
     S.alive = torch.empty((Kmax + 1, N), dtype=dt, device=dev)
     S.areg = torch.empty((Kmax, N, 36), dtype=torch.float64, device=dev) if S.need_grad else None
     S.n_start = torch.empty((N,), dtype=dt, device=dev)
-    S.partials = torch.empty((N, S.nblk, _lib.NACC_PAD), dtype=dt, device=dev)
     want_certs = S.want_certs
     arena = _Arena(dev)
     arena.take((N, Kmax, 6), dt)
@@ -348,8 +348,11 @@
     arena.take((Kmax + 1, 8) if want_certs else (0,), torch.int32)
     arena.take((Kmax, N) if S.adaptive else (0,), torch.int32)
     arena.take((N,) if (want_certs and cfg.cert_sets) else (0,), torch.int32)
+    arena.take((N, S.nblk, _lib.NACC_PAD) if cfg.fused_step else (0,), dt)
     (S.deltas, S.costs, S.converged, S.iterations, S.matched, S.n_matched, S.counters, cert_count, S.cert_cloud, cert_pend, cert_gcount, S.sweep_form,
-     cert_scount) = arena.finish()
+     cert_scount, S.partials) = arena.finish()
+    if not cfg.fused_step:
+        S.partials = torch.empty((N, S.nblk, _lib.NACC_PAD), dtype=dt, device=dev)
     S.certs = None
     if want_certs:
         units = (n + 63) // 64
@@ -413,7 +416,7 @@
 def _fwd_loop_buffers(S, plan_call):
     cfg, sweep, certs = S.cfg, S.sweep, S.certs
     LB = _lib.LoopBuffers(
-        src=_p(S.src), tgt=_p(S.tgt), w_init=_p(S.w0c), c=S.c, K=S.Kmax, search_knn_variant=S.kind | (cfg.knn_variant & 0xff00) | ((0 if cfg.small_loop else 1) << 25), search_m_pad=S.m_pad,
+        src=_p(S.src), tgt=_p(S.tgt), w_init=_p(S.w0c), c=S.c, K=S.Kmax, search_knn_variant=S.kind | (cfg.knn_variant & 0xff00) | ((0 if cfg.small_loop else 1) << 25) | (_lib.LOOP_FUSED_STEP if cfg.fused_step else 0), search_m_pad=S.m_pad,
         search_tgt4=_p(S.tgt4), search_tperm=_p(sweep.tperm) if sweep else None,
         search_bucket=_p(sweep.bucket) if sweep else None, search_brange=_p(sweep.brange) if sweep else None,
         search_nbkt=SweepIndex.NBKT, hist_per_iter=int(S.need_grad), search_pairs=_p(sweep.pair_shards) if sweep else None,
diff --git a/dicp_amd/csrc/dicp_call.hip b/dicp_amd/csrc/dicp_call.hip
--- a/dicp_amd/csrc/dicp_call.hip
+++ b/dicp_amd/csrc/dicp_call.hip
@@ -87,6 +87,7 @@
     L->n_matched = w.take(N * es);
     L->counters = w.take(K * 4);
     L->pairs = w.take(DICP_PAIR_SHARDS * 8);
+    if (c->flags & DICP_CALL_FUSED_STEP) L->partials = w.take(N * L->nblk * DICP_NACC_PAD * es);
     L->zeroed = w.off;
     L->T = w.take(N * 16 * es);
     L->pc = w.take(N * n * 3 * es);
@@ -95,7 +96,7 @@
     L->alive = w.take((K + 1) * N * es);
     L->areg = c->need_grad ? w.take(K * N * 36 * 8) : 0;
     L->n_start = w.take(N * es);
-    L->partials = w.take(N * L->nblk * DICP_NACC_PAD * es);
+    if (!(c->flags & DICP_CALL_FUSED_STEP)) L->partials = w.take(N * L->nblk * DICP_NACC_PAD * es);
     L->tgs4 = w.take(N * m_pad * 4 * es);
     L->tperm = w.take(N * m_pad * 4);
     L->bucket = w.take(N * (DICP_CALL_NBKT + 1) * 4);
@@ -155,7 +156,7 @@
     memset(&B, 0, sizeof(B));
     B.abi = DICP_ABI_VERSION;
     B.src = c->src; B.tgt = c->tgt; B.w_init = c->w0; B.c = c->c; B.K = K;
-    B.search.knn_variant = DICP_KNN_SWEEP | ((c->flags & DICP_CALL_NO_SMALL_LOOP) ? (1 << 25) : 0);
+    B.search.knn_variant = DICP_KNN_SWEEP | ((c->flags & DICP_CALL_NO_SMALL_LOOP) ? (1 << 25) : 0) | ((c->flags & DICP_CALL_FUSED_STEP) ? DICP_LOOP_FUSED_STEP : 0);
     B.search.m_pad = L.m_pad;
     B.search.tgt4 = at(c, L.tgs4); B.search.tperm = (int32_t*)at(c, L.tperm); B.search.bucket = (int32_t*)at(c, L.bucket); B.search.brange = at(c, L.brange);
     B.search.nbkt = DICP_CALL_NBKT; B.hist.per_iter = c->need_grad ? 1 : 0; B.search.pairs = (unsigned long long*)at(c, L.pairs);
diff --git a/dicp_amd/csrc/dicp_kernels.hip b/dicp_amd/csrc/dicp_kernels.hip
--- a/dicp_amd/csrc/dicp_kernels.hip
+++ b/dicp_amd/csrc/dicp_kernels.hip
@@ -408,7 +408,8 @@
 
 static int accumulate_go(int dtype, const dicp_weight_params* prm, const void* src, const void* tgt, int c,
                          const int32_t* idx, const void* pose, const void* w_init, const void* alive, const int32_t* src_rows,
-                         int N, int n, int m, void* partials, void* w_out, int64_t w_stride, void* stream, const CertAcc* ca, const void* w_prev = nullptr) {
+                         int N, int n, int m, void* partials, void* w_out, int64_t w_stride, void* stream, const CertAcc* ca, const void* w_prev = nullptr,
+                         const dicp_step_io* fused = nullptr ) {
     if (const int e = check_params(prm, c)) return e;
     if (!src || !tgt || !partials) return DICP_ERR_NULL;
     if (bad_dtype(dtype)) return DICP_ERR_DTYPE;
@@ -420,8 +421,9 @@
     const unsigned g = grid_for(N, bpc);
     hipEvent_t ev0, ev1;
     take_launch_events(ev0, ev1);
-#define DICP_ACC(T, M, CERT, PS) hipExtLaunchKernelGGL((accumulate_kernel<T, M, CERT>), dim3(g), dim3(BLOCK), 0, st, ev0, ev1, 0, P, (const T*)src, (const T*)tgt, c, idx, (const T*)pose, \
-        (const T*)w_init, (const T*)alive, N, n, m, bpc, (T*)partials, (T*)w_out, (long)w_stride, src_rows, PS, (const T*)w_prev)
+#define DICP_ACC_F(T, M, CERT, PS, F, FS) hipExtLaunchKernelGGL((accumulate_kernel<T, M, CERT, F>), dim3(g), dim3(BLOCK), 0, st, ev0, ev1, 0, P, (const T*)src, (const T*)tgt, c, idx, (const T*)pose, \
+        (const T*)w_init, (const T*)alive, N, n, m, bpc, (T*)partials, (T*)w_out, (long)w_stride, src_rows, PS, (const T*)w_prev, FS)
+#define DICP_ACC(T, M, CERT, PS) do { if (fused) { FusedStep<true> fs; fs.io = *fused; DICP_ACC_F(T, M, CERT, PS, true, fs); } else DICP_ACC_F(T, M, CERT, PS, false, FusedStep<false>{}); } while (0)
 #define DICP_ACC_T(T) do { \
         AccCert<T> ps{}; \
         if (ca) { \
@@ -432,6 +434,7 @@
     if (dtype == DICP_F32) DICP_ACC_T(float); else DICP_ACC_T(double);
 #undef DICP_ACC_T
 #undef DICP_ACC
+#undef DICP_ACC_F
     return launch_status();
 }
 
@@ -441,12 +444,16 @@
     return accumulate_go(dtype, prm, src, tgt, c, idx, pose, w_init, alive, src_rows, N, n, m, partials, w_out, w_stride, stream, nullptr);
 }
 
-int dicp_step(int dtype, const dicp_step_io* io, int N, void* stream) {
+static int check_step_io(int dtype, const dicp_step_io* io, int N) {
     if (!io || !io->partials || !io->pose_in || !io->pose_out || !io->delta || !io->cost || !io->alive || !io->alive_out ||
         !io->converged || !io->iterations || !io->matched_ratio || !io->n_start) return DICP_ERR_NULL;
     if (bad_dtype(dtype)) return DICP_ERR_DTYPE;
     if (N <= 0 || io->nblk <= 0 || (io->dim != 2 && io->dim != 3) || io->delta_stride < 6 || io->cost_stride < 1 ||
         (io->w_cur && io->w_stride < io->n)) return DICP_ERR_SHAPE;
+    return 0;
+}
+int dicp_step(int dtype, const dicp_step_io* io, int N, void* stream) {
+    if (const int e = check_step_io(dtype, io, N)) return e;
     hipStream_t st = (hipStream_t)stream;
     begin_launch();
     if (dtype == DICP_F32) step_kernel<float><<<N, WAVE, 0, st>>>(*io, N);
@@ -843,6 +850,7 @@
         if (const int e = launch_status()) return e;
         return report_counters(B, const_iter, k0, k1, stream);
     }
+    const bool fuse = (B->search.knn_variant & DICP_LOOP_FUSED_STEP) != 0;
     for (int k = k0; k < k1; ++k) {
         const char* pose_k = (const char*)B->hist.poses + (size_t)k * N * 12 * es;
         const char* pose_s = B->search.poses ? (const char*)B->search.poses + (size_t)k * N * 12 * es : pose_k;
@@ -850,6 +858,19 @@
         char* w_k = (char*)B->hist.w + (size_t)k * B->hist.w_iter * es;
         const char* w_prev_k = k > k0 ? (const char*)B->hist.w + (size_t)(k - 1) * B->hist.w_iter * es : (const char*)B->hist.w_prev0;
         const char* alive_k = (const char*)B->hist.alive + (size_t)k * N * es;
+        dicp_step_io io = make_step_io(*B, k, k0, N, n, prm->mode, dim, const_iter, tolerance, es, nblk);
+        io.w_copied = w_prev_k ? 1 : 0;
+        if (kind == DICP_KNN_SWEEP && B->cert.q && B->cert.qu && B->cert.glist && B->cert.gcount && B->cert.rmax && B->cert.dcum && k + 1 < B->K) {
+            const int cfgp = ((B->search.knn_variant >> 8) & 0xff) ? ((B->search.knn_variant >> 8) & 0xff) : sweep_auto_cfg(N, n);
+            const int Qp = sweep_queries_per_lane(cfgp);
+            if (Qp > 0) {
+                io.cert_qu = B->cert.qu; io.cert_units = (n + WAVE * Qp - 1) / (WAVE * Qp); io.glist_cap = guard_list_cap(N, n);
+                io.glist = B->cert.glist; io.gcount = B->cert.gcount + (size_t)(k + 1) * 8;
+                io.cert_scount = B->cert.set ? B->cert.scount : nullptr; io.cert_slist = B->cert.set ? B->cert.slist : nullptr;
+            }
+        }
+        const dicp_step_io* fio = fuse ? &io : nullptr;
+        if (fuse) if (const int e = check_step_io(dtype, &io, N)) return e;
         if (B->events) {
             if (kind == DICP_KNN_SWEEP) set_launch_events((hipEvent_t)B->events[6 * k + 0], (hipEvent_t)B->events[6 * k + 1]);
             else if (hipEventRecord((hipEvent_t)B->events[6 * k + 0], st) != hipSuccess) return -(int)hipGetLastError();
@@ -892,12 +913,12 @@
                 const CertAcc ca{spos_k, B->hist.spos, B->hist.spos_prev_chunk, B->hist.per_iter ? B->hist.spos_of : nullptr, B->hist.spos_floor, k,
                                  B->cert.nbr, B->cert.gdirty, B->cert.pend, B->cert.cloud, fresh ? 1 : 0, cert_units, B->cert.set ? 1 : 0, B->cert.scount};
                 rc = accumulate_go(dtype, prm, B->src, B->search.tgt_sorted, B->search.tgt_sorted_stride, spos_k, pose_k, B->w_init, alive_k, B->src_rows, N, n, B->search.m_pad,
-                                   B->partials, w_k, B->hist.w_stride, stream, &ca, w_prev_k);
+                                   B->partials, w_k, B->hist.w_stride, stream, &ca, w_prev_k, fio);
             } else if (sorted_rows)
                 rc = accumulate_go(dtype, prm, B->src, B->search.tgt_sorted, B->search.tgt_sorted_stride, spos_k, pose_k, B->w_init, alive_k, B->src_rows, N, n, B->search.m_pad,
-                                   B->partials, w_k, B->hist.w_stride, stream, nullptr, w_prev_k);
+                                   B->partials, w_k, B->hist.w_stride, stream, nullptr, w_prev_k, fio);
             else
-                rc = accumulate_go(dtype, prm, B->src, B->tgt, B->c, idx_k, pose_k, B->w_init, alive_k, B->src_rows, N, n, m, B->partials, w_k, B->hist.w_stride, stream, nullptr, w_prev_k);
+                rc = accumulate_go(dtype, prm, B->src, B->tgt, B->c, idx_k, pose_k, B->w_init, alive_k, B->src_rows, N, n, m, B->partials, w_k, B->hist.w_stride, stream, nullptr, w_prev_k, fio);
             set_launch_events(nullptr, nullptr);
             if (rc) return rc;
         } else if (G) {
@@ -910,7 +931,7 @@
                 if (hipEventRecord((hipEvent_t)B->events[6 * k + 1], st) != hipSuccess) return -(int)hipGetLastError();
                 set_launch_events((hipEvent_t)B->events[6 * k + 2], (hipEvent_t)B->events[6 * k + 3]);
             }
-            rc = accumulate_go(dtype, prm, B->src, nbr_k, B->c, nullptr, pose_k, B->w_init, alive_k, nullptr, N, n, n, B->partials, w_k, B->hist.w_stride, stream, nullptr, w_prev_k);
+            rc = accumulate_go(dtype, prm, B->src, nbr_k, B->c, nullptr, pose_k, B->w_init, alive_k, nullptr, N, n, n, B->partials, w_k, B->hist.w_stride, stream, nullptr, w_prev_k, fio);
             set_launch_events(nullptr, nullptr);
             if (rc) return rc;
         } else {
@@ -920,23 +941,14 @@
                 if (hipEventRecord((hipEvent_t)B->events[6 * k + 1], st) != hipSuccess) return -(int)hipGetLastError();
                 set_launch_events((hipEvent_t)B->events[6 * k + 2], (hipEvent_t)B->events[6 * k + 3]);
             }
-            rc = accumulate_go(dtype, prm, B->src, B->tgt, B->c, idx_k, pose_k, B->w_init, alive_k, B->src_rows, N, n, m, B->partials, w_k, B->hist.w_stride, stream, nullptr, w_prev_k);
+            rc = accumulate_go(dtype, prm, B->src, B->tgt, B->c, idx_k, pose_k, B->w_init, alive_k, B->src_rows, N, n, m, B->partials, w_k, B->hist.w_stride, stream, nullptr, w_prev_k, fio);
             set_launch_events(nullptr, nullptr);
             if (rc) return rc;
         }
-        dicp_step_io io = make_step_io(*B, k, k0, N, n, prm->mode, dim, const_iter, tolerance, es, nblk);
-        io.w_copied = w_prev_k ? 1 : 0;
-        if (kind == DICP_KNN_SWEEP && B->cert.q && B->cert.qu && B->cert.glist && B->cert.gcount && B->cert.rmax && B->cert.dcum && k + 1 < B->K) {
-            const int cfgp = ((B->search.knn_variant >> 8) & 0xff) ? ((B->search.knn_variant >> 8) & 0xff) : sweep_auto_cfg(N, n);
-            const int Qp = sweep_queries_per_lane(cfgp);
-            if (Qp > 0) {
-                io.cert_qu = B->cert.qu; io.cert_units = (n + WAVE * Qp - 1) / (WAVE * Qp); io.glist_cap = guard_list_cap(N, n);
-                io.glist = B->cert.glist; io.gcount = B->cert.gcount + (size_t)(k + 1) * 8;
-                io.cert_scount = B->cert.set ? B->cert.scount : nullptr; io.cert_slist = B->cert.set ? B->cert.slist : nullptr;
-            }
+        if (!fuse) {
+            rc = dicp_step(dtype, &io, N, stream);
+            if (rc) return rc;
         }
-        rc = dicp_step(dtype, &io, N, stream);
-        if (rc) return rc;
     }
     return report_counters(B, const_iter, k0, k1, stream);
 }
diff --git a/dicp_amd/csrc/dicp_math.h b/dicp_amd/csrc/dicp_math.h
--- a/dicp_amd/csrc/dicp_math.h
+++ b/dicp_amd/csrc/dicp_math.h
@@ -374,6 +374,28 @@
 }
 
 template <int D>
+DICP_HD int lane_pivot(const double (&col)[D], int k, double& best) {
+    int piv = k;
+    best = fabs(col[k]);
+#pragma unroll
+    for (int i = 0; i < D; ++i) {
+        if (i <= k) continue;
+        const double v = fabs(col[i]);
+        if (v > best) { best = v; piv = i; }
+    }
+    return piv;
+}
+DICP_HD int lane_swap_row(int i, int k, int piv) { return i == k ? piv : (i == piv ? k : i); }
+DICP_HD void lane_eliminate(double& m, double& r, int i, int c, int k, double mik, double mkk, double mkc, double rk) {
+    if (i <= k) return;
+    const double inv = 1.0 / mkk;
+    const double f = mik * inv;
+    if (c > k) m -= f * mkc;
+    r -= f * rk;
+}
+DICP_HD void lane_back_step(double& v, double mic, double xc) { v -= mic * xc; }
+
+template <int D>
 DICP_HD void step_solve_fixed(const double* A6, const double* b6, double* delta6, double* Areg) {
     constexpr int OFF = (D == 3) ? 2 : 0;
     double M[D * D], rhs[D], x[D];
diff --git a/dicp_amd/csrc/kernels_accumulate.h b/dicp_amd/csrc/kernels_accumulate.h
--- a/dicp_amd/csrc/kernels_accumulate.h
+++ b/dicp_amd/csrc/kernels_accumulate.h
@@ -8,6 +8,8 @@
         v[k] = keep + __shfl_xor(give, 2 * H);
     }
 }
+template <typename T, int NV, int PAD, int NT>
+__device__ __forceinline__ T block_reduce_row(T* v, T* lds);
 template <typename T, int NV, int PAD, int NT>
 __device__ __forceinline__ void block_reduce_store(T* v, T* __restrict__ out, T* lds ) {
     static_assert(NV <= 32 && PAD >= NV, "reduce-scatter over 32 slots");
@@ -35,6 +37,12 @@
         }
         return;
     }
+    const T s = block_reduce_row<T, NV, PAD, NT>(v, lds);
+    if (tid < PAD) out[tid] = s;
+}
+template <typename T, int NV, int PAD, int NT>
+__device__ __forceinline__ T block_reduce_row(T* v, T* lds ) {
+    const int tid = threadIdx.x, lane = tid & (WAVE - 1), wave = tid >> 6;
     T a[32];
 #pragma unroll
     for (int k = 0; k < 32; ++k) a[k] = k < NV ? v[k] : T(0);
@@ -47,15 +55,20 @@
     const int slot = ((lane >> 5) & 1) * 16 + ((lane >> 4) & 1) * 8 + ((lane >> 3) & 1) * 4 + ((lane >> 2) & 1) * 2 + ((lane >> 1) & 1);
     if (!(lane & 1) && slot < NV) lds[wave * PAD + slot] = x;
     __syncthreads();
-    if (tid < PAD) {
-        T s = T(0);
-        if (tid < NV) {
-#pragma unroll
-            for (int w = 0; w < NT / WAVE; ++w) s += lds[w * PAD + tid];
-        }
-        out[tid] = s;
-    }
-}
+    T s = T(0);
+    if (tid < NV) {
+#pragma unroll
+        for (int w = 0; w < NT / WAVE; ++w) s += lds[w * PAD + tid];
+    }
+    return s;
+}
+
+__device__ __forceinline__ void coherent_store(float* p, float v)   { __hip_atomic_store(p, v, __ATOMIC_RELAXED, __HIP_MEMORY_SCOPE_AGENT); }
+__device__ __forceinline__ void coherent_store(double* p, double v) { __hip_atomic_store(p, v, __ATOMIC_RELAXED, __HIP_MEMORY_SCOPE_AGENT); }
+__device__ __forceinline__ void coherent_store(int32_t* p, int32_t v) { __hip_atomic_store(p, v, __ATOMIC_RELAXED, __HIP_MEMORY_SCOPE_AGENT); }
+__device__ __forceinline__ float  coherent_load(const float* p)  { return __hip_atomic_load(p, __ATOMIC_RELAXED, __HIP_MEMORY_SCOPE_AGENT); }
+__device__ __forceinline__ double coherent_load(const double* p) { return __hip_atomic_load(p, __ATOMIC_RELAXED, __HIP_MEMORY_SCOPE_AGENT); }
+__device__ __forceinline__ int32_t coherent_load(const int32_t* p) { return __hip_atomic_load(p, __ATOMIC_RELAXED, __HIP_MEMORY_SCOPE_AGENT); }
 
 constexpr bool PAIR_ROWS = true;
 template <typename T, int NB> __device__ __forceinline__ void load_cached_row(const T* __restrict__ p, T* v) {
@@ -84,13 +97,18 @@
 #ifndef DICP_ACC_PRELOAD
 #define DICP_ACC_PRELOAD 2
 #endif
-template <typename T, int MODE, bool CERT = false>
+template <typename T, int NT, bool FUSED = false>
+__device__ __forceinline__ void step_body(const dicp_step_io& io, int cloud, int tid);
+template <bool FUSED> struct FusedStep {};
+template <> struct FusedStep<true> { dicp_step_io io; };
+template <typename T, int MODE, bool CERT = false, bool FUSED = false>
 __global__ __launch_bounds__(BLOCK, (CERT && sizeof(T) == 4) ? DICP_ACC_CERT_WAVES : 1) void accumulate_kernel(WeightParams P, const T* __restrict__ src, const T* __restrict__ tgt, int c ,
                                                            const int32_t* __restrict__ idx, const T* __restrict__ pose,
                                                            const T* __restrict__ w_init, const T* __restrict__ alive,
                                                            int N, int n, int m, int bpc, T* __restrict__ partials,
                                                            T* __restrict__ w_out, long w_stride, const int32_t* __restrict__ src_rows, AccCert<T> ps,
-                                                           const T* __restrict__ w_prev ) {
+                                                           const T* __restrict__ w_prev ,
+                                                           FusedStep<FUSED> fs) {
     constexpr int NB = MODE == MODE_PT2PL ? 6 : 3;
     constexpr int ROUNDS = ACC_PTS / BLOCK;
     __shared__ T red[(BLOCK / WAVE) * NACC_PAD];
@@ -119,8 +137,13 @@
             live_mask |= have ? (1u << t) : 0u;
         }
         cached = !ps.fresh && !(cstate > 0) && cstate != CERT_RECERTIFY;
+        if (FUSED) {
+            if (ps.cloud && !ps.fresh && blk == 0 && threadIdx.x == 0) { coherent_store(ps.cloud + (size_t)cloud * CERT_CLOUD + 3, ps.units); coherent_store(ps.cloud + (size_t)cloud * CERT_CLOUD + 5, ps.sets); }
+            if (ps.fresh && ps.scount && blk == 0 && threadIdx.x == 0) coherent_store(ps.scount + cloud, 0);
+        } else {
         if (ps.cloud && !ps.fresh && blk == 0 && threadIdx.x == 0) { ps.cloud[(size_t)cloud * CERT_CLOUD + 3] = ps.units; ps.cloud[(size_t)cloud * CERT_CLOUD + 5] = ps.sets; }
         if (ps.fresh && ps.scount && blk == 0 && threadIdx.x == 0) ps.scount[cloud] = 0;
+        }
         if (cached) {
 #pragma unroll
             for (int t = 0; t < ROUNDS; ++t)
@@ -236,7 +259,32 @@
             if (on) point(p, y, nrm, pt, i);
         }
     }
-    block_reduce_store<T, NACC, NACC_PAD>(acc, partials + ((size_t)cloud * bpc + blk) * NACC_PAD, red);
+    if constexpr (!FUSED) {
+        block_reduce_store<T, NACC, NACC_PAD>(acc, partials + ((size_t)cloud * bpc + blk) * NACC_PAD, red);
+    } else {
+        __shared__ int s_last;
+        const T s = block_reduce_row<T, NACC, NACC_PAD, BLOCK>(acc, red);
+        if (threadIdx.x < NACC) coherent_store(partials + ((size_t)cloud * bpc + blk) * NACC_PAD + threadIdx.x, s);
+        if (w_out) {
+            T sw = T(0);
+#pragma unroll
+            for (int w = 0; w < BLOCK / WAVE; ++w) sw += red[w * NACC_PAD + ACC_SUMW];
+            if (sw == T(0) && fs.io.w_cur && fs.io.w_prev && !(fs.io.w_copied && live == T(0))) {
+                __builtin_amdgcn_fence(__ATOMIC_RELEASE, "agent");
+                asm volatile("s_waitcnt vmcnt(0)" ::: "memory");
+                __syncthreads();
+            }
+        }
+        if (threadIdx.x == 0) {
+            asm volatile("s_waitcnt vmcnt(0)" ::: "memory");
+            int32_t* arrive = reinterpret_cast<int32_t*>(partials + (size_t)cloud * bpc * NACC_PAD + NACC);
+            const int last = __hip_atomic_fetch_add(arrive, 1, __ATOMIC_RELAXED, __HIP_MEMORY_SCOPE_AGENT) == bpc - 1;
+            if (last) coherent_store(arrive, 0);
+            s_last = last;
+        }
+        __syncthreads();
+        if (s_last) step_body<T, BLOCK, true>(fs.io, cloud, (int)threadIdx.x);
+    }
 }
 
 __host__ __device__ inline dicp_step_io make_step_io(const dicp_loop_buffers& B, int k, int k0, int N, int n, int mode, int dim,
@@ -263,9 +311,58 @@
     return io;
 }
 
-template <typename T, int NT>
+__device__ __forceinline__ double lane_value(double v, int src) {
+    const int lo = __builtin_amdgcn_readlane(__double2loint(v), src), hi = __builtin_amdgcn_readlane(__double2hiint(v), src);
+    return __hiloint2double(hi, lo);
+}
+template <int D>
+__device__ __forceinline__ void wave_step_solve(const double* acc, int lane, double* delta6, double* Areg) {
+    constexpr int OFF = (D == 3) ? 2 : 0;
+    const int l = lane < D * D ? lane : 0;
+    const int i = l / D, c = l % D;
+    const int a = min(i, c) + OFF, b = max(i, c) + OFF;
+    double m = acc[ACC_A + a * 6 - a * (a - 1) / 2 + (b - a)];
+    if (i == c) m += 1e-12;
+    double r = acc[ACC_B + i + OFF];
+    if (lane < 36) Areg[lane] = 0.0;
+    if (lane == 0) {
+#pragma unroll
+        for (int q = 0; q < 6; ++q) delta6[q] = 0.0;
+    }
+    if (lane < D * D) Areg[i * 6 + c] = m;
+    bool ok = true;
+#pragma unroll
+    for (int k = 0; k < D; ++k) {
+        double col[D];
+#pragma unroll
+        for (int q = 0; q < D; ++q) col[q] = q >= k ? lane_value(m, q * D + k) : 0.0;
+        double best;
+        const int piv = lane_pivot<D>(col, k, best);
+        if (best == 0.0) { ok = false; break; }
+        const int from = lane_swap_row(i, k, piv) * D + c;
+        m = __shfl(m, from);
+        r = __shfl(r, from);
+        const double mik = __shfl(m, i * D + k), mkk = lane_value(m, k * D + k), mkc = __shfl(m, k * D + c), rk = lane_value(r, k * D);
+        lane_eliminate(m, r, i, c, k, mik, mkk, mkc, rk);
+    }
+    if (!ok) return;
+    double x[D];
+#pragma unroll
+    for (int q = D - 1; q >= 0; --q) {
+        double v = lane_value(r, q * D);
+#pragma unroll
+        for (int e = q + 1; e < D; ++e) lane_back_step(v, lane_value(m, q * D + e), x[e]);
+        x[q] = v / lane_value(m, q * D + q);
+    }
+    if (lane == 0) {
+#pragma unroll
+        for (int q = 0; q < D; ++q) delta6[q + OFF] = -x[q];
+    }
+}
+
+template <typename T, int NT, bool FUSED>
 __device__ __forceinline__ void step_body(const dicp_step_io& io, int cloud, int tid) {
-    __shared__ double sacc[NACC_PAD], sA[36], sAreg[36], spose[12], sout[24], smisc[16];
+    __shared__ double sacc[NACC_PAD], sAreg[36], spose[12], sout[24], smisc[16];
     __shared__ T sframe[12];
     __shared__ int scc[7];
     __shared__ int s_copy, s_next_state;
@@ -274,11 +371,14 @@
         const int slot_i = tid & 31, part = tid >> 5;
         const T* pp = (const T*)io.partials + (size_t)cloud * io.nblk * NACC_PAD + slot_i;
         double s = 0.0;
-        constexpr int UB = 8;
+        constexpr int UB = FUSED ? 16 : 8;
         for (int b0 = part; b0 < io.nblk; b0 += 2 * UB) {
             T v[UB];
 #pragma unroll
-            for (int u = 0; u < UB; ++u) v[u] = (b0 + 2 * u < io.nblk) ? pp[(size_t)(b0 + 2 * u) * NACC_PAD] : T(0);
+            for (int u = 0; u < UB; ++u) {
+                if (FUSED) v[u] = (b0 + 2 * u < io.nblk && slot_i < NACC) ? coherent_load(pp + (size_t)(b0 + 2 * u) * NACC_PAD) : T(0);
+                else v[u] = (b0 + 2 * u < io.nblk) ? pp[(size_t)(b0 + 2 * u) * NACC_PAD] : T(0);
+            }
 #pragma unroll
             for (int u = 0; u < UB; ++u) if (b0 + 2 * u < io.nblk) s += (double)v[u];
         }
@@ -294,13 +394,16 @@
         if (tid == 51) smisc[11] = (double)((const T*)io.iterations)[cloud];
         if (tid == 52) smisc[12] = (double)((const T*)io.matched_ratio)[cloud];
         if (tid >= 12 && tid < 24 && io.frame) sframe[tid - 12] = ((const T*)io.frame)[(size_t)cloud * 12 + (tid - 12)];
-        if (tid >= 24 && tid < 31 && io.cert_cloud) scc[tid - 24] = io.cert_cloud[(size_t)cloud * CERT_CLOUD + (tid - 24)];
+        if (tid >= 24 && tid < 31 && io.cert_cloud)
+            scc[tid - 24] = FUSED ? coherent_load(io.cert_cloud + (size_t)cloud * CERT_CLOUD + (tid - 24)) : io.cert_cloud[(size_t)cloud * CERT_CLOUD + (tid - 24)];
     }
     __syncthreads();
+    if (tid < WAVE) {
+        if (io.dim == 2) wave_step_solve<3>(sacc, tid, sout, sAreg);
+        else             wave_step_solve<6>(sacc, tid, sout, sAreg);
+    }
     if (tid == 0) {
         double* d6 = sout;
-        unpack_sym6(sacc + ACC_A, sA);
-        step_solve(sA, sacc + ACC_B, io.dim, d6, sAreg);
         T* dout = (T*)io.delta + (size_t)cloud * io.delta_stride;
         double nrm2 = 0.0;
         for (int k = 0; k < 6; ++k) { const T v = (T)d6[k]; dout[k] = v; d6[k] = (double)v; nrm2 += d6[k] * d6[k]; }
@@ -412,7 +515,7 @@
             if (!certs_on) { if (tid == 0) io.cert_scount[cloud] = 0; }
             else {
                 const int nwr = (io.n + WAVE - 1) / WAVE;
-                const int have = min(io.cert_scount[cloud], io.n);
+                const int have = min(FUSED ? coherent_load(io.cert_scount + cloud) : io.cert_scount[cloud], io.n);
                 const int nch = (have + WAVE - 1) / WAVE;
                 if (io.cert_slist && nch > 0) {
                     const int upto = min(nch * WAVE, io.n);
diff --git a/dicp_amd/csrc/kernels_backward.h b/dicp_amd/csrc/kernels_backward.h
--- a/dicp_amd/csrc/kernels_backward.h
+++ b/dicp_amd/csrc/kernels_backward.h
@@ -775,10 +775,6 @@
         }
 }
 
-__device__ __forceinline__ void coherent_store(float* p, float v)   { __hip_atomic_store(p, v, __ATOMIC_RELAXED, __HIP_MEMORY_SCOPE_AGENT); }
-__device__ __forceinline__ void coherent_store(double* p, double v) { __hip_atomic_store(p, v, __ATOMIC_RELAXED, __HIP_MEMORY_SCOPE_AGENT); }
-__device__ __forceinline__ float  coherent_load(const float* p)  { return __hip_atomic_load(p, __ATOMIC_RELAXED, __HIP_MEMORY_SCOPE_AGENT); }
-__device__ __forceinline__ double coherent_load(const double* p) { return __hip_atomic_load(p, __ATOMIC_RELAXED, __HIP_MEMORY_SCOPE_AGENT); }
 
 template <typename T, int MODE, int WT>
 __global__ __launch_bounds__(BLOCK, sizeof(T) == 4 ? 2 : 1) void bwd_tail_kernel(WeightParams P, dicp_loop_buffers B, int N, int n, int dim, int spb, int bpc,
diff --git a/include/dicp_hip.h b/include/dicp_hip.h
--- a/include/dicp_hip.h
+++ b/include/dicp_hip.h
@@ -14,6 +14,7 @@
 enum { DICP_LOSS_NONE = 0, DICP_LOSS_HUBER = 1, DICP_LOSS_CAUCHY = 2, DICP_LOSS_TRIM = 3 };
 enum { DICP_KNN_AUTO = 0, DICP_KNN_VALU = 1, DICP_KNN_MFMA = 2, DICP_KNN_SWEEP = 3 ,
        DICP_KNN_GUMBEL = 4  };
+enum { DICP_LOOP_FUSED_STEP = 1 << 26  };
 enum { DICP_ERR_NULL = 1, DICP_ERR_SHAPE = 2, DICP_ERR_DTYPE = 3, DICP_ERR_ENUM = 4, DICP_ERR_ALIGN = 5, DICP_ERR_ABI = 6  };
 
 #define DICP_NACC_PAD 32
@@ -353,7 +354,8 @@
                          const void* err, const void* gw, int64_t rows, int r, void* gerr, void* stream);
 
 #define DICP_CALL_NBKT 1024
-enum { DICP_CALL_FIRST_SEARCH = 1 , DICP_CALL_NO_SMALL_LOOP = 2  };
+enum { DICP_CALL_FIRST_SEARCH = 1 , DICP_CALL_NO_SMALL_LOOP = 2 ,
+       DICP_CALL_FUSED_STEP = 4  };
 typedef struct dicp_call {
     const void* src;
     const void* tgt;
```

Measured after the change: 3.321 million (median of 2 runs). About the same (-0.1%).
